# voichek/kmersGWAS

Measured on AMD Instinct MI355X. Metric: k-mers x permutations scored/sec, higher is better.
Workload: dtype fp4 x fp6/fp4 block-scaled filter + f32/f64 exact re-score

## Files before the change

include/kgwas.h:

```cpp
#ifndef KGWAS_H
#define KGWAS_H

#include <stddef.h>
#include <stdint.h>

#ifdef __cplusplus
extern "C" {
#endif

#define KGWAS_OK 0
#define KGWAS_ERR_ARG (-1)
#define KGWAS_ERR_IO (-2)
#define KGWAS_ERR_FORMAT (-3)
#define KGWAS_ERR_DEVICE (-4)
#define KGWAS_ERR_STATE (-5)
#define KGWAS_ERR_NOMEM (-6)

const char* kgwas_last_error(void);
int kgwas_version(void);
int kgwas_device_count(int* n_devices);
uint32_t kgwas_host_cpu_quota(void);

typedef struct kgwas_table kgwas_table;
int kgwas_table_open(const char* base, uint32_t kmer_len, kgwas_table** out);
int kgwas_table_info(const kgwas_table* t, uint64_t* n_acc_file, uint64_t* n_rows, uint64_t* words_per_row,
                     uint32_t* kmer_len);
int kgwas_table_name(const kgwas_table* t, uint64_t i, const char** name);
int kgwas_table_column_map(const kgwas_table* t, const char* const* acc, uint64_t n, uint64_t* col_out);
int kgwas_table_read_rows(kgwas_table* t, uint64_t row0, uint64_t n, uint64_t* dst);
void kgwas_table_close(kgwas_table* t);

typedef struct kgwas_pheno kgwas_pheno;
int kgwas_pheno_load(const char* path, kgwas_pheno** out);
int kgwas_pheno_info(const kgwas_pheno* p, uint64_t* n_pheno, uint64_t* n_acc);
int kgwas_pheno_name(const kgwas_pheno* p, uint64_t j, const char** name);
int kgwas_pheno_accession(const kgwas_pheno* p, uint64_t i, const char** acc);
int kgwas_pheno_values(const kgwas_pheno* p, const float** Y);
void kgwas_pheno_free(kgwas_pheno* p);

uint64_t kgwas_min_count(uint64_t n_acc, double maf, uint64_t mac);

int kgwas_heap_selfcheck(uint32_t flags);
typedef struct kgwas_heap kgwas_heap;
int kgwas_heap_new(uint64_t max_results, kgwas_heap** out);
int kgwas_heap_add_many(kgwas_heap* h, const uint64_t* kmer, const double* score, const uint64_t* row, uint64_t n);
int kgwas_heap_size(const kgwas_heap* h, uint64_t* size, uint64_t* insertions, double* lowest);
int kgwas_heap_pop_all(const kgwas_heap* h, uint64_t* kmer, double* score, uint64_t* row);
int kgwas_heap_output_list(const kgwas_heap* h, uint64_t* kmer, uint64_t* rank, uint64_t* row);
int kgwas_heap_rows_sorted(const kgwas_heap* h, uint64_t* row);
int kgwas_heap_output_to_file(const kgwas_heap* h, const char* path, int with_scores);
void kgwas_heap_free(kgwas_heap* h);

int kgwas_select_check(uint64_t topn, uint64_t n_chunks, const uint64_t* chunk_n, const uint64_t* chunk_row0, const double* chunk_thr,
                       const double* score, const uint64_t* kmer, const uint32_t* row_in_chunk, int by_ref, int64_t detach_after_chunk,
                       int* selected, uint64_t* out_kmer, double* out_score, uint64_t* out_row, uint64_t* out_n);

typedef struct kgwas_scan kgwas_scan;

#define KGWAS_KERNEL_AUTO 0
#define KGWAS_KERNEL_VALU 1
#define KGWAS_KERNEL_MFMA 2
#define KGWAS_KERNEL_COARSE 3
#define KGWAS_KERNEL_NARROW 4

typedef struct kgwas_scan_params {
    uint32_t struct_size;
    int32_t device;
    uint64_t n_acc_file;
    uint64_t n_acc;
    const uint64_t* col;
    uint64_t n_pheno;
    const float* Y;
    const uint64_t* topn;
    uint64_t min_count;
    uint64_t chunk_rows;
    uint32_t host_threads;
    uint32_t kernel;
    uint32_t record_history;
    uint32_t count_patterns;
} kgwas_scan_params;

typedef struct kgwas_scan_stats {
    uint64_t rows_fed;
    uint64_t rows_tested;
    uint64_t candidates;
    uint64_t heap_pushes;
    uint64_t chunks;
    uint64_t score_launches;
    double score_kernel_ms;
    double squeeze_kernel_ms;
    double replay_ms;
    double gpu_wait_ms;
    double dense_ms;
    double coarse_kernel_ms;
    uint64_t coarse_launches;
    uint32_t kernel_used;
    uint32_t direct_mode;
    uint64_t patterns;
    uint32_t coarse_mode_tiles[2];
    uint32_t coarse_mode_lgroups[2];
    uint64_t coarse_mode_launches[2];
    uint64_t coarse_mode_rows[2];
    double coarse_mode_ms[2];
    double replay_cpu_ms;
    double replay_tail_ms;
    uint32_t coarse_mode_tile_slices[2];
    uint32_t coarse_mx;
    uint32_t coarse_mx_s1_fp6;
    uint32_t coarse_mx_steps;
    uint32_t replay_threads;
    double replay_min_ms;
    double replay_wall_ms;
    uint64_t replay_splits;
    uint64_t columns_popped_ahead;
    uint32_t coarse_mx32;
    uint32_t coarse_mx_stream;
    uint32_t columns_selected;
    uint32_t columns_replayed_at_finish;
} kgwas_scan_stats;

#define KGWAS_ABI_VERSION 14
uint32_t kgwas_abi_version(void);

int kgwas_scan_create(const kgwas_scan_params* p, kgwas_scan** out);
int kgwas_scan_expect_finish(kgwas_scan* s);
int kgwas_scan_feed_device(kgwas_scan* s, const void* d_rows, uint64_t n_rows, uint64_t first_row, void* hip_stream);
int kgwas_scan_feed_host(kgwas_scan* s, const uint64_t* rows, uint64_t n_rows, uint64_t first_row);
int kgwas_scan_feed_table(kgwas_scan* s, kgwas_table* t, uint64_t row0, uint64_t n_rows);
int kgwas_scan_finish(kgwas_scan* s);
int kgwas_scan_result(kgwas_scan* s, uint64_t j, uint64_t* n, const uint64_t** kmer, const double** score,
                      const uint64_t** row);
int kgwas_scan_history(kgwas_scan* s, uint64_t j, uint64_t* n, const uint64_t** kmer, const double** score,
                       const uint64_t** row);
int kgwas_scan_get_stats(const kgwas_scan* s, kgwas_scan_stats* st);
int kgwas_scan_reset(kgwas_scan* s);
void kgwas_scan_destroy(kgwas_scan* s);

int kgwas_scan_lowest(kgwas_scan* s, double* lowest, uint8_t* full);
int kgwas_scan_select_mode(const kgwas_scan* s, int* on);
int kgwas_scan_debug_residuals(const kgwas_scan* s, uint32_t form, uint64_t column, double* out);
int kgwas_scan_debug_survivors(const kgwas_scan* s, uint64_t* n_chunks, uint64_t chunk, uint64_t* info, double* thr, uint32_t* pairs);
int kgwas_scan_absorb(kgwas_scan* s, uint64_t n_shards, const uint64_t* counts, const uint64_t* const* kmer,
                      const double* const* score, const uint64_t* const* row);
int kgwas_scan_history_above(kgwas_scan* s, const double* thr, uint64_t* counts, const uint64_t** kmer,
                             const double** score, const uint64_t** row);
int kgwas_scan_heaps_export(kgwas_scan* s, uint64_t n_cols, const uint64_t* cols, uint64_t* sizes, const uint64_t** kmer,
                            const double** score, const uint64_t** row);
int kgwas_scan_heaps_import(kgwas_scan* s, uint64_t n_cols, const uint64_t* cols, const uint64_t* sizes, const uint64_t* kmer,
                            const double* score, const uint64_t* row);
int kgwas_scan_history_above_msgs(kgwas_scan* s, const double* thr, uint64_t n_msgs, const uint64_t* msg_col0,
                                  const uint64_t* msg_ncols, uint64_t* out, uint64_t cap_words, uint64_t* msg_words);
int kgwas_scan_heaps_export_msgs(kgwas_scan* s, uint64_t n_msgs, const uint64_t* msg_col0, const uint64_t* msg_ncols,
                                 uint64_t* out, uint64_t cap_words, uint64_t* msg_words);

typedef struct kgwas_multiscan kgwas_multiscan;
int kgwas_multiscan_create(const kgwas_scan_params* p, const int32_t* devices, uint32_t n_devices, kgwas_multiscan** out);
int kgwas_multiscan_run_table(kgwas_multiscan* m, kgwas_table* t, uint64_t row0, uint64_t n_rows);
int kgwas_multiscan_run_device(kgwas_multiscan* m, const void* const* d_rows, const uint64_t* n_rows, const uint64_t* first_row);
int kgwas_multiscan_finish(kgwas_multiscan* m);
int kgwas_multiscan_result(kgwas_multiscan* m, uint64_t j, uint64_t* n, const uint64_t** kmer, const double** score,
                           const uint64_t** row);
int kgwas_multiscan_get_stats(const kgwas_multiscan* m, kgwas_scan_stats* total, kgwas_scan_stats* per_shard, double* scan_ms,
                              double* merge_ms, uint64_t* rescans);
void kgwas_multiscan_destroy(kgwas_multiscan* m);

int kgwas_scan_scores_dense(kgwas_scan* s, const void* rows, int rows_on_device, uint64_t n_rows, double* scores,
                            uint32_t* popcnt);

int kgwas_merge_shards(uint64_t n_pheno, const uint64_t* topn, uint64_t n_shards, const uint64_t* counts,
                       const uint64_t* const* kmer, const double* const* score, const uint64_t* const* row,
                       uint32_t threads, kgwas_heap** out_heaps);

typedef struct kgwas_kinship kgwas_kinship;
int kgwas_kinship_create(int32_t device, uint64_t n_acc_file, uint64_t min_count, kgwas_kinship** out);
int kgwas_kinship_feed_device(kgwas_kinship* k, const void* d_rows, uint64_t n_rows, void* hip_stream);
int kgwas_kinship_feed_host(kgwas_kinship* k, const uint64_t* rows, uint64_t n_rows);
int kgwas_kinship_feed_table(kgwas_kinship* k, kgwas_table* t, uint64_t row0, uint64_t n_rows);
int kgwas_kinship_partials(kgwas_kinship* k, uint64_t* hamming, uint64_t* n_used);
int kgwas_kinship_from_partials(uint64_t n_acc_file, const uint64_t* hamming, uint64_t n_used, uint64_t* K);
int kgwas_kinship_get_stats(const kgwas_kinship* k, double* kernel_ms, uint64_t* launches, uint64_t* rows_fed);
void kgwas_kinship_destroy(kgwas_kinship* k);
int kgwas_kinship_table_multi(const int32_t* devices, uint32_t n_devices, kgwas_table* t, uint64_t min_count, uint64_t* hamming,
                              uint64_t* n_used);
uint64_t kgwas_kinship_format(uint64_t n_acc_file, const uint64_t* K, uint64_t n_used, char* out, uint64_t cap);

int kgwas_write_plink(const char* out_base, kgwas_table* t, const uint64_t* col, uint64_t n_acc,
                      const char* const* acc_names, const float* y, uint64_t n, const uint64_t* kmer_pop,
                      const uint64_t* row_pop);
int kgwas_write_plink_many(uint64_t n_cols, const char* const* out_bases, kgwas_table* t, const uint64_t* col, uint64_t n_acc,
                           const char* const* acc_names, const float* Y, const uint64_t* n_win, const uint64_t* const* kmer_pop,
                           const uint64_t* const* row_pop, uint32_t threads);

int kgwas_table_to_bed(kgwas_table* t, const uint64_t* col, uint64_t n_acc, const char* const* acc_names, const float* y,
                       uint64_t min_count, uint64_t batch_size, int unique_patterns, const char* out_base, int device,
                       uint64_t* n_batches, uint64_t* n_written);

int kgwas_kmer_encode(const char* word, uint64_t len, uint64_t* code);
int kgwas_filter_kmers(kgwas_table* t, const uint64_t* codes, uint64_t n, int32_t device, uint64_t* file_rows, uint64_t* rows,
                       uint64_t* n_found);
int kgwas_filter_kmers_write(kgwas_table* t, const uint64_t* codes, uint64_t n, int32_t device, const char* out_path,
                             uint64_t* n_found);

int kgwas_build_table(const char* all_kmers_path, const char* const* kmer_paths, const char* const* names, uint64_t n,
                      uint32_t kmer_len, int32_t device, const char* out_base, uint64_t* n_rows);

int kgwas_list_kmers(const char* const* kmer_paths, uint64_t n, uint32_t kmer_len, uint64_t mac, double min_strand_percent,
                     int32_t device, const char* out_path, uint64_t counts[3]);

int kgwas_count_kmers_files(const char* const* paths, uint64_t n, uint32_t kmer_len, uint64_t ci, uint64_t cx, int32_t device,
                            const char* out_path, uint64_t counts[8]);
int kgwas_count_kmers_bases(const void* bases, uint64_t n_bytes, int on_device, uint32_t kmer_len, uint64_t ci, uint64_t cx,
                            int32_t device, const char* out_path, uint64_t counts[8]);

typedef struct kgwas_snps kgwas_snps;
int kgwas_snps_open(const char* base_bedbim, const char* const* samples, uint64_t n_samples, kgwas_snps** out);
int kgwas_snps_info(const kgwas_snps* s, uint64_t* n_snps, uint64_t* n_samples_file, uint64_t* bytes_per_snp);
int kgwas_snps_scores(kgwas_snps* s, const float* Y, uint64_t n_pheno, double mac, int device, double* scores);
int kgwas_snps_best(kgwas_snps* s, const float* Y, uint64_t n_pheno, uint64_t topn, double mac, int device, uint64_t* counts,
                    uint64_t* indices);
int kgwas_snps_write(kgwas_snps* s, uint64_t n_lists, const char* const* out_bases, const uint64_t* counts,
                     const uint64_t* indices, uint64_t stride);
void kgwas_snps_close(kgwas_snps* s);

typedef struct kgwas_snpkin kgwas_snpkin;
int kgwas_snpkin_open(const char* base_bedbim, int32_t device, kgwas_snpkin** out);
int kgwas_snpkin_info(const kgwas_snpkin* h, uint64_t* n_samples, uint64_t* n_snps, uint64_t* bytes_per_snp);
int kgwas_snpkin_feed_bed(kgwas_snpkin* h, const uint8_t* body, uint64_t n_snps);
int kgwas_snpkin_feed_file(kgwas_snpkin* h);
int kgwas_snpkin_sums(kgwas_snpkin* h, double* lower, uint64_t* n_used);
int kgwas_snpkin_matrix(kgwas_snpkin* h, double* K, uint64_t* n_used);
uint64_t kgwas_snpkin_format(uint64_t n_samples, const double* K, char* out, uint64_t cap);
void kgwas_snpkin_close(kgwas_snpkin* h);

typedef struct kgwas_lmm kgwas_lmm;
typedef struct kgwas_lmm_stats {
    double eigen_ms, rotate_ms, grid_ms, refine_ms;
    uint64_t variants_read, variants_tested, chunks, eigendecompositions, n_individuals;
} kgwas_lmm_stats;
int kgwas_sym_eigen(uint64_t n, const double* K, double* d, double* U, uint32_t threads);
int kgwas_lmm_create(uint64_t n, const double* K, int32_t device, double lmin, double lmax, uint64_t chunk_variants, kgwas_lmm** out);
int kgwas_lmm_null(kgwas_lmm* h, const double* y, double* logl0, double* lambda0);
int kgwas_lmm_test_bed(kgwas_lmm* h, const double* y, const uint8_t* bed_body, uint64_t n_variants, double maf, double miss, double* lrt,
                       double* lambda, double* p, double* af, uint32_t* n_miss, uint8_t* tested);
int kgwas_lmm_run_files(const char* kinship_path, uint64_t n_beds, const char* const* bfile_bases, const char* const* out_paths,
                        uint32_t pheno_col, double maf, double miss, double lmin, double lmax, uint64_t chunk_variants, int32_t device,
                        kgwas_lmm_stats* total);
int kgwas_lmm_test_bed_multi(kgwas_lmm* h, uint32_t n_pheno, const double* Y, const uint8_t* bed_body, uint64_t n_variants, double maf,
                             double miss, double* lrt, double* lambda, double* p, double* logl0, double* lambda0, double* af,
                             uint32_t* n_miss, uint8_t* tested);
int kgwas_lmm_run_file_multi(const char* kinship_path, const char* bfile_base, uint32_t n_cols, const uint32_t* pheno_cols,
                             const char* const* out_paths, double maf, double miss, double lmin, double lmax, uint64_t chunk_variants,
                             int32_t device, kgwas_lmm_stats* total);
int kgwas_lmm_get_stats(const kgwas_lmm* h, kgwas_lmm_stats* out);
void kgwas_lmm_destroy(kgwas_lmm* h);
int kgwas_lmm_read_kinship(const char* path, uint64_t n_expected, double* K);
int kgwas_lmm_read_fam(const char* path, uint32_t pheno_col, uint64_t cap, double* values, uint8_t* keep, uint64_t* n_lines);
uint64_t kgwas_lmm_format_assoc(const char* chr, const char* rs, const char* ps, uint32_t n_miss, const char* allele1, const char* allele0,
                                double af, double l_mle, double p_lrt, char* out, uint64_t cap);

int kgwas_synth_rows_device(void* d_rows, uint64_t first_row, uint64_t n_rows, uint64_t n_acc_file, uint64_t seed,
                            void* hip_stream);
int kgwas_synth_rows_host(uint64_t* rows, uint64_t first_row, uint64_t n_rows, uint64_t n_acc_file, uint64_t seed);

#ifdef __cplusplus
}
#endif
#endif
```

kmersgwas_amd/capi.py:

```python
from __future__ import annotations

import ctypes as C
import os

import numpy as np

_HERE = os.path.dirname(os.path.abspath(__file__))
LIB_PATH = os.environ.get("KGWAS_LIB") or os.path.join(_HERE, "lib", "libkgwas.so")

KGWAS_OK = 0
KGWAS_ERR_ARG, KGWAS_ERR_IO, KGWAS_ERR_FORMAT, KGWAS_ERR_DEVICE, KGWAS_ERR_STATE, KGWAS_ERR_NOMEM = -1, -2, -3, -4, -5, -6
KERNEL_AUTO, KERNEL_VALU, KERNEL_MFMA, KERNEL_COARSE, KERNEL_NARROW = 0, 1, 2, 3, 4

SYMBOLS = [
    "kgwas_last_error", "kgwas_version", "kgwas_abi_version", "kgwas_device_count", "kgwas_host_cpu_quota",
    "kgwas_table_open", "kgwas_table_info", "kgwas_table_name", "kgwas_table_column_map", "kgwas_table_read_rows",
    "kgwas_table_close",
    "kgwas_pheno_load", "kgwas_pheno_info", "kgwas_pheno_name", "kgwas_pheno_accession", "kgwas_pheno_values",
    "kgwas_pheno_free", "kgwas_min_count",
    "kgwas_heap_selfcheck", "kgwas_heap_new", "kgwas_heap_add_many", "kgwas_heap_size", "kgwas_heap_pop_all", "kgwas_heap_output_list", "kgwas_heap_rows_sorted", "kgwas_heap_output_to_file", "kgwas_select_check",
    "kgwas_heap_free",
    "kgwas_scan_create", "kgwas_scan_feed_device", "kgwas_scan_feed_host", "kgwas_scan_feed_table", "kgwas_scan_finish", "kgwas_scan_result",
    "kgwas_scan_history", "kgwas_scan_get_stats", "kgwas_scan_reset", "kgwas_scan_lowest", "kgwas_scan_select_mode", "kgwas_scan_debug_residuals", "kgwas_scan_debug_survivors", "kgwas_scan_absorb", "kgwas_scan_history_above", "kgwas_scan_heaps_export", "kgwas_scan_heaps_import", "kgwas_scan_expect_finish", "kgwas_scan_history_above_msgs", "kgwas_scan_heaps_export_msgs", "kgwas_scan_destroy", "kgwas_scan_scores_dense",
    "kgwas_merge_shards",
    "kgwas_multiscan_create", "kgwas_multiscan_run_table", "kgwas_multiscan_run_device", "kgwas_multiscan_finish",
    "kgwas_multiscan_result", "kgwas_multiscan_get_stats", "kgwas_multiscan_destroy", "kgwas_kinship_table_multi",
    "kgwas_kinship_create", "kgwas_kinship_feed_device", "kgwas_kinship_feed_host", "kgwas_kinship_feed_table", "kgwas_kinship_partials",
    "kgwas_kinship_from_partials", "kgwas_kinship_get_stats", "kgwas_kinship_destroy", "kgwas_kinship_format",
    "kgwas_write_plink", "kgwas_write_plink_many", "kgwas_table_to_bed",
    "kgwas_kmer_encode", "kgwas_filter_kmers", "kgwas_filter_kmers_write", "kgwas_build_table", "kgwas_list_kmers",
    "kgwas_count_kmers_files", "kgwas_count_kmers_bases",
    "kgwas_snps_open", "kgwas_snps_info", "kgwas_snps_scores", "kgwas_snps_best", "kgwas_snps_write", "kgwas_snps_close",
    "kgwas_snpkin_open", "kgwas_snpkin_info", "kgwas_snpkin_feed_bed", "kgwas_snpkin_feed_file", "kgwas_snpkin_sums",
    "kgwas_snpkin_matrix", "kgwas_snpkin_format", "kgwas_snpkin_close",
    "kgwas_sym_eigen", "kgwas_lmm_create", "kgwas_lmm_null", "kgwas_lmm_test_bed", "kgwas_lmm_run_files", "kgwas_lmm_get_stats",
    "kgwas_lmm_test_bed_multi", "kgwas_lmm_run_file_multi",
    "kgwas_lmm_destroy", "kgwas_lmm_read_kinship", "kgwas_lmm_read_fam", "kgwas_lmm_format_assoc",
    "kgwas_synth_rows_device", "kgwas_synth_rows_host",
]


class KgwasError(RuntimeError):
    def __init__(self, code: int, msg: str):
        super().__init__("libkgwas error %d: %s" % (code, msg))
        self.code = code
        self.msg = msg


class ScanParams(C.Structure):
    _fields_ = [
        ("struct_size", C.c_uint32), ("device", C.c_int32),
        ("n_acc_file", C.c_uint64), ("n_acc", C.c_uint64), ("col", C.POINTER(C.c_uint64)),
        ("n_pheno", C.c_uint64), ("Y", C.POINTER(C.c_float)), ("topn", C.POINTER(C.c_uint64)),
        ("min_count", C.c_uint64), ("chunk_rows", C.c_uint64),
        ("host_threads", C.c_uint32), ("kernel", C.c_uint32), ("record_history", C.c_uint32),
        ("count_patterns", C.c_uint32),
    ]


class ScanStats(C.Structure):
    _fields_ = [
        ("rows_fed", C.c_uint64), ("rows_tested", C.c_uint64), ("candidates", C.c_uint64),
        ("heap_pushes", C.c_uint64), ("chunks", C.c_uint64), ("score_launches", C.c_uint64),
        ("score_kernel_ms", C.c_double), ("squeeze_kernel_ms", C.c_double), ("replay_ms", C.c_double),
        ("gpu_wait_ms", C.c_double), ("dense_ms", C.c_double),
        ("coarse_kernel_ms", C.c_double), ("coarse_launches", C.c_uint64),
        ("kernel_used", C.c_uint32), ("direct_mode", C.c_uint32), ("patterns", C.c_uint64),
        ("coarse_mode_tiles", C.c_uint32 * 2), ("coarse_mode_lgroups", C.c_uint32 * 2),
        ("coarse_mode_launches", C.c_uint64 * 2), ("coarse_mode_rows", C.c_uint64 * 2),
        ("coarse_mode_ms", C.c_double * 2),
        ("replay_cpu_ms", C.c_double), ("replay_tail_ms", C.c_double),
        ("coarse_mode_tile_slices", C.c_uint32 * 2),
        ("coarse_mx", C.c_uint32), ("coarse_mx_s1_fp6", C.c_uint32), ("coarse_mx_steps", C.c_uint32),
        ("replay_threads", C.c_uint32),
        ("replay_min_ms", C.c_double), ("replay_wall_ms", C.c_double),
        ("replay_splits", C.c_uint64),
        ("columns_popped_ahead", C.c_uint64),
        ("coarse_mx32", C.c_uint32), ("coarse_mx_stream", C.c_uint32),
        ("columns_selected", C.c_uint32), ("columns_replayed_at_finish", C.c_uint32),
    ]

    def as_dict(self):
        d = {}
        for k, _ in self._fields_:
            v = getattr(self, k)
            d[k] = list(v) if hasattr(v, "__len__") else v
        return d


class LmmStats(C.Structure):
    _fields_ = [
        ("eigen_ms", C.c_double), ("rotate_ms", C.c_double), ("grid_ms", C.c_double), ("refine_ms", C.c_double),
        ("variants_read", C.c_uint64), ("variants_tested", C.c_uint64), ("chunks", C.c_uint64),
        ("eigendecompositions", C.c_uint64), ("n_individuals", C.c_uint64),
    ]

    def as_dict(self):
        return {k: getattr(self, k) for k, _ in self._fields_}


if not os.path.exists(LIB_PATH):
    raise ImportError(
        "libkgwas.so not found at %s — build it with `make -C kmersgwas_amd/csrc` "
        "(or __graft_entry__.build()). There is no fallback implementation." % LIB_PATH)



def _load_hip_runtime():
    import importlib.util
    cands = []
    try:
        spec = importlib.util.find_spec("torch")
        if spec and spec.origin:
            cands.append(os.path.join(os.path.dirname(spec.origin), "lib", "libamdhip64.so"))
    except Exception:
        pass
    rocm = os.environ.get("ROCM_PATH", "/opt/rocm")
    cands += [os.path.join(rocm, "lib", "libamdhip64.so.7"), os.path.join(rocm, "lib", "libamdhip64.so"),
              "libamdhip64.so.7", "libamdhip64.so"]
    errs = []
    for c in cands:
        if os.path.isabs(c) and not os.path.exists(c):
            continue
        try:
            return C.CDLL(c, mode=C.RTLD_GLOBAL), c
        except OSError as e:
            errs.append("%s: %s" % (c, e))
    raise ImportError("no HIP runtime (libamdhip64) could be loaded: %s" % "; ".join(errs))


_hip, HIP_RUNTIME_PATH = _load_hip_runtime()
lib = C.CDLL(LIB_PATH)

_vp, _u64, _u32, _i32, _dbl = C.c_void_p, C.c_uint64, C.c_uint32, C.c_int32, C.c_double
_pp = C.POINTER(C.c_void_p)
_pu64 = C.POINTER(C.c_uint64)
_pdbl = C.POINTER(C.c_double)
_pstr = C.POINTER(C.c_char_p)

lib.kgwas_last_error.restype = C.c_char_p
lib.kgwas_version.restype = C.c_int
lib.kgwas_device_count.argtypes = [C.POINTER(C.c_int)]
lib.kgwas_abi_version.argtypes = []
lib.kgwas_abi_version.restype = C.c_uint32
ABI_VERSION = 14
if lib.kgwas_abi_version() != ABI_VERSION:
    raise ImportError("libkgwas.so speaks ABI version %d, kmersgwas_amd/capi.py %d: rebuild (make -C kmersgwas_amd/csrc)" % (lib.kgwas_abi_version(), ABI_VERSION))
lib.kgwas_host_cpu_quota.argtypes = []
lib.kgwas_host_cpu_quota.restype = C.c_uint32
lib.kgwas_table_open.argtypes = [C.c_char_p, _u32, _pp]
lib.kgwas_table_info.argtypes = [_vp, _pu64, _pu64, _pu64, C.POINTER(_u32)]
lib.kgwas_table_name.argtypes = [_vp, _u64, _pstr]
lib.kgwas_table_column_map.argtypes = [_vp, _pstr, _u64, _pu64]
lib.kgwas_table_read_rows.argtypes = [_vp, _u64, _u64, _vp]
lib.kgwas_table_close.argtypes = [_vp]
lib.kgwas_table_close.restype = None
lib.kgwas_pheno_load.argtypes = [C.c_char_p, _pp]
lib.kgwas_pheno_info.argtypes = [_vp, _pu64, _pu64]
lib.kgwas_pheno_name.argtypes = [_vp, _u64, _pstr]
lib.kgwas_pheno_accession.argtypes = [_vp, _u64, _pstr]
lib.kgwas_pheno_values.argtypes = [_vp, C.POINTER(C.POINTER(C.c_float))]
lib.kgwas_pheno_free.argtypes = [_vp]
lib.kgwas_pheno_free.restype = None
lib.kgwas_min_count.argtypes = [_u64, _dbl, _u64]
lib.kgwas_min_count.restype = _u64
lib.kgwas_heap_new.argtypes = [_u64, _pp]
lib.kgwas_heap_add_many.argtypes = [_vp, _vp, _vp, _vp, _u64]
lib.kgwas_heap_size.argtypes = [_vp, _pu64, _pu64, _pdbl]
lib.kgwas_heap_pop_all.argtypes = [_vp, _vp, _vp, _vp]
lib.kgwas_heap_output_list.argtypes = [_vp, _vp, _vp, _vp]
lib.kgwas_heap_rows_sorted.argtypes = [_vp, _vp]
lib.kgwas_heap_output_to_file.argtypes = [_vp, C.c_char_p, C.c_int]
lib.kgwas_select_check.argtypes = [C.c_uint64, C.c_uint64, _vp, _vp, _vp, _vp, _vp, _vp, C.c_int, C.c_int64, C.POINTER(C.c_int), _vp, _vp, _vp, C.POINTER(C.c_uint64)]
lib.kgwas_heap_free.argtypes = [_vp]
lib.kgwas_heap_free.restype = None
lib.kgwas_scan_create.argtypes = [C.POINTER(ScanParams), _pp]
lib.kgwas_scan_feed_device.argtypes = [_vp, _vp, _u64, _u64, _vp]
lib.kgwas_scan_feed_host.argtypes = [_vp, _vp, _u64, _u64]
lib.kgwas_scan_feed_table.argtypes = [_vp, _vp, _u64, _u64]
lib.kgwas_scan_finish.argtypes = [_vp]
lib.kgwas_scan_expect_finish.argtypes = [_vp]
lib.kgwas_scan_result.argtypes = [_vp, _u64, _pu64, C.POINTER(_pu64), C.POINTER(_pdbl), C.POINTER(_pu64)]
lib.kgwas_scan_history.argtypes = [_vp, _u64, _pu64, C.POINTER(_pu64), C.POINTER(_pdbl), C.POINTER(_pu64)]
lib.kgwas_scan_get_stats.argtypes = [_vp, C.POINTER(ScanStats)]
lib.kgwas_scan_reset.argtypes = [_vp]
lib.kgwas_scan_lowest.argtypes = [_vp, _vp, _vp]
lib.kgwas_scan_select_mode.argtypes = [_vp, C.POINTER(C.c_int)]
lib.kgwas_scan_select_mode.restype = C.c_int
lib.kgwas_scan_debug_residuals.argtypes = [_vp, C.c_uint32, C.c_uint64, _vp]
lib.kgwas_scan_debug_residuals.restype = C.c_int
lib.kgwas_scan_debug_survivors.argtypes = [_vp, _vp, C.c_uint64, _vp, _vp, _vp]
lib.kgwas_scan_debug_survivors.restype = C.c_int
lib.kgwas_heap_selfcheck.argtypes = [C.c_uint32]
lib.kgwas_heap_selfcheck.restype = C.c_int
lib.kgwas_scan_absorb.argtypes = [_vp, _u64, _vp, _pp, _pp, _pp]
lib.kgwas_scan_history_above.argtypes = [_vp, _vp, _vp, _vp, _vp, _vp]
lib.kgwas_scan_heaps_export.argtypes = [_vp, _u64, _vp, _vp, _vp, _vp, _vp]
lib.kgwas_scan_history_above_msgs.argtypes = [_vp, _vp, _u64, _vp, _vp, _vp, _u64, _vp]
lib.kgwas_scan_heaps_export_msgs.argtypes = [_vp, _u64, _vp, _vp, _vp, _u64, _vp]
lib.kgwas_scan_heaps_import.argtypes = [_vp, _u64, _vp, _vp, _vp, _vp, _vp]
lib.kgwas_scan_destroy.argtypes = [_vp]
lib.kgwas_scan_destroy.restype = None
lib.kgwas_scan_scores_dense.argtypes = [_vp, _vp, C.c_int, _u64, _vp, _vp]
lib.kgwas_merge_shards.argtypes = [_u64, _vp, _u64, _vp, _pp, _pp, _pp, _u32, _pp]
lib.kgwas_multiscan_create.argtypes = [C.POINTER(ScanParams), _vp, _u32, _pp]
lib.kgwas_multiscan_run_table.argtypes = [_vp, _vp, _u64, _u64]
lib.kgwas_multiscan_run_device.argtypes = [_vp, _pp, _vp, _vp]
lib.kgwas_multiscan_finish.argtypes = [_vp]
lib.kgwas_multiscan_result.argtypes = [_vp, _u64, _pu64, C.POINTER(_pu64), C.POINTER(_pdbl), C.POINTER(_pu64)]
lib.kgwas_multiscan_get_stats.argtypes = [_vp, C.POINTER(ScanStats), _vp, _pdbl, _pdbl, _pu64]
lib.kgwas_multiscan_destroy.argtypes = [_vp]
lib.kgwas_multiscan_destroy.restype = None
lib.kgwas_kinship_table_multi.argtypes = [_vp, _u32, _vp, _u64, _vp, _pu64]
lib.kgwas_kinship_create.argtypes = [_i32, _u64, _u64, _pp]
lib.kgwas_kinship_feed_device.argtypes = [_vp, _vp, _u64, _vp]
lib.kgwas_kinship_feed_host.argtypes = [_vp, _vp, _u64]
lib.kgwas_kinship_feed_table.argtypes = [_vp, _vp, _u64, _u64]
lib.kgwas_kinship_partials.argtypes = [_vp, _vp, _pu64]
lib.kgwas_kinship_from_partials.argtypes = [_u64, _vp, _u64, _vp]
lib.kgwas_kinship_get_stats.argtypes = [_vp, _pdbl, _pu64, _pu64]
lib.kgwas_kinship_destroy.argtypes = [_vp]
lib.kgwas_kinship_destroy.restype = None
lib.kgwas_kinship_format.argtypes = [_u64, _vp, _u64, C.c_char_p, _u64]
lib.kgwas_kinship_format.restype = _u64
lib.kgwas_write_plink.argtypes = [C.c_char_p, _vp, _vp, _u64, _pstr, _vp, _u64, _vp, _vp]
lib.kgwas_write_plink_many.argtypes = [_u64, _pstr, _vp, _vp, _u64, _pstr, _vp, _vp, _pp, _pp, _u32]
lib.kgwas_snps_open.argtypes = [C.c_char_p, _pstr, _u64, _vp]
lib.kgwas_snps_info.argtypes = [_vp, _vp, _vp, _vp]
lib.kgwas_snps_scores.argtypes = [_vp, _vp, _u64, C.c_double, C.c_int, _vp]
lib.kgwas_snps_best.argtypes = [_vp, _vp, _u64, _u64, C.c_double, C.c_int, _vp, _vp]
lib.kgwas_snps_write.argtypes = [_vp, _u64, _pstr, _vp, _vp, _u64]
lib.kgwas_snps_close.argtypes = [_vp]
lib.kgwas_snps_close.restype = None
lib.kgwas_snpkin_open.argtypes = [C.c_char_p, _i32, _pp]
lib.kgwas_snpkin_info.argtypes = [_vp, _pu64, _pu64, _pu64]
lib.kgwas_snpkin_feed_bed.argtypes = [_vp, _vp, _u64]
lib.kgwas_snpkin_feed_file.argtypes = [_vp]
lib.kgwas_snpkin_sums.argtypes = [_vp, _vp, _pu64]
lib.kgwas_snpkin_matrix.argtypes = [_vp, _vp, _pu64]
lib.kgwas_snpkin_format.argtypes = [_u64, _vp, C.c_char_p, _u64]
lib.kgwas_snpkin_format.restype = _u64
lib.kgwas_snpkin_close.argtypes = [_vp]
lib.kgwas_snpkin_close.restype = None
lib.kgwas_table_to_bed.argtypes = [_vp, _vp, _u64, _pstr, _vp, _u64, _u64, C.c_int, C.c_char_p, C.c_int, _vp, _vp]
lib.kgwas_kmer_encode.argtypes = [C.c_char_p, _u64, _pu64]
lib.kgwas_filter_kmers.argtypes = [_vp, _vp, _u64, _i32, _vp, _vp, _pu64]
lib.kgwas_filter_kmers_write.argtypes = [_vp, _vp, _u64, _i32, C.c_char_p, _pu64]
lib.kgwas_build_table.argtypes = [C.c_char_p, _pstr, _pstr, _u64, _u32, _i32, C.c_char_p, _pu64]
lib.kgwas_list_kmers.argtypes = [_pstr, _u64, _u32, _u64, C.c_double, _i32, C.c_char_p, _pu64]
lib.kgwas_count_kmers_files.argtypes = [_pstr, _u64, _u32, _u64, _u64, _i32, C.c_char_p, _pu64]
lib.kgwas_count_kmers_bases.argtypes = [_vp, _u64, C.c_int, _u32, _u64, _u64, _i32, C.c_char_p, _pu64]
lib.kgwas_sym_eigen.argtypes = [_u64, _vp, _vp, _vp, _u32]
lib.kgwas_lmm_create.argtypes = [_u64, _vp, _i32, _dbl, _dbl, _u64, _pp]
lib.kgwas_lmm_null.argtypes = [_vp, _vp, _pdbl, _pdbl]
lib.kgwas_lmm_test_bed.argtypes = [_vp, _vp, _vp, _u64, _dbl, _dbl, _vp, _vp, _vp, _vp, _vp, _vp]
lib.kgwas_lmm_run_files.argtypes = [C.c_char_p, _u64, _pstr, _pstr, _u32, _dbl, _dbl, _dbl, _dbl, _u64, _i32, C.POINTER(LmmStats)]
lib.kgwas_lmm_test_bed_multi.argtypes = [_vp, _u32, _vp, _vp, _u64, _dbl, _dbl, _vp, _vp, _vp, _vp, _vp, _vp, _vp, _vp]
lib.kgwas_lmm_run_file_multi.argtypes = [C.c_char_p, C.c_char_p, _u32, _vp, _pstr, _dbl, _dbl, _dbl, _dbl, _u64, _i32, C.POINTER(LmmStats)]
lib.kgwas_lmm_get_stats.argtypes = [_vp, C.POINTER(LmmStats)]
lib.kgwas_lmm_destroy.argtypes = [_vp]
lib.kgwas_lmm_destroy.restype = None
lib.kgwas_lmm_read_kinship.argtypes = [C.c_char_p, _u64, _vp]
lib.kgwas_lmm_read_fam.argtypes = [C.c_char_p, _u32, _u64, _vp, _vp, _pu64]
lib.kgwas_lmm_format_assoc.argtypes = [C.c_char_p, C.c_char_p, C.c_char_p, _u32, C.c_char_p, C.c_char_p, _dbl, _dbl, _dbl, C.c_char_p, _u64]
lib.kgwas_lmm_format_assoc.restype = _u64
lib.kgwas_synth_rows_device.argtypes = [_vp, _u64, _u64, _u64, _u64, _vp]
lib.kgwas_synth_rows_host.argtypes = [_vp, _u64, _u64, _u64, _u64]


def check(rc: int) -> None:
    if rc != KGWAS_OK:
        raise KgwasError(rc, (lib.kgwas_last_error() or b"").decode(errors="replace"))


def ptr(a: np.ndarray):
    return a.ctypes.data_as(C.c_void_p)


def device_count() -> int:
    n = C.c_int(0)
    check(lib.kgwas_device_count(C.byref(n)))
    return n.value
```

kmersgwas_amd/csrc/kernels.h:

```cpp
#pragma once
#include <hip/hip_runtime.h>
#include <stdint.h>

#include "env.h"
#include "launch.h"

namespace kgwas {

struct Cand {
    uint64_t kmer;
    double score;
    uint64_t row;
};

struct RowSrc {
    const uint32_t* base;
    uint64_t stride_dw;
    uint32_t off_dw;
    uint32_t avail_dw;
};

constexpr uint32_t TESTED_SHARDS = 256;

struct ScoreArgs {
    RowSrc src;
    const uint32_t* dmask;
    const uint64_t* file_rows;
    uint64_t file_stride_w;
    uint64_t n_rows;
    uint64_t first_row;
    uint32_t S;
    uint32_t W_m;
    uint32_t n_pheno;
    uint32_t min_count;
    const float* Yperm;
    const float* Ymfma;
    const float* sums;
    const double* thr;
    double* dense;
    uint32_t* n1_out;
    uint64_t* kmer_out;
    Cand* cand;
    uint32_t* cand_cnt;
    uint32_t cap;
    unsigned long long* tested;
    uint32_t* hist;
    const uint32_t* hist_base;
    uint32_t hist_bins;
    double* so_score;
    uint64_t* so_kmer;
    uint32_t* so_row;
};

constexpr int HIST_SHIFT = 44;
constexpr uint32_t HIST_BINS = 16384;

hipError_t launch_copy_to_host(const void* src, void* dst_dev, size_t bytes, hipStream_t st);
hipError_t launch_chunk_tail(const uint32_t* meta, uint32_t n_meta, uint32_t* h_meta, const unsigned long long* tested, uint32_t n_tested,
                             unsigned long long* h_tested, const double* thr, uint32_t n_thr, double* h_thr, hipStream_t st);
hipError_t launch_thr_tail(const uint32_t* hist, const uint32_t* hist_base, uint32_t bins, const uint64_t* topn, const double* thr_host, double* thr,
                           uint32_t n_pheno, const uint32_t* meta, uint32_t n_meta, uint32_t* h_meta, const unsigned long long* tested,
                           uint32_t n_tested, unsigned long long* h_tested, double* h_thr, hipStream_t st);
hipError_t launch_records_to_host(const double* sc, const uint64_t* km, const uint32_t* rw, uint32_t n, double* h_sc, uint64_t* h_km, uint32_t* h_rw,
                                  hipStream_t st);
hipError_t launch_thr_update(const uint32_t* hist, const uint32_t* hist_base, uint32_t bins, const uint64_t* topn,
                             const double* thr_host, double* thr, uint32_t n_pheno, hipStream_t st);

hipError_t launch_dense_select(const double* dense, const uint32_t* n1, uint32_t n_rows, uint32_t n_pheno, uint32_t S, uint32_t min_count,
                               const uint64_t* topn, double* thr_a, double* thr_b, double* thr_host_copy, uint32_t* info, hipStream_t st);

hipError_t launch_score_valu(const ScoreArgs& a, hipStream_t st);
hipError_t launch_score_mfma(const ScoreArgs& a, uint32_t rows_per_block, uint32_t nb_full, hipStream_t st);
size_t mfma_lds_bytes(uint32_t W_m);

struct CoarseCol {
    double kalpha;
    float iu;
    int32_t pheno;
};
struct CoarseArgs {
    RowSrc src;
    uint64_t n_rows;
    uint32_t S, n_pheno, min_count;
    uint32_t n_kgroups;
    uint32_t n_lgroups;
    uint32_t n_slices;
    const int8_t* Bq;
    const CoarseCol* cols;
    const double* thr;
    unsigned long long* bitmap;
    uint64_t words_per_col;
    unsigned long long* tested;
    float eg_max, rall_max, rmax_max;
};
size_t coarse_lds_bytes(uint32_t n_kgroups, uint32_t T);
hipError_t launch_coarse(const CoarseArgs& a, uint32_t T, uint32_t rows_per_block, hipStream_t st);
struct MxArgs {
    RowSrc src;
    uint64_t n_rows;
    uint32_t S, n_pheno, min_count;
    uint32_t n_full, n_quarter;
    uint32_t n_lgroups;
    uint32_t n_slices;
    uint32_t s1_fp6;
    uint32_t scale0;
    const uint8_t* Bq;
    const CoarseCol* cols;
    const double* thr;
    unsigned long long* bitmap;
    uint64_t words_per_col;
    unsigned long long* tested;
    float eg_max, rall_max, rmax_max;
};
size_t mx_lds_bytes(uint32_t n_steps, uint32_t CT, uint32_t n_slices, uint32_t s1_fp6);
uint32_t mx_step_bytes_rt(uint32_t n_slices, uint32_t s1_fp6);
uint32_t mx_row_tiles(uint32_t CT);
hipError_t launch_mx(const MxArgs& a, uint32_t CT, uint32_t rows_per_block, hipStream_t st);
bool mxs_supported(uint32_t CT, uint32_t NG, uint32_t n_slices, uint32_t s1_fp6);
size_t mxs_lds_bytes(uint32_t CT, uint32_t NG);
hipError_t launch_mxs(const MxArgs& a, uint32_t CT, uint32_t NG, uint32_t form, uint32_t rows_per_block, hipStream_t st);
hipError_t launch_rescore(const ScoreArgs& a, const uint32_t* keys, const uint32_t* surv_off, const uint32_t* surv_cnt,
                          uint32_t row_bits, uint32_t* tile_pref, uint32_t* tile_cnt, double* tmp_score,
                          const uint32_t* key_count, uint32_t* meta, hipStream_t st);
hipError_t launch_rescore_direct(const ScoreArgs& a, const uint32_t* keys, const uint32_t* surv_off, const uint32_t* surv_cnt,
                                 uint32_t row_bits, const uint32_t* tile_pref, hipStream_t st);
struct PrepThr {
    const uint32_t* hist;
    const uint32_t* hist_base;
    uint32_t bins;
    const uint64_t* topn;
    const double* thr_host;
    double* thr;
};
hipError_t launch_chunk_prep(uint32_t* cand_cnt, uint32_t n_pheno, unsigned long long* tested, uint32_t* key_count,
                             unsigned long long* bitmap, uint64_t bitmap_words, uint32_t* seg_cnt, uint32_t n_seg_words, const PrepThr& tu,
                             hipStream_t st);

constexpr int NARROW_SLICES = 3;
constexpr uint32_t NARROW_MAX_COLS = 4;
struct NarrowCol {
    double w[NARROW_SLICES];
    double t1;
    double eg, rall, rmax;
    double pad;
    float wf[3];
    float slackf;
};
struct NarrowArgs {
    RowSrc src;
    uint64_t n_rows;
    uint32_t S, n_pheno, min_count;
    uint32_t n_kgroups;
    const uint8_t* Bn;
    const NarrowCol* cols;
    const double* thr;
    unsigned long long* bitmap;
    uint64_t words_per_col;
    unsigned long long* tested;
    uint32_t row_off;
    uint32_t* seg_cnt;
    uint32_t n_segs;
    uint64_t slack_rows;
    uint32_t pack1;
};
hipError_t launch_bitmap_keys(unsigned long long* bitmap, uint64_t words_per_col, uint64_t n_rows, uint32_t n_pheno, uint32_t* blk_scratch,
                              unsigned long long* blk_mask, uint32_t* keys_sorted, uint32_t key_cap, uint32_t row_bits, uint32_t* surv_off,
                              uint32_t* surv_cnt, uint32_t* key_count, uint32_t* tile_pref, bool nibble_transposed, hipStream_t st);
hipError_t launch_narrow_keys(const unsigned long long* bitmap, uint64_t words_per_col, uint64_t n_rows, uint32_t n_pheno, const uint32_t* seg_cnt,
                              uint32_t* keys_sorted, uint32_t key_cap, uint32_t row_bits, uint32_t* surv_off, uint32_t* surv_cnt,
                              uint32_t* key_count, uint32_t* tile_pref, uint32_t* meta, const unsigned long long* tested_shards, hipStream_t st);
size_t narrow_lds_bytes(uint32_t n_kgroups);
hipError_t launch_narrow(const NarrowArgs& a, uint32_t rows_per_block, hipStream_t st);

hipError_t launch_pattern_hash(const RowSrc& src, const uint32_t* dmask, uint64_t n_rows, uint32_t S, uint32_t W_m,
                               uint32_t min_count, uint64_t* out, unsigned long long* out_count, hipStream_t st);
hipError_t count_distinct_u64(uint64_t* keys, uint64_t n, uint64_t* result, hipStream_t st);

hipError_t launch_bed_rowinfo(const uint32_t* sq, uint64_t n_rows, uint32_t W_m, uint32_t* n1_out, uint64_t* hash_out,
                              hipStream_t st);
hipError_t launch_bed_bytes(const uint32_t* sq, uint64_t n_rows, uint32_t W_m, uint32_t bytes_per_row, uint8_t* out,
                            hipStream_t st);

hipError_t launch_snp_planes(const uint8_t* bed, uint64_t n_snps, uint32_t bytes_per_snp, const uint32_t* byte_idx,
                             const uint32_t* shift, uint32_t S, uint32_t ndw, uint32_t* planes, hipStream_t st);
hipError_t launch_snp_score(const uint32_t* planes, uint64_t n_snps, uint32_t ndw, const float* Yperm, uint32_t L, uint32_t n_pheno,
                            double mac, double* scores, hipStream_t st);

uint32_t snpkin_vals_stride(uint32_t S);
size_t snpkin_vals_bytes(uint32_t S, uint32_t chunk_snps);
size_t snpkin_params_bytes(uint32_t chunk_snps);
hipError_t launch_snpkin_prep(const uint8_t* bed, uint32_t n_snps, uint32_t bytes_per_snp, uint32_t S, void* params, void* vals,
                              unsigned long long* n_used, hipStream_t st);
hipError_t launch_snpkin_accumulate(int rows_per_wave, const uint8_t* bed, uint32_t n_snps, uint32_t bytes_per_snp, uint32_t S,
                                    const void* params, const void* vals, const uint2* tiles, uint32_t n_tiles, double* sums,
                                    hipStream_t st);

constexpr uint32_t FK_SPLITTERS = 4096;
hipError_t launch_fk_match(const uint64_t* rows, uint64_t stride, uint32_t n_rows, const uint64_t* L, uint64_t n,
                           const uint64_t* spl, uint32_t ns, uint64_t B, uint64_t carry_key, bool has_prev, uint64_t* lb,
                           uint64_t* cnt, uint32_t* head, uint32_t* first_desc, hipStream_t st);
size_t fk_scan_temp_bytes(uint32_t max_rows);
hipError_t launch_fk_select(const uint64_t* rows, uint64_t stride, uint32_t n_rows, const uint64_t* cnt, const uint32_t* head,
                            uint32_t* run_start, uint64_t carry_run, const uint32_t* first_desc, uint8_t* emit, uint32_t* sel,
                            uint32_t* n_sel, uint64_t* info, void* temp, size_t temp_bytes, hipStream_t st);
hipError_t launch_fk_keys(const uint64_t* rows, uint64_t stride, uint32_t r0, uint32_t n_rows, uint64_t* keys, hipStream_t st);
hipError_t launch_fk_gather(const uint64_t* rows, uint64_t stride, const uint32_t* sel, uint32_t m, uint64_t* out, hipStream_t st);
hipError_t launch_fk_format(const uint64_t* rows, uint64_t stride, const uint32_t* sel, uint32_t m, uint32_t k, uint32_t S_f,
                            void* text, hipStream_t st);

hipError_t launch_bt_init(uint64_t* A, uint64_t n, uint64_t stride, uint64_t* rows, hipStream_t st);
hipError_t launch_bt_match(const uint64_t* A, uint64_t n, const uint64_t* spl, uint32_t ns, uint64_t B, const uint64_t* slice,
                           uint32_t m, uint64_t carry_key, bool has_prev, uint64_t* rows, uint64_t stride, uint64_t accession,
                           uint32_t* descends, hipStream_t st);

constexpr uint32_t LL_MAX_SLOTS = 4096;
constexpr uint32_t LL_NEED_NONE = 0xFFFFFFFFu;
struct ListArgs {
    const uint64_t* words;
    const uint32_t* seg_off;
    const uint32_t* seg_len;
    uint32_t n_seg;
    const uint64_t* sample;
    uint32_t m, nb, slots;
    uint64_t N, mac;
    const uint32_t* need;
    uint64_t* stage_pass;
    uint64_t* stage_np_key;
    uint64_t* stage_np_cnt;
    uint32_t* bk_base;
    uint32_t* bk_pass;
    uint32_t* bk_np;
    unsigned long long* stats;
    uint32_t* flags;
    unsigned long long* err_key;
};
hipError_t launch_ll_check(const uint64_t* words, uint32_t m, uint64_t carry_key, bool has_prev, uint32_t file, uint32_t* flags,
                           hipStream_t st);
size_t ll_temp_bytes(uint32_t max_sample, uint32_t max_buckets);
hipError_t launch_ll_splitters(const uint64_t* words, uint64_t total, uint32_t m, uint64_t* sample_raw, uint64_t* sample, void* temp,
                               size_t temp_bytes, hipStream_t st);
size_t ll_count_lds_bytes(uint32_t slots);
hipError_t launch_ll_count(const ListArgs& a, hipStream_t st);
hipError_t launch_ll_gather(const ListArgs& a, uint32_t* off_pass, uint32_t* off_np, uint64_t* out_pass, uint64_t* out_np_key,
                            uint64_t* out_np_cnt, void* temp, size_t temp_bytes, hipStream_t st);
hipError_t launch_ll_commit(unsigned long long* total, unsigned long long* piece, uint64_t n, hipStream_t st);

constexpr uint64_t CK_MAX_PASS_WORDS = 1ull << 30;
uint32_t ck_blocks(uint64_t max_words);
size_t ck_temp_bytes(uint64_t max_words, uint32_t max_sample, uint32_t kmer_len);
hipError_t launch_ck_encode(const uint8_t* bases, uint64_t n, uint32_t kmer_len, uint64_t lo, uint64_t hi, uint64_t* words, uint64_t cap,
                            unsigned long long* ctr, hipStream_t st);
hipError_t launch_ck_sample(const uint8_t* bases, uint64_t n, uint32_t kmer_len, uint32_t m, uint64_t* sample, hipStream_t st);
hipError_t launch_ck_sort_sample(const uint64_t* raw, uint64_t* sorted, uint32_t m, void* temp, size_t temp_bytes, hipStream_t st);
hipError_t launch_ck_sort(const uint64_t* words, uint64_t* sorted, uint64_t n, uint32_t kmer_len, void* temp, size_t temp_bytes, hipStream_t st);
hipError_t launch_ck_heads(const uint64_t* sorted, uint64_t n, uint32_t* blk, uint32_t* off, uint32_t* heads, void* temp, size_t temp_bytes,
                           hipStream_t st);
hipError_t launch_ck_reduce(const uint64_t* sorted, uint64_t n, const uint32_t* heads, uint32_t n_runs, uint64_t ci, uint64_t cx, uint64_t* res,
                            uint32_t* blk, uint32_t* off, uint64_t* out, unsigned long long* counts, void* temp, size_t temp_bytes, hipStream_t st);

constexpr uint64_t SQUEEZE_MAX_WORDS = 319;
void check_squeeze_fits(const char* who, uint64_t S_f, uint64_t S);
hipError_t launch_squeeze(const uint64_t* file_rows, uint64_t file_stride_w, uint64_t n_rows, const uint32_t* colmap,
                          uint32_t W_m, uint32_t W_f, uint32_t* out, hipStream_t st);

hipError_t launch_synth(uint64_t* rows, uint64_t first_row, uint64_t n_rows, uint64_t n_acc, uint64_t seed,
                        hipStream_t st);

// ... 10 lines not shown
```

kmersgwas_amd/csrc/scan_api.cpp:

```cpp
#include "scan_internal.h"

namespace {
struct MsgPlan {
    std::vector<uint64_t> start;
    uint64_t total() const { return start.back(); }
};
struct FinishHint {
    kgwas_scan* s;
    bool given;
    explicit FinishHint(kgwas_scan* s_) : s(s_), given(s_ && s_->final_feed_next) {
        if (s) s->final_feed_next = false;
    }
    ~FinishHint() {
        if (s) s->final_feed_next = false;
    }
};

template <class Cnt>
MsgPlan plan_msgs(const kgwas_scan* s, uint64_t n_msgs, const uint64_t* col0, const uint64_t* ncols, uint64_t* msg_words, Cnt cnt, const char* who) {
    MsgPlan p;
    p.start.assign(n_msgs + 1, 0);
    for (uint64_t m = 0; m < n_msgs; m++) {
        if (ncols[m] && (col0[m] >= s->n_pheno || ncols[m] > s->n_pheno - col0[m])) throw Error(KGWAS_ERR_ARG, std::string(who) + ": columns out of range");
        uint64_t T = 0;
// ... 452 lines not shown
}

int kgwas_scan_heaps_export_msgs(kgwas_scan* s, uint64_t n_msgs, const uint64_t* msg_col0, const uint64_t* msg_ncols,
                                 uint64_t* out, uint64_t cap_words, uint64_t* msg_words) {
    return guarded([&] {
        if (!s || (n_msgs && (!msg_col0 || !msg_ncols || !msg_words))) throw Error(KGWAS_ERR_ARG, "kgwas_scan_heaps_export_msgs: null argument");
        lazy_materialize_all(s);
        const MsgPlan plan = plan_msgs(s, n_msgs, msg_col0, msg_ncols, msg_words, [&](uint64_t j) { return (uint64_t)s->heaps[j].size(); }, "kgwas_scan_heaps_export_msgs");
        if (!out || cap_words < plan.total()) return;
        struct Job {
            uint64_t j, ok, os, orw;
        };
        std::vector<Job> jobs;
        for (uint64_t m = 0; m < n_msgs; m++) {
            uint64_t* msg = out + plan.start[m];
            msg[0] = msg_words[m] - 1;
            uint64_t T = 0;
            for (uint64_t c = 0; c < msg_ncols[m]; c++) T += (msg[1 + c] = s->heaps[msg_col0[m] + c].size());
            uint64_t o = plan.start[m] + 1 + msg_ncols[m];
            for (uint64_t c = 0; c < msg_ncols[m]; c++) {
                const uint64_t j = msg_col0[m] + c;
                jobs.push_back(Job{j, o, o + T, o + 2 * T});
                o += s->heaps[j].size();
            }
        }
        static_assert(sizeof(double) == sizeof(uint64_t), "score bit patterns travel as 64-bit words");
        s->pool->parallel_for(jobs.size(), [&](size_t i) {
            const Job& b = jobs[i];
            s->heaps[b.j].export_state(out + b.ok, reinterpret_cast<double*>(out + b.os), out + b.orw);
        });
    });
}

int kgwas_scan_debug_residuals(const kgwas_scan* s, uint32_t form, uint64_t column, double* out) {
    return guarded([&] {
        if (!s || !out || form > 2 || column >= s->n_pheno) throw Error(KGWAS_ERR_ARG, "kgwas_scan_debug_residuals: bad argument");
        if (!s->dbg_keep_resid) throw Error(KGWAS_ERR_STATE, "kgwas_scan_debug_residuals: the session was not created under KGWAS_DEBUG_RESIDUALS=1");
        memcpy(out, s->dbg_resid[form].data() + column * s->S, s->S * sizeof(double));
    });
}

int kgwas_scan_debug_survivors(const kgwas_scan* s, uint64_t* n_chunks, uint64_t chunk, uint64_t* info, double* thr, uint32_t* pairs) {
    return guarded([&] {
        if (!s) throw Error(KGWAS_ERR_ARG, "kgwas_scan_debug_survivors: null session");
        if (!s->dbg_keep_surv) throw Error(KGWAS_ERR_STATE, "kgwas_scan_debug_survivors: the session was not created under KGWAS_DEBUG_SURVIVORS=1 (or has no filter)");
        if (n_chunks) *n_chunks = s->dbg_chunks.size();
        if (!info && !thr && !pairs) return;
        if (chunk >= s->dbg_chunks.size()) throw Error(KGWAS_ERR_ARG, "kgwas_scan_debug_survivors: no such chunk");
        const kgwas_scan::DbgChunk& ch = s->dbg_chunks[chunk];
        if (info) {
            info[0] = ch.first_row;
            info[1] = ch.n_rows;
            info[2] = ch.set;
            info[3] = ch.overflow;
            info[4] = ch.pairs.size() / 2;
        }
        if (thr) memcpy(thr, ch.thr.data(), s->n_pheno * sizeof(double));
        if (pairs && !ch.pairs.empty()) memcpy(pairs, ch.pairs.data(), ch.pairs.size() * sizeof(uint32_t));
    });
}

int kgwas_scan_select_mode(const kgwas_scan* s, int* on) {
    return guarded([&] {
        if (!s || !on) throw Error(KGWAS_ERR_ARG, "kgwas_scan_select_mode: null argument");
        *on = s->lazy_enabled ? 1 : 0;
    });
}

int kgwas_scan_lowest(kgwas_scan* s, double* lowest, uint8_t* full) {
    return guarded([&] {
        if (!s || !lowest || !full) throw Error(KGWAS_ERR_ARG, "kgwas_scan_lowest: null argument");
        for (uint64_t j = 0; j < s->n_pheno; j++) {
            if (s->lazy[j].on) {
                bool f = false;
                if (lazy_lowest(s, j, &lowest[j], &f)) {
                    full[j] = f ? 1 : 0;
                    continue;
                }
                s->st.heap_pushes += lazy_materialize(s, j);
            }
            lowest[j] = s->heaps[j].lowest();
            full[j] = s->heaps[j].full() ? 1 : 0;
        }
    });
}

int kgwas_scan_absorb(kgwas_scan* s, uint64_t n_shards, const uint64_t* counts, const uint64_t* const* kmer,
                      const double* const* score, const uint64_t* const* row) {
    return guarded([&] {
        if (!s || (n_shards && (!counts || !kmer || !score || !row))) throw Error(KGWAS_ERR_ARG, "kgwas_scan_absorb: null argument");
        const uint64_t P = s->n_pheno;
        std::vector<std::vector<uint64_t>> off(n_shards, std::vector<uint64_t>(P + 1, 0));
        for (uint64_t g = 0; g < n_shards; g++)
            for (uint64_t j = 0; j < P; j++) off[g][j + 1] = off[g][j] + counts[g * P + j];
        std::atomic<uint64_t> pushes(0);
        s->pool->parallel_for(P, [&](size_t j) {
            BestHeap& h = s->heaps[j];
            uint64_t local = 0;
            if (s->lazy[j].on) {
                for (uint64_t g = 0; g < n_shards; g++) {
                    const uint64_t o = off[g][j], n = counts[g * P + j];
                    for (uint64_t i = 0; i < n; i++) s->lazy[j].add(kmer[g][o + i], score[g][o + i], row[g][o + i]);
                }
                return;
            }
            for (uint64_t g = 0; g < n_shards; g++) {
                const uint64_t o = off[g][j], n = counts[g * P + j];
                for (uint64_t i = 0; i < n; i++)
                    if (h.add(kmer[g][o + i], score[g][o + i], (size_t)row[g][o + i])) {
                        local++;
                        if (s->record_history) s->hist[j].push(kmer[g][o + i], score[g][o + i], row[g][o + i]);
                    }
            }
            if (s->record_history) _mm_sfence();
        pushes += local;
        });
        s->st.heap_pushes += pushes.load();
        s->finished = false;
        for (uint64_t j = 0; j < s->n_pheno; j++) s->col_popped[j].store(0);
        refresh_full(s);
        KGWAS_HIP(hipSetDevice(s->device));
        s->hist_ready = false;
        upload_thresholds(s);
    });
}

int kgwas_scan_reset(kgwas_scan* s) {
    return guarded([&] {
        if (!s) throw Error(KGWAS_ERR_ARG, "kgwas_scan_reset: null");
        KGWAS_HIP(hipSetDevice(s->device));
        KGWAS_HIP(hipStreamSynchronize(s->stream));
        make_heaps(s);
        lazy_reset(s);
        for (uint64_t j = 0; j < s->n_pheno; j++) s->col_popped[j].store(0);
        s->final_feed_next = false;
        for (auto& h : s->hist) h.clear();
        s->all_full = false;
        s->hist_ready = false;
        s->rows_submitted = 0;
        s->pat_upper = 0;
        KGWAS_HIP(hipMemset(s->d_pat_cnt.p, 0, 8));
        KGWAS_HIP(hipStreamSynchronize(nullptr));
        s->rows_done = 0;
        s->finished = false;
        s->dbg_chunks.clear();
        const kgwas_scan_stats old = s->st;
        s->st = kgwas_scan_stats{};
        s->st.kernel_used = old.kernel_used;
        s->st.direct_mode = old.direct_mode;
        s->st.coarse_mx = old.coarse_mx;
        s->st.coarse_mx_s1_fp6 = old.coarse_mx_s1_fp6;
        s->st.coarse_mx_steps = old.coarse_mx_steps;
        s->st.coarse_mx_stream = old.coarse_mx_stream;
        s->st.replay_threads = old.replay_threads;
        for (int mi = 0; mi < 2; mi++) {
            s->st.coarse_mode_tiles[mi] = old.coarse_mode_tiles[mi];
            s->st.coarse_mode_lgroups[mi] = old.coarse_mode_lgroups[mi];
            s->st.coarse_mode_tile_slices[mi] = old.coarse_mode_tile_slices[mi];
        }
    });
}

int kgwas_scan_get_stats(const kgwas_scan* s, kgwas_scan_stats* st) {
    return guarded([&] {
        if (!s || !st) throw Error(KGWAS_ERR_ARG, "kgwas_scan_get_stats: null");
        *st = s->st;
    });
}

void kgwas_scan_destroy(kgwas_scan* s) { delete s; }

int kgwas_scan_scores_dense(kgwas_scan* s, const void* rows, int rows_on_device, uint64_t n_rows, double* scores,
                            uint32_t* popcnt) {
    return guarded([&] {
        if (!s || (!rows && n_rows) || !scores || !popcnt) throw Error(KGWAS_ERR_ARG, "kgwas_scan_scores_dense: null argument");
        KGWAS_HIP(hipSetDevice(s->device));
        const uint64_t stride = 1 + s->W_f;
        const uint64_t piece = s->dense_rows;
        if (!rows_on_device && s->d_stage.n < piece * stride) s->d_stage.alloc(piece * stride);
        std::vector<double> tmp(s->n_pheno * piece);
        for (uint64_t pos = 0; pos < n_rows; pos += piece) {
            const uint64_t c = std::min<uint64_t>(piece, n_rows - pos);
            const uint64_t* d_rows;
            if (rows_on_device) {
                d_rows = reinterpret_cast<const uint64_t*>(rows) + pos * stride;
            } else {
                KGWAS_HIP(hipMemcpy(s->d_stage.p, reinterpret_cast<const uint64_t*>(rows) + pos * stride, c * stride * 8,
                                    hipMemcpyHostToDevice));
                d_rows = s->d_stage.p;
            }
            run_dense(s, d_rows, c, pos, tmp.data(), popcnt + pos, false);
            for (uint64_t j = 0; j < s->n_pheno; j++)
                memcpy(scores + j * n_rows + pos, tmp.data() + j * c, c * sizeof(double));
        }
    });
}

struct kgwas_heap {
    BestHeap h;
    explicit kgwas_heap(size_t n) : h(n) {}
};

int kgwas_heap_new(uint64_t max_results, kgwas_heap** out) {
    return guarded([&] {
        if (!out || max_results == 0) throw Error(KGWAS_ERR_ARG, "kgwas_heap_new: bad argument");
        require_heap_emulation();
        *out = new kgwas_heap((size_t)max_results);
    });
}
int kgwas_heap_add_many(kgwas_heap* h, const uint64_t* kmer, const double* score, const uint64_t* row, uint64_t n) {
    return guarded([&] {
        if (!h || (n && (!kmer || !score || !row))) throw Error(KGWAS_ERR_ARG, "kgwas_heap_add_many: null argument");
        for (uint64_t i = 0; i < n; i++) h->h.add(kmer[i], score[i], (size_t)row[i]);
    });
}
int kgwas_heap_size(const kgwas_heap* h, uint64_t* size, uint64_t* insertions, double* lowest) {
    return guarded([&] {
        if (!h) throw Error(KGWAS_ERR_ARG, "kgwas_heap_size: null");
        if (size) *size = h->h.size();
        if (insertions) *insertions = h->h.inserted();
        if (lowest) *lowest = h->h.lowest();
    });
}
int kgwas_heap_pop_all(const kgwas_heap* h, uint64_t* kmer, double* score, uint64_t* row) {
    return guarded([&] {
        if (!h) throw Error(KGWAS_ERR_ARG, "kgwas_heap_pop_all: null");
        std::vector<uint64_t> k, r;
        std::vector<double> sc;
        h->h.pop_all(k, sc, r);
        if (kmer) memcpy(kmer, k.data(), k.size() * 8);
        if (score) memcpy(score, sc.data(), sc.size() * 8);
        if (row) memcpy(row, r.data(), r.size() * 8);
    });
}
int kgwas_heap_output_list(const kgwas_heap* h, uint64_t* kmer, uint64_t* rank, uint64_t* row) {
    return guarded([&] {
        if (!h || !kmer || !rank || !row) throw Error(KGWAS_ERR_ARG, "kgwas_heap_output_list: null");
        std::vector<uint64_t> k, r;
        std::vector<double> sc;
        h->h.pop_all(k, sc, r);
        const size_t n = k.size();
        std::vector<size_t> idx(n);
        for (size_t i = 0; i < n; i++) idx[i] = i;
        std::sort(idx.begin(), idx.end(), [&](size_t a, size_t b) { return r[a] < r[b]; });
        for (size_t i = 0; i < n; i++) {
            kmer[i] = k[idx[i]];
            rank[i] = n - idx[i];
            row[i] = r[idx[i]];
        }
    });
}
int kgwas_heap_rows_sorted(const kgwas_heap* h, uint64_t* row) {
    return guarded([&] {
        if (!h || !row) throw Error(KGWAS_ERR_ARG, "kgwas_heap_rows_sorted: null");
        const std::vector<uint64_t> r = h->h.rows_sorted();
        std::copy(r.begin(), r.end(), row);
    });
}
int kgwas_heap_output_to_file(const kgwas_heap* h, const char* path, int with_scores) {
    return guarded([&] {
        if (!h || !path) throw Error(KGWAS_ERR_ARG, "kgwas_heap_output_to_file: null");
        std::vector<uint64_t> k, r;
        std::vector<double> sc;
        h->h.pop_all(k, sc, r);
        FILE* f = fopen(path, "wb");
        if (!f) throw Error(KGWAS_ERR_IO, std::string("cannot open ") + path);
        bool ok = true;
        for (size_t i = 0; i < k.size() && ok; i++) {
            ok = fwrite(&k[i], 8, 1, f) == 1;
            if (ok && with_scores) ok = fwrite(&sc[i], 8, 1, f) == 1;
        }
        ok = (fclose(f) == 0) && ok;
        if (!ok) throw Error(KGWAS_ERR_IO, std::string("cannot write ") + path);
    });
}
void kgwas_heap_free(kgwas_heap* h) { delete h; }

int kgwas_merge_shards(uint64_t n_pheno, const uint64_t* topn, uint64_t n_shards, const uint64_t* counts,
                       const uint64_t* const* kmer, const double* const* score, const uint64_t* const* row,
                       uint32_t threads, kgwas_heap** out_heaps) {
    return guarded([&] {
        if (!topn || !counts || !kmer || !score || !row || !out_heaps) throw Error(KGWAS_ERR_ARG, "kgwas_merge_shards: null");
        for (uint64_t j = 0; j < n_pheno; j++) {
            if (topn[j] == 0) throw Error(KGWAS_ERR_ARG, "heap size must be >= 1");
            out_heaps[j] = new kgwas_heap((size_t)topn[j]);
        }
        std::vector<std::vector<uint64_t>> off(n_shards, std::vector<uint64_t>(n_pheno + 1, 0));
        for (uint64_t g = 0; g < n_shards; g++)
            for (uint64_t j = 0; j < n_pheno; j++) off[g][j + 1] = off[g][j] + counts[g * n_pheno + j];
        unsigned nt = threads ? threads : usable_cpus();
        nt = (unsigned)std::min<uint64_t>(nt, n_pheno);
        Pool pool(nt);
        pool.parallel_for(n_pheno, [&](size_t j) {
            BestHeap& h = out_heaps[j]->h;
            for (uint64_t g = 0; g < n_shards; g++) {
                const uint64_t o = off[g][j], n = counts[g * n_pheno + j];
                for (uint64_t i = 0; i < n; i++) h.add(kmer[g][o + i], score[g][o + i], (size_t)row[g][o + i]);
            }
        });
    });
}

}
```

kmersgwas_amd/csrc/scan_create.cpp:

```cpp
#include "scan_internal.h"
#include <chrono>

struct CreateTrace {
    const bool on = opt_set("KGWAS_TRACE");
    const std::chrono::steady_clock::time_point t0 = std::chrono::steady_clock::now();
    void operator()(const char* what) const {
        if (on)
            fprintf(stderr, "[kgwas] scan_create +%.1f ms: %s\n", std::chrono::duration<double, std::milli>(std::chrono::steady_clock::now() - t0).count(), what);
    }
};

static std::unique_ptr<kgwas_scan> new_session(const kgwas_scan_params* p, ScanShape& sh) {
    if (p->struct_size != sizeof(kgwas_scan_params)) throw Error(KGWAS_ERR_ARG, "kgwas_scan_params: size mismatch");
    if (!p->col || !p->Y || !p->topn || p->n_acc == 0 || p->n_pheno == 0 || p->n_acc_file == 0)
        throw Error(KGWAS_ERR_ARG, "kgwas_scan_create: empty problem");
    if (p->n_acc > p->n_acc_file) throw Error(KGWAS_ERR_ARG, "more phenotyped accessions than table columns");
    if (p->n_acc_file >= (1ull << 31)) throw Error(KGWAS_ERR_ARG, "too many accessions");
    require_heap_emulation();
    check_device(p->device);
    KGWAS_HIP(hipSetDevice(p->device));
    std::unique_ptr<kgwas_scan> s(new kgwas_scan);
    s->device = p->device;
    s->S_f = p->n_acc_file;
    s->S = p->n_acc;
    s->W_f = (s->S_f + 63) / 64;
    s->W_m = 2 * ((s->S + 127) / 128);
    s->L = 64 * s->W_m;
    s->n_pheno = p->n_pheno;
    s->min_count = p->min_count;
    s->col.assign(p->col, p->col + s->S);
    s->topn.assign(p->topn, p->topn + s->n_pheno);
    s->Y.assign(p->Y, p->Y + s->n_pheno * s->S);
    if (p->record_history > 2) throw Error(KGWAS_ERR_ARG, "record_history: 0 (off), 1 (full log) or 2 (eviction ring)");
    s->record_history = p->record_history == 1;
    if (p->record_history == 2) {
        s->history_ring = 1;
        if (const char* e = opt_str("KGWAS_HISTORY_RING"))
            if (atoll(e) > 0) s->history_ring = (size_t)atoll(e);
    }
    s->count_patterns = p->count_patterns != 0;
    std::vector<bool> seen(s->S_f, false);
    for (uint64_t i = 0; i < s->S; i++) {
        if (s->col[i] >= s->S_f) throw Error(KGWAS_ERR_ARG, "column index out of range");
        if (seen[s->col[i]]) throw Error(KGWAS_ERR_ARG, "duplicate column index");
        seen[s->col[i]] = true;
    }
    for (uint64_t j = 0; j < s->n_pheno; j++) {
        if (s->topn[j] == 0) throw Error(KGWAS_ERR_ARG, "heap size must be >= 1");
        s->max_topn = std::max(s->max_topn, s->topn[j]);
        s->sum_topn += s->topn[j];
    }
    s->direct = true;
    for (uint64_t i = 0; i < s->S; i++) s->direct = s->direct && (s->col[i] == i);
    if (!s->direct) check_squeeze_fits("kgwas_scan_create", s->S_f, s->S);

    bool finite = true;
    for (float v : s->Y) finite = finite && std::isfinite(v);
    bool chain_safe = finite;
    for (uint64_t j = 0; j < s->n_pheno && chain_safe; j++) {
        double a = 0;
        for (uint64_t i = 0; i < s->S; i++) a += std::fabs((double)s->Y[j * s->S + i]);
        chain_safe = a * (1.0 + (double)(s->S + 8) * 0x1p-23) < 0.99 * (double)std::numeric_limits<float>::max();
    }
    sh = ScanShape{s->S, s->L, s->W_m, s->W_f, s->n_pheno, s->max_topn, s->direct, finite, chain_safe};
    return s;
}

static void create_streams(kgwas_scan* s, const CreateTrace& tcreate) {
    KGWAS_HIP(hipStreamCreateWithFlags(&s->stream, hipStreamNonBlocking));
    tcreate("stream created (HIP context up)");
    KGWAS_HIP(hipEventCreate(&s->ev_user));
    KGWAS_HIP(hipEventCreate(&s->ev_ds));
    KGWAS_HIP(hipEventCreateWithFlags(&s->ev_dcopy, hipEventDisableTiming));
    KGWAS_HIP(hipEventCreate(&s->ev_d0));
    KGWAS_HIP(hipEventCreate(&s->ev_d1));
    tcreate("events created");
}

static std::vector<float> upload_exact_layouts(kgwas_scan* s, const ScanShape& sh, const CreateTrace& tcreate) {
    ExactLayouts ex = exact_layouts(sh, s->col, s->Y);
    s->nb_full = ex.nb_full;
    tcreate("phenotype layouts built (host)");
    const uint64_t P = s->n_pheno;
    s->d_dmask.alloc(ex.dmask.size());
    s->d_colmap.alloc(ex.colmap.size());
    s->d_sums.alloc(P);
    s->d_thr.alloc(P);
    s->h_thr.alloc(8 * P);
    s->d_thr_host.alloc(P);
    s->d_thr_redo.alloc(P);
    s->h_thr_redo.alloc(P);
    s->d_hist.alloc(P * (size_t)HIST_BINS);
    s->d_hist_base.alloc(P);
    s->h_hist_base.alloc(P);
    s->d_pat_cnt.alloc(1);
    KGWAS_HIP(hipMemset(s->d_pat_cnt.p, 0, 8));
    KGWAS_HIP(hipMemset(s->d_thr.p, 0, P * sizeof(double)));
    KGWAS_HIP(hipMemset(s->d_thr_host.p, 0, P * sizeof(double)));
    KGWAS_HIP(hipStreamSynchronize(nullptr));
    s->d_topn.alloc(P);
    s->d_sel.alloc(P);
    s->h_sel.alloc(P);
    s->d_sel_info.alloc(2);
    s->h_sel_info.alloc(2);
    KGWAS_HIP(hipMemcpy(s->d_topn.p, s->topn.data(), P * 8, hipMemcpyHostToDevice));
    KGWAS_HIP(hipMemcpy(s->d_dmask.p, ex.dmask.data(), ex.dmask.size() * 4, hipMemcpyHostToDevice));
    KGWAS_HIP(hipMemcpy(s->d_colmap.p, ex.colmap.data(), ex.colmap.size() * 4, hipMemcpyHostToDevice));
    KGWAS_HIP(hipMemcpy(s->d_sums.p, ex.sums.data(), P * 4, hipMemcpyHostToDevice));
    if (s->kernel_used == KGWAS_KERNEL_MFMA) {
        s->d_Ymfma.alloc(ex.Ymfma.size());
        KGWAS_HIP(hipMemcpy(s->d_Ymfma.p, ex.Ymfma.data(), ex.Ymfma.size() * 4, hipMemcpyHostToDevice));
    }
    if (s->kernel_used != KGWAS_KERNEL_MFMA || s->coarse) {
        s->d_Yperm.alloc(ex.Yperm.size());
        KGWAS_HIP(hipMemcpy(s->d_Yperm.p, ex.Yperm.data(), ex.Yperm.size() * 4, hipMemcpyHostToDevice));
    }
    tcreate("small device buffers allocated and uploaded");
    return std::move(ex.sums);
}

static void upload_filters(kgwas_scan* s, const ScanPlan& pl, const ScanShape& sh, const std::vector<float>& sums) {
    if (pl.narrow) {
        const NarrowOperands op = narrow_operands(sh, pl, s->Y, sums, s->dbg_keep_resid ? s->dbg_resid[2].data() : nullptr);
        s->d_Bn.alloc(op.Bn.size());
        s->d_ncols.alloc(sh.P);
        KGWAS_HIP(hipMemcpy(s->d_Bn.p, op.Bn.data(), op.Bn.size(), hipMemcpyHostToDevice));
        KGWAS_HIP(hipMemcpy(s->d_ncols.p, op.ncols.data(), sh.P * sizeof(NarrowCol), hipMemcpyHostToDevice));
    }
    for (int mi = 0; mi < 2; mi++) {
        const FilterSet& fs = pl.set[mi];
        if (!fs.slices) continue;
        kgwas_scan::CoarseMode& M = s->cmode[mi];
        M.mx = fs.mx;
        M.mx_full = fs.n_full;
        M.mx_quarter = fs.n_quarter;
        M.mx_s1_fp6 = fs.s1_fp6;
        if (fs.mx) M.mx_scale0 = 0x01010101u * (uint32_t)(0x7F + (fs.slices == 1 ? 0 : 5));
        M.slices = fs.slices;
        M.n_parts = (uint32_t)fs.parts.size();
        M.tile_slices = fs.tile_slices;
        M.tile_slices_eq = fs.tile_slices_eq;
        uint32_t groups_all = 0;
        for (size_t pi = 0; pi < fs.parts.size(); pi++) {
            const FilterPart& fp = fs.parts[pi];
            kgwas_scan::CoarsePart& Pt = M.part[pi];
            Pt.T = fp.T;
            Pt.n_lgroups = (uint32_t)(fp.groups / fp.ng);
            Pt.stream = fp.stream;
            Pt.ng = fp.ng;
            if (fp.stream) s->st.coarse_mx_stream = fp.stream;
            groups_all += Pt.n_lgroups;
            double* resid = s->dbg_keep_resid ? s->dbg_resid[mi].data() : nullptr;
            const PartOperands op = fs.mx ? block_scaled_operands(sh, fs, fp, s->Y, sums, resid)
                                          : int8_operands(sh, pl.n_kgroups, fs, fp, s->Y, sums, resid);
            M.eg_max = std::max(M.eg_max, op.eg_max);
            M.rall_max = std::max(M.rall_max, op.rall_max);
            M.rmax_max = std::max(M.rmax_max, op.rmax_max);
            Pt.d_Bq.alloc(op.Bq.size());
            Pt.d_cols.alloc(op.cols.size());
            KGWAS_HIP(hipMemcpy(Pt.d_Bq.p, op.Bq.data(), op.Bq.size(), hipMemcpyHostToDevice));
            KGWAS_HIP(hipMemcpy(Pt.d_cols.p, op.cols.data(), op.cols.size() * sizeof(CoarseCol), hipMemcpyHostToDevice));
        }
        s->st.coarse_mode_tiles[mi] = M.part[0].T;
        s->st.coarse_mode_lgroups[mi] = groups_all;
        s->st.coarse_mode_tile_slices[mi] = M.tile_slices;
        if (fs.mx) {
            if (pl.use_mx) s->st.coarse_mx = 1;
            s->st.coarse_mx_s1_fp6 = fs.s1_fp6;
            s->st.coarse_mx_steps = fs.n_steps;
        }
        M.ready = true;
    }
}

static void alloc_filter_buffers(kgwas_scan* s) {
    const uint64_t P = s->n_pheno;
    s->key_slots = (uint32_t)std::min<uint64_t>((uint64_t)s->cap * P, 0x7FFFFFFFull);
    s->d_surv_sorted.alloc(s->key_slots);
    s->bitmap_words = (s->chunk_max + 63) / 64;
    s->d_bitmap.alloc(P * s->bitmap_words);
    s->d_bm_blocks.alloc(P * ((s->bitmap_words + 1023) / 1024 + 1) + 4);
    if (!s->narrow) s->d_bm_mask.alloc(P * ((s->bitmap_words + 1023) / 1024) * 4 + 4);
    s->bitmap_clean = false;
    s->d_surv_cnt.alloc(P);
    s->d_surv_off.alloc(P);
    s->d_key_count.alloc(2);
    s->d_tile_pref.alloc(P + 1);
    s->d_tile_cnt.alloc((size_t)s->key_slots / 256 + P + 2);
    s->d_tmp_score.alloc(s->key_slots);
    int least = 0, greatest = 0;
    KGWAS_HIP(hipDeviceGetStreamPriorityRange(&least, &greatest));
    const bool hi = !(exp_int("KGWAS_COPY_PRIO", 1) == 0);
    KGWAS_HIP(hipStreamCreateWithPriority(&s->copy_stream, hipStreamNonBlocking, hi ? greatest : least));
    s->row_key_bits = 1;
    while (s->row_key_bits < 32 && (1ull << s->row_key_bits) < s->chunk_max) s->row_key_bits++;
}

static void alloc_slots(kgwas_scan* s, const CreateTrace& tcreate) {
    const uint64_t P = s->n_pheno;
    if (!s->direct) s->d_sq.alloc(s->chunk_max * 2 * s->W_m);
    if (s->coarse) {
        const uint64_t slot_bytes = (uint64_t)s->key_slots * 20;
        s->n_slots = (int)std::min<uint64_t>(MAX_SLOTS, std::max<uint64_t>(4, (4ull << 30) / std::max<uint64_t>(slot_bytes, 1)));
        s->ring_size = (size_t)std::max<uint64_t>(std::min<uint64_t>(1ull << 30, std::min<uint64_t>((uint64_t)s->n_slots * slot_bytes, std::max<uint64_t>(64ull << 20, 8 * slot_bytes))),
                                                  2 * slot_bytes + 4096);
        if (opt_str("KGWAS_RING_BYTES"))
            s->ring_size = (size_t)std::max<uint64_t>(strtoull(opt_str("KGWAS_RING_BYTES"), nullptr, 10), slot_bytes + 4096);
        tcreate("device buffers and slots allocated");
        s->ring.alloc(s->ring_size);
        s->ring_dev = s->ring.dev();
        tcreate("pinned record ring allocated");
    } else {
        const uint64_t slot_bytes = (uint64_t)s->cap * P * sizeof(Cand);
        s->n_slots = (int)std::min<uint64_t>(16, std::max<uint64_t>(4, (1ull << 30) / std::max<uint64_t>(slot_bytes, 1)));
    }
    for (int si = 0; si < s->n_slots + (s->coarse ? 1 : 0); si++) {
        const bool is_redo = si == s->n_slots;
        Slot& sl = is_redo ? s->redo : s->slot[si];
        if (s->coarse && !is_redo) {
            sl.d_so_score.alloc(s->key_slots);
            sl.d_so_kmer.alloc(s->key_slots);
            sl.d_so_row.alloc(s->key_slots);
            sl.d_meta.alloc(2 * P + 4);
            sl.h_meta.alloc(2 * P + 4);
            sl.h_thr.alloc(P);
            memset(sl.h_thr.p, 0, P * sizeof(double));
            memset(sl.h_meta.p, 0, (2 * P + 4) * sizeof(uint32_t));
            sl.h_meta_dev = sl.h_meta.dev();
            sl.h_thr_dev = sl.h_thr.dev();
            KGWAS_HIP(hipEventCreateWithFlags(&sl.ev_counts, hipEventBlockingSync));
        } else {
            sl.cand.alloc((uint64_t)s->cap * P);
            sl.d_cand = sl.cand.dev();
        }
        sl.d_cnt.alloc(P);
        sl.h_cnt.alloc(P);
        sl.d_tested.alloc(TESTED_SHARDS);
        sl.h_tested.alloc(TESTED_SHARDS);
        sl.h_tested_dev = sl.h_tested.dev();
        KGWAS_HIP(hipEventCreate(&sl.ev_sq0));
        KGWAS_HIP(hipEventCreate(&sl.ev_k0));
        KGWAS_HIP(hipEventCreate(&sl.ev_k1));
        KGWAS_HIP(hipEventCreateWithFlags(&sl.ev_done, hipEventBlockingSync));
        KGWAS_HIP(hipEventCreate(&sl.ev_mid));
    }
    s->d_dense.alloc(P * s->dense_rows);
    s->h_dense.alloc(P * s->dense_rows);
    s->d_n1.alloc(s->dense_rows);
    s->h_n1.alloc(s->dense_rows);
    s->d_kmer.alloc(s->dense_rows);
    s->h_kmer.alloc(s->dense_rows);
    s->h_dense_dev = s->h_dense.dev();
    s->h_n1_dev = s->h_n1.dev();
    s->h_kmer_dev = s->h_kmer.dev();
    s->d_tested_dense.alloc(TESTED_SHARDS);
}

static void make_heaps_and_select(kgwas_scan* s) {
    make_heaps(s);
    const char* fr = opt_str("KGWAS_FULL_REPLAY");
    s->lazy_enabled = s->coarse && !s->record_history && !(fr && atoi(fr) != 0);
    s->lazy_log_mode = s->lazy_enabled && s->history_ring != 0;
    lazy_reset(s);
    s->hist.resize(s->n_pheno);
    s->keys.resize(s->n_pheno);
    s->col_ms.assign(s->n_pheno, 0.0);
}

static void make_replay_pool(kgwas_scan* s, const kgwas_scan_params& p) {
    const uint64_t P = s->n_pheno;
    s->trace = opt_set("KGWAS_TRACE");
    unsigned nt = p.host_threads ? p.host_threads : usable_cpus();
    if (const char* e = opt_str("KGWAS_HOST_THREADS"))
        if (atoi(e) > 0) nt = (unsigned)atoi(e);
    nt = (unsigned)std::min<uint64_t>(nt, P);
    s->pool.reset(new Pool(nt, pick_replay_cpus(nt, s->device)));
    s->st.replay_threads = nt;
    s->ingest.producer_cpus_ = p.host_threads ? p.host_threads : usable_cpus();
    const uint64_t T = nt, base = P / T;
    const uint64_t MKc = (uint64_t)BestHeap::MAX_LOCKSTEP;
    uint64_t per = base ? (base + ((base + MKc - 1) / MKc) - 1) / ((base + MKc - 1) / MKc) : 0;
    if (const char* e = exp_str("KGWAS_REPLAY_GROUP"))
        if (atoi(e) > 0 && per) per = std::min<uint64_t>((uint64_t)atoi(e), MKc);
    for (uint64_t w = 0; w < T && base; w++) {
        std::vector<uint32_t> cur;
        for (uint64_t i = 0; i < base; i++) {
            cur.push_back((uint32_t)(i * T + w));
            if (cur.size() == per || i + 1 == base) {
                s->grp_cols.push_back(cur);
                s->grp_home.push_back((int)w);
                cur.clear();
            }
        }
    }
    for (uint64_t j = base * T; j < P; j++) {
        s->grp_cols.push_back(std::vector<uint32_t>(1, (uint32_t)j));
        s->grp_home.push_back(-1);
    }
    s->n_groups0 = s->grp_cols.size();
    s->n_groups.store(s->n_groups0);
    s->grp_cols0 = s->grp_cols;
    const size_t cap = s->n_groups0 + (size_t)P;
    s->grp_cols.resize(cap);
// ... 66 lines not shown
```

kmersgwas_amd/csrc/scan_gpu.cpp:

```cpp
#include "scan_internal.h"

namespace kgwas {


void fill_args(kgwas_scan* s, ScoreArgs& a, const uint64_t* d_rows, uint64_t n_rows, uint64_t first_row,
               bool squeezed) {
    memset(&a, 0, sizeof(a));
    if (squeezed) {
        a.src.base = s->d_sq.p;
        a.src.stride_dw = 2 * s->W_m;
        a.src.off_dw = 0;
        a.src.avail_dw = (uint32_t)(2 * s->W_m);
    } else {
        a.src.base = reinterpret_cast<const uint32_t*>(d_rows);
        a.src.stride_dw = 2 * (1 + s->W_f);
        a.src.off_dw = 2;
        a.src.avail_dw = (uint32_t)(2 * s->W_f);
    }
    a.dmask = s->d_dmask.p;
    a.file_rows = d_rows;
    a.file_stride_w = 1 + s->W_f;
    a.n_rows = n_rows;
    a.first_row = first_row;
    a.S = (uint32_t)s->S;
// ... 236 lines not shown
    kgwas_scan::DbgChunk ch;
    ch.first_row = first_row;
    ch.n_rows = n_rows;
    ch.set = set;
    ch.thr.resize(s->n_pheno);
    KGWAS_HIP(hipMemcpyAsync(ch.thr.data(), d_thr, s->n_pheno * sizeof(double), hipMemcpyDeviceToHost, s->stream));
    KGWAS_HIP(hipStreamSynchronize(s->stream));
    s->dbg_chunks.push_back(std::move(ch));
}

static void dbg_log_survivors(kgwas_scan* s) {
    kgwas_scan::DbgChunk& ch = s->dbg_chunks.back();
    const uint64_t P = s->n_pheno;
    std::vector<uint32_t> off(P), cnt(P);
    uint32_t total = 0;
    KGWAS_HIP(hipMemcpyAsync(off.data(), s->d_surv_off.p, P * sizeof(uint32_t), hipMemcpyDeviceToHost, s->stream));
    KGWAS_HIP(hipMemcpyAsync(cnt.data(), s->d_surv_cnt.p, P * sizeof(uint32_t), hipMemcpyDeviceToHost, s->stream));
    KGWAS_HIP(hipMemcpyAsync(&total, s->d_key_count.p, sizeof(uint32_t), hipMemcpyDeviceToHost, s->stream));
    KGWAS_HIP(hipStreamSynchronize(s->stream));
    ch.overflow = total > s->key_slots ? 1u : 0u;
    if (ch.overflow || !total) return;
    std::vector<uint32_t> keys(total);
    KGWAS_HIP(hipMemcpyAsync(keys.data(), s->d_surv_sorted.p, (size_t)total * sizeof(uint32_t), hipMemcpyDeviceToHost, s->stream));
    KGWAS_HIP(hipStreamSynchronize(s->stream));
    const uint32_t row_mask = s->row_key_bits >= 32 ? 0xFFFFFFFFu : (1u << s->row_key_bits) - 1u;
    for (uint64_t p = 0; p < P; p++) {
        if ((uint64_t)off[p] + cnt[p] > total) throw Error(KGWAS_ERR_STATE, "survivor log: a column's key range leaves the list");
        for (uint32_t i = 0; i < cnt[p]; i++) {
            const uint32_t key = keys[off[p] + i];
            ch.pairs.push_back(s->row_key_bits >= 32 ? 0u : key >> s->row_key_bits);
            ch.pairs.push_back(key & row_mask);
        }
    }
}

void submit_sparse(kgwas_scan* s, Slot& sl, const uint64_t* d_rows, uint64_t n_rows, uint64_t first_row,
                   bool count_hist) {
    ScoreArgs a;
    fill_args(s, a, d_rows, n_rows, first_row, !s->direct);
    a.cand = sl.d_cand;
    a.cand_cnt = sl.d_cnt.p;
    a.cap = s->cap;
    a.tested = sl.d_tested.p;
    if (count_hist) {
        if (!s->hist_ready) start_histograms(s);
        a.hist = s->d_hist.p;
        a.hist_base = s->d_hist_base.p;
        a.hist_bins = HIST_BINS;
    } else {
        for (uint64_t j = 0; j < s->n_pheno; j++) s->h_thr_redo.p[j] = s->lazy[j].on ? s->lazy[j].bound() : s->heaps[j].lowest();
        KGWAS_HIP(hipMemcpyAsync(s->d_thr_redo.p, s->h_thr_redo.p, s->n_pheno * sizeof(double), hipMemcpyHostToDevice,
                                 s->stream));
        a.thr = s->d_thr_redo.p;
    }
    const bool use_coarse = s->coarse && count_hist;
    if (!s->direct) {
        KGWAS_HIP(hipEventRecord(sl.ev_sq0, s->stream));
        maybe_squeeze(s, d_rows, n_rows);
        KGWAS_HIP(hipEventRecord(sl.ev_k0, s->stream));
    }
    {
        const uint64_t n_words = (n_rows + 63) / 64;
        const uint32_t n_segs = (uint32_t)((n_words + 1023) / 1024);
        PrepThr tu;
        memset(&tu, 0, sizeof(tu));
        if (use_coarse && s->narrow && s->hist_ready) {
            tu.hist = s->d_hist.p;
            tu.hist_base = s->d_hist_base.p;
            tu.bins = HIST_BINS;
            tu.topn = s->d_topn.p;
            tu.thr_host = s->d_thr_host.p;
            tu.thr = s->d_thr.p;
        }
        const bool zero_bitmap = use_coarse && (s->narrow || !s->bitmap_clean);
        const uint64_t zero_words = !zero_bitmap ? 0 : (s->narrow ? s->n_pheno * n_words : s->d_bitmap.n);
        const auto prep = [&] {
            return launch_chunk_prep(sl.d_cnt.p, (uint32_t)s->n_pheno, sl.d_tested.p, use_coarse ? s->d_key_count.p : nullptr,
                                     zero_bitmap ? s->d_bitmap.p : nullptr, zero_words,
                                     (use_coarse && s->narrow) ? s->d_bm_blocks.p : nullptr, (use_coarse && s->narrow) ? (uint32_t)s->n_pheno * n_segs : 0u,
                                     tu, s->stream);
        };
        if (s->direct) KGWAS_HIP(bind_stop(sl.ev_k0, s->stream, prep));
        else KGWAS_HIP(prep());
    }
    sl.used_coarse = use_coarse;
    if (use_coarse) {
        CoarseArgs c;
        memset(&c, 0, sizeof(c));
        c.src = a.src;
        c.n_rows = n_rows;
        c.S = a.S;
        c.n_pheno = a.n_pheno;
        c.min_count = a.min_count;
        c.n_kgroups = s->n_kgroups;
        const int cm = s->narrow ? 0 : pick_coarse_mode(s);
        if (s->dbg_keep_surv) dbg_log_thresholds(s, a.thr, n_rows, first_row, s->narrow ? 2u : (uint32_t)cm);
        const kgwas_scan::CoarseMode& M = s->cmode[cm];
        sl.coarse_mode = cm;
        sl.cand_est = (double)s->sum_topn * (double)n_rows / (double)std::max<uint64_t>(s->rows_submitted, 1);
        c.n_slices = M.slices;
        c.eg_max = M.eg_max;
        c.rall_max = M.rall_max;
        c.rmax_max = M.rmax_max;
        c.thr = a.thr;
        c.tested = a.tested;
        static const uint32_t rpb_env = (uint64_t)exp_int("KGWAS_COARSE_RPB", 0u);
        const uint64_t n_words = (n_rows + 63) / 64;
        if (s->narrow) {
            NarrowArgs na;
            memset(&na, 0, sizeof(na));
            na.src = a.src;
            na.n_rows = n_rows;
            na.S = a.S;
            na.n_pheno = a.n_pheno;
            na.min_count = a.min_count;
            na.n_kgroups = s->n_kgroups;
            na.Bn = s->d_Bn.p;
            na.cols = s->d_ncols.p;
            na.thr = a.thr;
            na.bitmap = s->d_bitmap.p;
            na.words_per_col = n_words;
            na.tested = a.tested;
            na.pack1 = s->narrow_pack1 ? 1u : 0u;
            na.seg_cnt = s->d_bm_blocks.p;
            na.n_segs = (uint32_t)((n_words + 1023) / 1024);
            na.slack_rows = s->direct ? s->slack_rows : 0;
            KGWAS_HIP(bind_stop(sl.ev_mid, s->stream, [&] { return launch_narrow(na, rpb_env ? rpb_env : (n_rows >= (1u << 24) ? 1280u : n_rows >= (1u << 18) ? 768u : 256u), s->stream); }));
        } else {
            s->bitmap_clean = false;
            c.bitmap = s->d_bitmap.p;
            c.words_per_col = n_words;
            for (uint32_t pi = 0; pi < M.n_parts; pi++) {
                const kgwas_scan::CoarsePart& Pt = M.part[pi];
                c.n_lgroups = Pt.n_lgroups;
                c.Bq = Pt.d_Bq.p;
                c.cols = Pt.d_cols.p;
                c.tested = pi == 0 ? a.tested : nullptr;
                const bool last_part = pi + 1u == M.n_parts;
                const uint32_t rpb = rpb_env ? rpb_env : (n_rows >= (1u << 22) ? 4096u : n_rows >= (1u << 20) ? 2048u : 512u);
                if (M.mx) {
                    MxArgs x;
                    memset(&x, 0, sizeof(x));
                    x.src = c.src;
                    x.n_rows = n_rows;
                    x.S = c.S;
                    x.n_pheno = c.n_pheno;
                    x.min_count = c.min_count;
                    x.n_full = M.mx_full;
                    x.n_quarter = M.mx_quarter;
                    x.n_lgroups = Pt.n_lgroups;
                    x.n_slices = M.slices;
                    x.s1_fp6 = M.mx_s1_fp6;
                    x.scale0 = M.mx_scale0;
                    x.Bq = reinterpret_cast<const uint8_t*>(Pt.d_Bq.p);
                    x.cols = Pt.d_cols.p;
                    x.thr = c.thr;
                    x.bitmap = c.bitmap;
                    x.words_per_col = c.words_per_col;
                    x.tested = c.tested;
                    x.eg_max = c.eg_max;
                    x.rall_max = c.rall_max;
                    x.rmax_max = c.rmax_max;
                    const auto filt = [&] {
                        return Pt.stream ? launch_mxs(x, Pt.T, Pt.ng, Pt.stream - 1u, rpb, s->stream) : launch_mx(x, Pt.T, rpb, s->stream);
                    };
                    if (last_part) KGWAS_HIP(bind_stop(sl.ev_mid, s->stream, filt));
                    else KGWAS_HIP(filt());
                } else {
                    const auto filt = [&] { return launch_coarse(c, Pt.T, rpb, s->stream); };
                    if (last_part) KGWAS_HIP(bind_stop(sl.ev_mid, s->stream, filt));
                    else KGWAS_HIP(filt());
                }
            }
            if (!M.n_parts) KGWAS_HIP(hipEventRecord(sl.ev_mid, s->stream));
        }
        a.tested = nullptr;
        a.so_score = sl.d_so_score.p;
        a.so_kmer = sl.d_so_kmer.p;
        a.so_row = sl.d_so_row.p;
        if (s->narrow) {
            KGWAS_HIP(launch_narrow_keys(s->d_bitmap.p, n_words, n_rows, (uint32_t)s->n_pheno, s->d_bm_blocks.p, s->d_surv_sorted.p, s->key_slots,
                                         s->row_key_bits, s->d_surv_off.p, s->d_surv_cnt.p, s->d_key_count.p, s->d_tile_pref.p, sl.d_meta.p, sl.d_tested.p, s->stream));
            if (s->dbg_keep_surv) dbg_log_survivors(s);
            KGWAS_HIP(bind_stop(sl.ev_k1, s->stream, [&] { return launch_rescore_direct(a, s->d_surv_sorted.p, s->d_surv_off.p, s->d_surv_cnt.p, s->row_key_bits, s->d_tile_pref.p, s->stream); }));
        } else {
        KGWAS_HIP(launch_bitmap_keys(s->d_bitmap.p, n_words, n_rows, (uint32_t)s->n_pheno, s->d_bm_blocks.p, s->d_bm_mask.p, s->d_surv_sorted.p, s->key_slots,
                                     s->row_key_bits, s->d_surv_off.p, s->d_surv_cnt.p, s->d_key_count.p, s->d_tile_pref.p, !s->narrow, s->stream));
        s->bitmap_clean = true;
        if (s->dbg_keep_surv) dbg_log_survivors(s);
        a.so_score = sl.d_so_score.p;
        a.so_kmer = sl.d_so_kmer.p;
        a.so_row = sl.d_so_row.p;
        KGWAS_HIP(bind_stop(sl.ev_k1, s->stream, [&] {
            return launch_rescore(a, s->d_surv_sorted.p, s->d_surv_off.p, s->d_surv_cnt.p, s->row_key_bits, s->d_tile_pref.p,
                                  s->d_tile_cnt.p, s->d_tmp_score.p, s->d_key_count.p, sl.d_meta.p, s->stream);
        }));
        }
        s->st.score_launches++;
    } else {
        if (s->direct) KGWAS_HIP(hipEventRecord(sl.ev_k0, s->stream));
        launch_score(s, a);
        KGWAS_HIP(hipEventRecord(sl.ev_k1, s->stream));
    }
    const bool fused_tail = use_coarse && s->narrow;
    static const bool tail_kernel = !(exp_int("KGWAS_TAIL_KERNEL", 1) == 0);
    const bool one_launch = use_coarse && tail_kernel && sl.h_meta_dev;
    const bool thr_and_tail = one_launch && s->hist_ready && !fused_tail;
    if (s->hist_ready && !fused_tail && !thr_and_tail)
        KGWAS_HIP(launch_thr_update(s->d_hist.p, s->d_hist_base.p, HIST_BINS, s->d_topn.p, s->d_thr_host.p, s->d_thr.p,
                                    (uint32_t)s->n_pheno, s->stream));
    if (!fused_tail && !one_launch)
        KGWAS_HIP(hipMemcpyAsync(sl.h_tested.p, sl.d_tested.p, TESTED_SHARDS * sizeof(unsigned long long), hipMemcpyDeviceToHost,
                                 s->stream));
    sl.tested_in_meta = fused_tail;
    if (thr_and_tail) {
        const bool thr_too = s->lazy_any.load(std::memory_order_relaxed);
        KGWAS_HIP(bind_stop(sl.ev_counts, s->stream, [&] {
            return launch_thr_tail(s->d_hist.p, s->d_hist_base.p, HIST_BINS, s->d_topn.p, s->d_thr_host.p, s->d_thr.p, (uint32_t)s->n_pheno, sl.d_meta.p,
                                   (uint32_t)(2 * s->n_pheno + 4), sl.h_meta_dev, sl.d_tested.p, (uint32_t)TESTED_SHARDS, sl.h_tested_dev,
                                   thr_too ? sl.h_thr_dev : nullptr, s->stream);
        }));
    } else if (one_launch) {
        const bool thr_too = s->lazy_any.load(std::memory_order_relaxed);
        KGWAS_HIP(bind_stop(sl.ev_counts, s->stream, [&] {
            return launch_chunk_tail(sl.d_meta.p, (uint32_t)(2 * s->n_pheno + 4), sl.h_meta_dev, sl.d_tested.p, fused_tail ? 0u : (uint32_t)TESTED_SHARDS,
                                     sl.h_tested_dev, s->d_thr.p, thr_too ? (uint32_t)s->n_pheno : 0u, sl.h_thr_dev, s->stream);
        }));
    } else if (use_coarse) {
        KGWAS_HIP(hipMemcpyAsync(sl.h_meta.p, sl.d_meta.p, (2 * s->n_pheno + 4) * sizeof(uint32_t), hipMemcpyDeviceToHost, s->stream));
        if (s->lazy_any.load(std::memory_order_relaxed))
            KGWAS_HIP(hipMemcpyAsync(sl.h_thr.p, s->d_thr.p, s->n_pheno * sizeof(double), hipMemcpyDeviceToHost, s->stream));
        KGWAS_HIP(hipEventRecord(sl.ev_counts, s->stream));
    } else {
        KGWAS_HIP(hipMemcpyAsync(sl.h_cnt.p, sl.d_cnt.p, s->n_pheno * sizeof(uint32_t), hipMemcpyDeviceToHost, s->stream));
        KGWAS_HIP(hipEventRecord(sl.ev_done, s->stream));
    }
    sl.rows = d_rows;
    sl.first_row = first_row;
    sl.n_rows = n_rows;
    sl.busy = true;
    s->st.chunks++;
}

bool chunk_complete(kgwas_scan* s, Slot& sl) {
    sl.busy = false;
    float ms = 0;
    KGWAS_HIP(hipEventElapsedTime(&ms, sl.ev_k0, sl.ev_k1));
    s->st.score_kernel_ms += ms;
    if (sl.used_coarse) {
        float mc = 0;
        KGWAS_HIP(hipEventElapsedTime(&mc, sl.ev_k0, sl.ev_mid));
        s->st.coarse_kernel_ms += mc;
        s->st.coarse_launches++;
        s->st.coarse_mode_ms[sl.coarse_mode] += mc;
        s->st.coarse_mode_launches[sl.coarse_mode]++;
        s->st.coarse_mode_rows[sl.coarse_mode] += sl.n_rows;
    }
    if (!s->direct) {
        float mq = 0;
        KGWAS_HIP(hipEventElapsedTime(&mq, sl.ev_sq0, sl.ev_k0));
        s->st.squeeze_kernel_ms += mq;
    }
    bool over = false;
    if (sl.used_coarse) {
        over = sl.h_meta.p[2 * s->n_pheno + 1] > s->key_slots;
    } else {
        for (uint64_t j = 0; j < s->n_pheno && !over; j++) over = sl.h_cnt.p[j] > s->cap;
    }
    if (s->trace) {
        uint64_t tot = 0, mx = 0;
        for (uint64_t q = 0; q < s->n_pheno; q++) {
            const uint64_t v = sl.used_coarse ? sl.h_meta.p[q] : sl.h_cnt.p[q];
            tot += v;
            mx = std::max<uint64_t>(mx, v);
        }
        fprintf(stderr, "[kgwas] chunk rows=%llu first=%llu kernel=%.3fms records %llu (max per column %llu)%s%s\n",
                (unsigned long long)sl.n_rows, (unsigned long long)sl.first_row, ms, (unsigned long long)tot,
                (unsigned long long)mx, sl.used_coarse ? (" survivors " + std::to_string(sl.h_meta.p[2 * s->n_pheno + 1])).c_str() : "",
                over ? " OVERFLOW" : "");
    }
    if (over) return false;
    if (sl.tested_in_meta)
        s->st.rows_tested += (uint64_t)sl.h_meta.p[2 * s->n_pheno + 2] | ((uint64_t)sl.h_meta.p[2 * s->n_pheno + 3] << 32);
    else
        for (uint32_t i = 0; i < TESTED_SHARDS; i++) s->st.rows_tested += sl.h_tested.p[i];
    return true;
}

uint64_t next_sparse_chunk(const kgwas_scan* s) {
    const double m = (double)std::max<uint64_t>(s->rows_submitted, 1);
    static const double fill_env = exp_num("KGWAS_FILL", 0.0);
    const double fill = fill_env > 0.0 ? fill_env : (s->narrow ? (s->lazy_any.load(std::memory_order_relaxed) ? 0.15 : 0.05) : 0.4);
    double c;
    if (s->coarse) {
        const double infl = s->narrow ? 1.0 : std::max(1.0, s->infl_obs[pick_coarse_mode(s)]);
        c = fill * m * (double)s->key_slots / (infl * (double)std::max<uint64_t>(s->sum_topn, 1));
    } else {
        c = m * (double)s->cap / (3.0 * (double)std::max<uint64_t>(s->max_topn, 1));
    }
    uint64_t ci = (uint64_t)std::min<double>(c, (double)s->chunk_max);
    ci = std::max<uint64_t>(ci, std::min<uint64_t>(s->dense_rows, s->chunk_max));
    ci = std::min<uint64_t>(ci, s->chunk_max);
    return (ci + 127) / 128 * 128;
}

void wait_event(kgwas_scan* s, hipEvent_t ev) {
// ... 84 lines not shown
```

kmersgwas_amd/csrc/scan_internal.h:

```cpp
#pragma once
#include <algorithm>
#include <atomic>
#include <chrono>
#include <cmath>
#include <condition_variable>
#include <deque>
#include <limits>
#include <cstdio>
#include <cstdlib>
#include <cstring>
#include <functional>
#include <memory>
#include <mutex>
#include <string>
#include <thread>
#include <vector>

#include <dirent.h>
#include <immintrin.h>
#include <pthread.h>
#include <sched.h>
#include <sys/mman.h>

#include "common.h"
// ... 183 lines not shown
    struct Ent {
        uint64_t bits;
        uint64_t kmer, row;
    };
    static constexpr uint64_t NEG_INF = 0xFFF0000000000000ull;
    bool on = false;
    bool bad = false;
    uint64_t topn = 0;
    uint64_t n_logged = 0;
    uint64_t bound_bits = 0;
    bool have_bound = false;
    uint32_t n_prunes = 0;
    struct Seg {
        const double* sc;
        const uint64_t* km;
        const uint32_t* rw;
        uint64_t row0;
        size_t off;
        uint32_t n;
    };
    std::vector<Seg> segs;
    double* l_sc = nullptr;
    uint64_t* l_km = nullptr;
    uint64_t* l_rw = nullptr;
    size_t l_n = 0, l_cap = 0;
    std::vector<Ent> pool;
    template <class F>
    inline void for_each(F&& f) const {
        for (const Seg& g : segs) {
            if (g.sc) {
                for (uint32_t i = 0; i < g.n; i++) f(g.sc[i], g.km[i], g.row0 + g.rw[i]);
            } else {
                for (size_t i = g.off; i < g.off + g.n; i++) f(l_sc[i], l_km[i], l_rw[i]);
            }
        }
    }
    inline void owned_appended(size_t n) {
        if (!segs.empty() && !segs.back().sc && segs.back().off + segs.back().n == l_n - n && (uint64_t)segs.back().n + n < (1ull << 32))
            segs.back().n += (uint32_t)n;
        else
            segs.push_back(Seg{nullptr, nullptr, nullptr, 0, l_n - n, (uint32_t)n});
    }
    void detach();
    LazyCol() = default;
    LazyCol(const LazyCol&) = delete;
    LazyCol& operator=(const LazyCol&) = delete;
    LazyCol(LazyCol&& o) noexcept { *this = std::move(o); }
    LazyCol& operator=(LazyCol&& o) noexcept {
        if (this != &o) {
            release_log();
            on = o.on, bad = o.bad, topn = o.topn, n_logged = o.n_logged, bound_bits = o.bound_bits, have_bound = o.have_bound, n_prunes = o.n_prunes;
            l_sc = o.l_sc, l_km = o.l_km, l_rw = o.l_rw, l_n = o.l_n, l_cap = o.l_cap;
            o.l_sc = nullptr, o.l_km = nullptr, o.l_rw = nullptr, o.l_n = o.l_cap = 0;
            segs = std::move(o.segs);
            o.segs.clear();
            scan_seg = o.scan_seg, scan_off = o.scan_off, unscanned = o.unscanned;
            pool = std::move(o.pool);
        }
        return *this;
    }
    ~LazyCol() { release_log(); }
    void release_log() {
        free(l_sc);
        free(l_km);
        free(l_rw);
        l_sc = nullptr, l_km = nullptr, l_rw = nullptr;
        l_n = l_cap = 0;
        segs.clear();
        scan_seg = 0, scan_off = 0, unscanned = 0;
    }
    void reserve_log(size_t need);
    void reset(bool enable, uint64_t topn_);
    void compact();
    void prune(uint64_t thr_bits);
    bool select(std::vector<uint64_t>& kmer, std::vector<double>& score, std::vector<uint64_t>& row);
    bool ties_now();
    void take_chunk(const double* sc, const uint64_t* km, const uint32_t* rw, uint32_t n, uint64_t row0, uint64_t thr_bits, bool by_ref);
    inline bool full() const { return n_logged >= topn; }
    inline double bound() const {
        double v = 0.0;
        if (have_bound) memcpy(&v, &bound_bits, 8);
        return v;
    }
    inline void add(uint64_t kmer, double score, uint64_t row) {
        uint64_t b;
        memcpy(&b, &score, 8);
        if (b == NEG_INF) return;
        if (l_n == l_cap) reserve_log(l_n + 1);
        l_sc[l_n] = score;
        l_km[l_n] = kmer;
        l_rw[l_n] = row;
        l_n++;
        owned_appended(1);
        n_logged++;
        if (++unscanned >= 4 * topn + 1024) scan_pending();
    }
    void scan_pending();
    size_t scan_seg = 0;
    uint32_t scan_off = 0;
    uint64_t unscanned = 0;
};

inline size_t ring_size(size_t forced, uint64_t topn) {
    if (forced > 1) return forced;
    const double r = 16.0 * std::sqrt(2.0 * (double)topn);
    return (size_t)std::min<double>(std::max<double>(r, 256.0), 1048576.0);
}

constexpr int MAX_SLOTS = 48;

struct ReplayAcc {
    uint64_t pushes = 0, cands = 0, busy_ns = 0, units = 0;
};

struct Slot {
    PinBuf<Cand> cand;
    Cand* d_cand = nullptr;
    DevBuf<uint32_t> d_cnt;
    PinBuf<uint32_t> h_cnt;
    bool copies_ordered = false;
    double* so_score = nullptr;
    uint64_t* so_kmer = nullptr;
    uint32_t* so_row = nullptr;
    size_t ring_end = 0;
    DevBuf<double> d_so_score;
    DevBuf<uint64_t> d_so_kmer;
    DevBuf<uint32_t> d_so_row;
    DevBuf<uint32_t> d_meta;
    PinBuf<uint32_t> h_meta;
    uint32_t* h_meta_dev = nullptr;
    double* h_thr_dev = nullptr;
    unsigned long long* h_tested_dev = nullptr;
    PinBuf<double> h_thr;
    bool tie_check = false;
    bool tested_in_meta = false;
    hipEvent_t ev_counts = nullptr;
    DevBuf<unsigned long long> d_tested;
    PinBuf<unsigned long long> h_tested;
    hipEvent_t ev_sq0 = nullptr, ev_k0 = nullptr, ev_k1 = nullptr, ev_done = nullptr, ev_mid = nullptr;
    bool used_coarse = false;
    int coarse_mode = 0;
    double cand_est = 0;
    const uint64_t* rows = nullptr;
    uint64_t first_row = 0, n_rows = 0;
    bool squeezed = false, busy = false;
};

}

using namespace kgwas;

struct kgwas_scan {
    int device = 0;
    uint64_t S_f = 0, S = 0, W_f = 0, W_m = 0, L = 0, n_pheno = 0, min_count = 0;
    std::vector<uint64_t> col, topn;
    std::vector<float> Y;
    bool direct = false;
    uint32_t kernel_used = 0;
    bool record_history = false;
    size_t history_ring = 0;
    uint64_t chunk_max = 0, dense_rows = 0, dense_chunk = 0;
    uint32_t cap = 0;
    uint64_t max_topn = 0;
    uint32_t nb_full = 0;

    hipStream_t stream = nullptr, copy_stream = nullptr;
    hipEvent_t ev_user = nullptr, ev_ds = nullptr, ev_d0 = nullptr, ev_d1 = nullptr;
    hipEvent_t ev_dcopy = nullptr;
    bool dense_copy_pending = false;
    DevBuf<uint32_t> d_dmask, d_colmap, d_sq;
    DevBuf<float> d_Yperm, d_Ymfma, d_sums;
    DevBuf<double> d_thr;
    PinBuf<double> h_thr;
    uint32_t thr_flip = 0;
    DevBuf<uint32_t> d_hist, d_hist_base;
    PinBuf<uint32_t> h_hist_base;
    DevBuf<uint64_t> d_topn;
    DevBuf<double> d_thr_host, d_thr_redo;
    PinBuf<double> h_thr_redo;
    bool hist_ready = false;
    uint64_t rows_submitted = 0;
    bool coarse = false;
    uint32_t n_kgroups = 0;
    struct CoarsePart {
        uint32_t T = 0, n_lgroups = 0;
        uint32_t stream = 0;
        uint32_t ng = 1;
        DevBuf<int8_t> d_Bq;
        DevBuf<CoarseCol> d_cols;
    };
    struct CoarseMode {
        bool ready = false;
        bool mx = false;
        uint32_t mx_full = 0, mx_quarter = 0, mx_s1_fp6 = 0, mx_scale0 = 0;
        uint32_t slices = 0, n_parts = 0;
        uint32_t tile_slices = 0;
        double tile_slices_eq = 0;
        float eg_max = 0, rall_max = 0, rmax_max = 0;
        CoarsePart part[2];
    } cmode[2];
    DevBuf<double> d_sel;
    PinBuf<double> h_sel;
    DevBuf<uint32_t> d_sel_info;
    PinBuf<uint32_t> h_sel_info;
    bool sel_valid = false;
    double infl_obs[2] = {4.0, 1.1};
    double mode_k = 0;
    std::chrono::steady_clock::time_point t_feed0;
    double t_ms() const { return std::chrono::duration<double, std::milli>(std::chrono::steady_clock::now() - t_feed0).count(); }
    uint64_t sum_topn = 0;
    bool narrow = false;
    bool narrow_pack1 = false;
    DevBuf<uint8_t> d_Bn;
    DevBuf<NarrowCol> d_ncols;
    DevBuf<unsigned long long> d_bitmap;
    uint64_t bitmap_words = 0;
    DevBuf<uint32_t> d_bm_blocks;
    DevBuf<unsigned long long> d_bm_mask;
    bool bitmap_clean = false;
    uint64_t slack_rows = 0;
    DevBuf<uint32_t> d_surv_sorted, d_surv_cnt, d_surv_off, d_key_count;
    DevBuf<uint32_t> d_tile_pref, d_tile_cnt;
    DevBuf<double> d_tmp_score;
    uint32_t key_slots = 0;
    uint32_t row_key_bits = 32;
    bool count_patterns = false;
    DevBuf<uint64_t> d_pat;
    DevBuf<unsigned long long> d_pat_cnt;
    uint64_t pat_upper = 0;
    Slot slot[MAX_SLOTS];
    PinBuf<uint8_t> ring;
    uint8_t* ring_dev = nullptr;
    bool streamed_feed = false;
    double* h_dense_dev = nullptr;
    uint32_t* h_n1_dev = nullptr;
    uint64_t* h_kmer_dev = nullptr;
    size_t ring_size = 0, ring_head = 0, ring_tail = 0;
    std::atomic<bool> ring_keep{false};
    size_t ring_feed_start = 0;
    uint64_t ring_freed = 0;
    Slot redo;
    int n_slots = MAX_SLOTS;
    DevBuf<double> d_dense;
    DevBuf<uint32_t> d_n1;
    DevBuf<uint64_t> d_kmer;
    PinBuf<double> h_dense;
    PinBuf<uint32_t> h_n1;
    PinBuf<uint64_t> h_kmer;
    DevBuf<unsigned long long> d_tested_dense;
    DevBuf<uint64_t> d_stage;
    Ingest ingest;

    struct HugeArena {
        void* p = nullptr;
        size_t bytes = 0;
        ~HugeArena() { free(p); }
    } heap_arena;
    std::unique_ptr<std::pmr::monotonic_buffer_resource> heap_mr;
    std::vector<BestHeap> heaps;
    bool lazy_enabled = false;
    bool dbg_keep_resid = false;
    std::vector<double> dbg_resid[3];
    struct DbgChunk {
        uint64_t first_row = 0, n_rows = 0;
        uint32_t set = 0, overflow = 0;
        std::vector<double> thr;
        std::vector<uint32_t> pairs;
    };
    bool dbg_keep_surv = false;
    std::vector<DbgChunk> dbg_chunks;
    bool lazy_log_mode = false;
    std::vector<LazyCol> lazy;
    std::atomic<bool> lazy_any{false};
    std::atomic<uint64_t> n_selected{0}, n_unselected{0}, lazy_pushes{0};
    uint64_t tie_check_rows = 0;
    std::vector<History> hist;
    std::vector<uint64_t> exp_kmer, exp_row;
    std::vector<double> exp_score;
    std::vector<std::vector<uint64_t>> keys;
    bool trace = false;
    std::vector<double> col_ms;
    bool all_full = false;
    uint64_t rows_done = 0;
    std::unique_ptr<Pool> pool;
    struct alignas(64) GroupState {
        std::atomic<uint64_t> done{0};
        std::atomic<uint32_t> busy{0};
    };
    std::atomic<size_t> n_groups{1};
    size_t n_groups0 = 1;
    std::vector<std::vector<uint32_t>> grp_cols;
    std::vector<std::vector<uint32_t>> grp_cols0;
    std::vector<int> grp_home;
    std::unique_ptr<std::atomic<int>[]> grp_owner;
    std::unique_ptr<GroupState[]> gstate;
    std::unique_ptr<std::atomic<uint32_t>[]> slot_left;
    std::atomic<int> rp_hungry{0};
    std::atomic<bool> rp_all_published{false};
    std::atomic<uint64_t> rp_final_pub{0};
    std::atomic<bool> final_feed{false};
    bool final_feed_next = false;
    std::unique_ptr<std::atomic<uint8_t>[]> col_popped;
    std::atomic<uint64_t> n_popped_ahead{0};
    std::mutex split_mu;
    bool split_lagging = true;
    uint64_t float_lead = 2;
    std::atomic<uint64_t> n_floated{0};
    int dbg_slow_worker = -1, dbg_slow_pct = 0, dbg_slow_min_us = 0;
    std::atomic<uint64_t> n_splits{0};
    std::atomic<uint64_t> seq_submitted{0}, seq_published{0}, seq_replayed{0};
    std::atomic<bool> rp_quit{false}, rp_failed{false};
    std::atomic<bool> rp_drain{false};
    std::atomic<int> rp_idle{0};
    std::mutex rp_mu;
    std::condition_variable rp_cv_work, rp_cv_done;
    std::function<void(size_t)> rp_fn;
    ReplayAcc rp_acc;
    std::atomic<uint64_t> prof_scan{0}, prof_heap{0};
    uint64_t rp_max_busy_ns = 0, rp_min_busy_ns = ~0ull;
    kgwas_scan_stats st{};
    bool finished = false;
    std::vector<std::vector<uint64_t>> res_kmer, res_row;
    std::vector<std::vector<double>> res_score;

    ~kgwas_scan() {
        (void)hipSetDevice(device);
        auto drop_events = [](Slot& s) {
            if (s.ev_sq0) (void)hipEventDestroy(s.ev_sq0);
            if (s.ev_k0) (void)hipEventDestroy(s.ev_k0);
            if (s.ev_k1) (void)hipEventDestroy(s.ev_k1);
            if (s.ev_done) (void)hipEventDestroy(s.ev_done);
            if (s.ev_mid) (void)hipEventDestroy(s.ev_mid);
            if (s.ev_counts) (void)hipEventDestroy(s.ev_counts);
        };
        for (auto& s : slot) drop_events(s);
        drop_events(redo);
        if (ev_user) (void)hipEventDestroy(ev_user);
        if (ev_ds) (void)hipEventDestroy(ev_ds);
        if (ev_dcopy) (void)hipEventDestroy(ev_dcopy);
        if (ev_d0) (void)hipEventDestroy(ev_d0);
        if (ev_d1) (void)hipEventDestroy(ev_d1);
        if (stream) (void)hipStreamDestroy(stream);
        if (copy_stream) (void)hipStreamDestroy(copy_stream);
    }
};

namespace kgwas {
void check_device(int device);
void make_heaps(kgwas_scan* s);
void fill_args(kgwas_scan* s, ScoreArgs& a, const uint64_t* d_rows, uint64_t n_rows, uint64_t first_row, bool squeezed);
void hash_patterns(kgwas_scan* s, const uint64_t* d_rows, uint64_t n_rows);
void upload_thresholds(kgwas_scan* s);
void refresh_full(kgwas_scan* s);
void run_dense(kgwas_scan* s, const uint64_t* d_rows, uint64_t n_rows, uint64_t first_row, double* scores_out, uint32_t* popcnt_out,
               bool replay, bool select = false);
void wait_dense_copy(kgwas_scan* s);
void dense_fill(kgwas_scan* s, uint64_t n_rows, uint64_t first_row, std::chrono::steady_clock::time_point td0,
                const std::function<void()>* meanwhile = nullptr);
int pick_coarse_mode(const kgwas_scan* s);
void submit_sparse(kgwas_scan* s, Slot& sl, const uint64_t* d_rows, uint64_t n_rows, uint64_t first_row, bool count_hist);
bool chunk_complete(kgwas_scan* s, Slot& sl);
uint64_t next_sparse_chunk(const kgwas_scan* s);
void wait_event(kgwas_scan* s, hipEvent_t ev);
bool fetch_records(kgwas_scan* s, Slot& sl, uint64_t seq);
void ring_to_recycling(kgwas_scan* s, uint64_t replayed);
uint64_t lazy_materialize(kgwas_scan* s, size_t j);
void lazy_materialize_all(kgwas_scan* s);
void lazy_finish_column(kgwas_scan* s, size_t j, bool known_tie = false);
void lazy_reset(kgwas_scan* s);
bool lazy_lowest(kgwas_scan* s, size_t j, double* lowest, bool* full);
void replay_group(kgwas_scan* s, Slot& sl, size_t g, ReplayAcc& acc);
void add_replay_stats(kgwas_scan* s, const ReplayAcc& a);
void replay_worker(kgwas_scan* s, size_t w);
void feed_device_impl(kgwas_scan* s, const uint64_t* d_rows, uint64_t n_rows, uint64_t first_row);
struct FilterOpts {
    int coarse_mx = -1;
    int coarse_slices = -1;
    bool mx_s1_fp6 = false;
    int mxs = 1, mxs_form = 0;
    bool narrow = true;
    bool debug_residuals = false;
    bool debug_survivors = false;
    bool mixed = true, split = true, narrow_pack = true;
    long long cap_mult = -1, cap_budget = 4ll << 20;
    double mode_k = 0.09;
};
FilterOpts read_filter_opts();
struct ScanShape {
    uint64_t S, L, W_m, W_f, P, max_topn;
    bool direct, finite, chain_safe;
};
struct FilterPart {
    uint64_t j0, n, cper;
    uint32_t T;
    uint64_t groups;
    uint32_t stream = 0, ng = 1;
};
struct FilterSet {
    bool mx = false;
    uint32_t slices = 0, s1_fp6 = 0;
    uint32_t n_full = 0, n_quarter = 0, n_steps = 0;
    std::vector<FilterPart> parts;
    uint32_t tile_slices = 0;
    double tile_slices_eq = 0;
};
struct ScanPlan {
    uint32_t kernel = 0;
    bool coarse = false, narrow = false, narrow_pack1 = false;
    bool use_mx = false;
    bool keep_resid = false;
    bool keep_surv = false;
    uint32_t n_kgroups = 0;
    uint64_t chunk_max = 0, dense_rows = 0, dense_chunk = 0;
    uint32_t cap = 0;
    FilterSet set[2];
};
ScanPlan plan_scan(const kgwas_scan_params& p, const ScanShape& sh, const FilterOpts& o, const std::vector<float>& Y,
                   std::vector<double> resid[3]);
struct ExactLayouts {
    std::vector<uint32_t> dmask, colmap;
    std::vector<float> Yperm, Ymfma, sums;
    uint32_t nb_full = 0;
};
ExactLayouts exact_layouts(const ScanShape& sh, const std::vector<uint64_t>& col, const std::vector<float>& Y);
struct NarrowOperands {
    std::vector<uint8_t> Bn;
    std::vector<NarrowCol> ncols;
};
NarrowOperands narrow_operands(const ScanShape& sh, const ScanPlan& pl, const std::vector<float>& Y, const std::vector<float>& sums,
                               double* resid);
struct PartOperands {
    std::vector<uint8_t> Bq;
    std::vector<CoarseCol> cols;
    float eg_max = 0, rall_max = 0, rmax_max = 0;
};
PartOperands int8_operands(const ScanShape& sh, uint32_t n_kgroups, const FilterSet& fs, const FilterPart& fp, const std::vector<float>& Y,
                           const std::vector<float>& sums, double* resid);
PartOperands block_scaled_operands(const ScanShape& sh, const FilterSet& fs, const FilterPart& fp, const std::vector<float>& Y,
                                   const std::vector<float>& sums, double* resid);
}
```

kmersgwas_amd/csrc/scan_plan.cpp:

```cpp
#include "scan_internal.h"

namespace kgwas {

FilterOpts read_filter_opts() {
    FilterOpts o;
    if (const char* e = opt_str("KGWAS_COARSE_MX"))
        if (*e) o.coarse_mx = atoll(e) != 0 ? 1 : 0;
    if (const char* e = opt_str("KGWAS_COARSE_SLICES")) o.coarse_slices = (atoi(e) == 1 || atoi(e) == 2) ? atoi(e) : 0;
    o.mx_s1_fp6 = opt_int("KGWAS_MX_S1", -1) == 6;
    o.mxs = (int)opt_int("KGWAS_MXS", 1);
    o.mxs_form = (int)opt_int("KGWAS_MXS_FORM", 0);
    o.narrow = !(opt_int("KGWAS_NARROW", 1) == 0);
    o.debug_residuals = opt_set("KGWAS_DEBUG_RESIDUALS");
    o.debug_survivors = opt_set("KGWAS_DEBUG_SURVIVORS");
    o.mixed = !(exp_int("KGWAS_COARSE_MIXED", 1) == 0);
    o.split = !exp_set("KGWAS_COARSE_NOSPLIT");
    o.narrow_pack = !(exp_int("KGWAS_NARROW_PACK", 1) == 0);
    o.cap_mult = exp_int("KGWAS_CAP_MULT", -1);
    o.cap_budget = exp_int("KGWAS_CAP_BUDGET", (long long)(4ull << 20));
    if (const char* e = exp_str("KGWAS_MODE_K")) o.mode_k = atof(e);
    return o;
}


static float permute_and_sum(const std::vector<float>& V, float* R) {
    const uint64_t L = V.size();
    for (uint64_t b = 0; b < L / 128; b++)
        for (uint64_t sx = 0; sx < 32; sx++)
            for (uint64_t l = 0; l < 4; l++) R[128 * b + 4 * sx + l] = V[128 * b + 32 * l + 31 - sx];
    volatile float sum = 0.0f;
    for (uint64_t i = 0; i < L; i++) sum = sum + R[i];
    return sum;
}

ExactLayouts exact_layouts(const ScanShape& sh, const std::vector<uint64_t>& col, const std::vector<float>& Y) {
    const uint64_t S = sh.S, L = sh.L, W_m = sh.W_m, P = sh.P;
    ExactLayouts ex;
    ex.dmask.assign(2 * W_m, 0);
    ex.colmap.assign(L, 0xFFFFFFFFu);
    for (uint64_t d = 0; d < 2 * W_m; d++) {
        if (!sh.direct)
            ex.dmask[d] = 0xFFFFFFFFu;
        else if (32 * d + 32 <= S)
            ex.dmask[d] = 0xFFFFFFFFu;
        else if (32 * d < S)
            ex.dmask[d] = (1u << (S - 32 * d)) - 1u;
    }
    for (uint64_t i = 0; i < S; i++) ex.colmap[i] = (uint32_t)col[i];
    const uint64_t P4 = (P + 3) / 4 * 4, nct = (P + 15) / 16;
    ex.Yperm.assign(P4 * L, 0.0f);
    ex.Ymfma.assign(nct * L * 16, 0.0f);
    ex.sums.assign(P, 0.0f);
    std::vector<float> V(L);
    for (uint64_t j = 0; j < P; j++) {
        std::fill(V.begin(), V.end(), 0.0f);
        for (uint64_t i = 0; i < S; i++) V[i] = Y[j * S + i];
        ex.sums[j] = permute_and_sum(V, &ex.Yperm[j * L]);
        const uint64_t ct = j / 16, n = j % 16;
        for (uint64_t b = 0; b < L / 128; b++)
            for (uint64_t l = 0; l < 4; l++)
                for (uint64_t sx = 0; sx < 32; sx++)
                {
                    const uint64_t t = sx / 4, kk = sx % 4;
                    ex.Ymfma[ct * L * 16 + (((b * 4 + l) * 2 + t / 4) * 64 + kk * 16 + n) * 4 + t % 4] =
                        V[128 * b + 32 * l + 31 - sx];
                }
    }
    const uint64_t avail = sh.direct ? 2 * sh.W_f : 2 * W_m;
    while (ex.nb_full < W_m / 2 && 4ull * ex.nb_full + 3 < avail && ex.dmask[4 * ex.nb_full] == 0xFFFFFFFFu &&
           ex.dmask[4 * ex.nb_full + 1] == 0xFFFFFFFFu && ex.dmask[4 * ex.nb_full + 2] == 0xFFFFFFFFu &&
           ex.dmask[4 * ex.nb_full + 3] == 0xFFFFFFFFu)
        ex.nb_full++;
    return ex;
}

struct ErrBound {
    float eg, rall, rmax;
    float egD, rallD, rmaxD;
};

static double chain_gamma(uint64_t L) {
    const double u32 = std::ldexp(1.0, -24);
    const double nterms = (double)L / 4.0 + 3.0;
    return nterms * u32 / (1.0 - nterms * u32);
}

static float up(double x) { return std::nextafter((float)x, std::numeric_limits<float>::infinity()); }

static void column_bound(uint64_t S, uint64_t L, double sum, double A, double u, double rpos, double rneg, double rmax,
                         CoarseCol& cc, ErrBound& eb) {
    const double Nd = (double)S;
    const double c = sum / Nd;
    const double rho = Nd * std::fabs(Nd * c - sum) * 2.0 + 1e-9 * (1.0 + std::fabs(sum));
    const double Eg = chain_gamma(L) * A * (1.0 + 1e-6) + 1e-12 * (1.0 + A);
    cc.kalpha = (1.0 - std::ldexp(1.0, -19)) / (Nd * u);
    cc.iu = up(1.0 / u * (1.0 + 1e-6));
    eb.eg = up((Eg + rho / Nd) * (1.0 + 1e-6) + 1e-30);
    eb.rall = up(std::max(rpos, rneg) * (1.0 + 1e-6));
    eb.rmax = up(rmax * (1.0 + 1e-6));
    const double iu = 1.0 / u * (1.0 + 1e-6);
    eb.egD = up((double)eb.eg * iu);
    eb.rallD = up((double)eb.rall * iu);
    eb.rmaxD = up((double)eb.rmax * iu);
}

static void narrow_bound(uint64_t S, uint64_t L, double sum, double c, double mx, double A, double rpos, double rneg, double rmax,
                         NarrowCol& nc) {
    const double Nd = (double)S;
    const double fuzz = 64.0 * std::ldexp(1.0, -52) * (mx + std::fabs(c));
    nc.t1 = Nd * c - sum;
    nc.eg = (chain_gamma(L) * A * (1.0 + 1e-6) + 1e-12 * (1.0 + A)) * (1.0 + 1e-9);
    nc.rall = (std::max(rpos, rneg) + Nd * fuzz) * (1.0 + 1e-9);
    nc.rmax = (rmax + fuzz) * (1.0 + 1e-9);
    nc.pad = 256.0 * std::ldexp(1.0, -52) * Nd * Nd * (mx + std::fabs(c) + 1.0) + 1e-300;
    const double slack = Nd * (nc.eg + std::min(nc.rall, Nd * nc.rmax)) + Nd * std::fabs(nc.t1) + nc.pad +
                         Nd * std::ldexp(1.0, -20) * mx * Nd;
    for (int k = 0; k < 3; k++) nc.wf[k] = (float)nc.w[k];
    nc.slackf = std::nextafter((float)(slack * 1.001), std::numeric_limits<float>::infinity());
}

static void quantise_int8(const float* y, uint64_t S, uint64_t L, double sum, int ns, int* q0, int* q1, double* resid,
                          CoarseCol& cc, ErrBound& eb) {
    const double c = sum / (double)S;
    double mx = 0, A = 0;
    for (uint64_t i = 0; i < S; i++) {
        mx = std::max(mx, std::fabs((double)y[i] - c));
        A += std::fabs((double)y[i]);
    }
    const double u = mx > 0 ? (ns == 2 ? mx / (127.0 * 254.0) : mx / 127.0) : 1.0;
    const double a0 = ns == 2 ? 254.0 * u : u;
    double rpos = 0, rneg = 0, rmax = 0;
    for (uint64_t i = 0; i < S; i++) {
        const double yc = (double)y[i] - c;
        int v0 = (int)std::lrint(yc / a0);
        v0 = std::max(-127, std::min(127, v0));
        double r = yc - a0 * v0;
        int v1 = 0;
        if (ns == 2) {
            v1 = (int)std::lrint(r / u);
            v1 = std::max(-127, std::min(127, v1));
            r -= u * v1;
        }
        q0[i] = v0;
        q1[i] = v1;
        if (resid) resid[i] = r;
        if (r > 0) rpos += r; else rneg -= r;
        rmax = std::max(rmax, std::fabs(r));
    }
    column_bound(S, L, sum, A, u, rpos, rneg, rmax, cc, eb);
}


static uint64_t tiles_for(uint64_t cols) { return (cols + 1 + 15) / 16; }

static uint64_t groups_for(uint64_t P, uint32_t tmax) {
    uint64_t g = 1;
    while (tmax && tiles_for((P + g - 1) / g) > tmax) g++;
    return tmax ? g : ~0ull;
}

static uint32_t resident_tiles(uint32_t n_steps, uint32_t ns, uint32_t s1_fp6) {
    for (uint32_t ct = 7; ct >= 1; ct--)
        if (mx_lds_bytes(n_steps, ct, ns, s1_fp6) <= 160u * 1024u) return ct;
    return 0u;
}

static bool streams(const FilterOpts& o, bool mxs_can, uint64_t P, uint32_t ct) {
    return mxs_can && (o.mxs >= 3 || !ct || (groups_for(P, ct) >= 2 && (o.mxs >= 2 || ct <= 2)));
}

static std::vector<FilterPart> split_parts(uint64_t P, uint32_t ns, uint32_t tmax, double premium, bool split) {
    const uint64_t groups = groups_for(P, tmax), cper = (P + groups - 1) / groups;
    const uint32_t T = ns * (uint32_t)tiles_for(cper);
    std::vector<FilterPart> parts{FilterPart{0, P, cper, T, groups}};
    const uint64_t cpf = (uint64_t)tmax * 16 - 1;
    const uint64_t full = P / cpf, rem = P - full * cpf;
    const uint64_t Tr = rem ? ns * tiles_for(rem) : 0;
    if (groups > 1 && split && full >= 1 && full + (rem ? 1 : 0) <= groups &&
        (double)(full * ns * tmax + Tr) + premium < (double)(groups * T)) {
        parts = {FilterPart{0, full * cpf, cpf, ns * tmax, full}};
        if (rem) parts.push_back(FilterPart{full * cpf, rem, rem, (uint32_t)Tr, 1});
    }
    return parts;
}

static FilterSet plan_int8(uint64_t P, int ns, uint32_t coarse_T, const FilterOpts& o) {
    FilterSet fs;
    fs.slices = (uint32_t)ns;
    const uint32_t Tmax = ns == 2 ? coarse_T & ~1u : coarse_T;
    fs.parts = split_parts(P, (uint32_t)ns, Tmax / (uint32_t)ns, 0.0, o.split);
    for (const FilterPart& fp : fs.parts) fs.tile_slices += fp.T * (uint32_t)fp.groups;
    return fs;
}

static FilterSet plan_block_scaled(uint64_t S, uint64_t P, int ns, uint32_t n_kgroups, bool mxs_can, const FilterOpts& o) {
    FilterSet fs;
    fs.mx = true;
    fs.slices = (uint32_t)ns;
    fs.n_full = (uint32_t)(S / 512);
    fs.n_quarter = (uint32_t)((S % 512 + 127) / 128);
    fs.n_steps = 4 * fs.n_full + fs.n_quarter;
    fs.s1_fp6 = ns == 2 && o.mx_s1_fp6 && resident_tiles(fs.n_steps, 2, 1) ? 1u : 0u;
    const uint32_t CTmax = resident_tiles(fs.n_steps, (uint32_t)ns, fs.s1_fp6);
    if (mxs_can && ns == 2 && !fs.s1_fp6 && streams(o, mxs_can, P, CTmax)) {
        uint64_t g = 1, ng = 1, ct = 0;
        uint32_t form = 0;
        if (P + 1 <= 7 * 16) {
            ct = std::max<uint64_t>(3, tiles_for(P));
        } else if (o.mxs_form == 1 || o.mxs_form == 2) {
            while (tiles_for((P + g - 1) / g) > 13) g++;
            ct = tiles_for((P + g - 1) / g);
            if (ct > 7) form = (uint32_t)o.mxs_form;
        } else {
            ng = 2;
            g = 2;
            while (tiles_for((P + g - 1) / g) > 7) g += 2;
            ct = std::max<uint64_t>(4, tiles_for((P + g - 1) / g));
        }
        if (mxs_supported((uint32_t)ct, (uint32_t)ng, 2, 0) && mxs_lds_bytes((uint32_t)ct, (uint32_t)ng) <= 160u * 1024u)
            fs.parts = {FilterPart{0, P, (P + g - 1) / g, (uint32_t)ct, g, 1u + form, (uint32_t)ng}};
    }
    if (!CTmax && fs.parts.empty()) throw Error(KGWAS_ERR_ARG, "coarse filter: too many accessions for the LDS");
    const bool streamed = !fs.parts.empty();
    if (!streamed) fs.parts = split_parts(P, 1, CTmax, 2.5, o.split);
    for (const FilterPart& fp : fs.parts) fs.tile_slices += fp.T * (uint32_t)ns * (uint32_t)fp.groups;
    fs.tile_slices_eq = (double)fs.tile_slices * (double)fs.n_steps / (8.0 * (double)n_kgroups) * ((CTmax <= 3 && !streamed) ? 1.30 : 1.0);
    return fs;
}

ScanPlan plan_scan(const kgwas_scan_params& p, const ScanShape& sh, const FilterOpts& o, const std::vector<float>& Y,
                   std::vector<double> resid[3]) {
    const uint64_t S = sh.S, P = sh.P;
    ScanPlan pl;
    uint32_t kern = p.kernel;
    const bool mfma_fits = mfma_lds_bytes((uint32_t)sh.W_m) <= 160u * 1024u;
    pl.n_kgroups = (uint32_t)((sh.W_m + 7) / 8);
    uint32_t coarse_T = 0;
    for (uint32_t T : {8u, 7u, 6u, 5u, 4u, 3u, 2u})
        if (coarse_lds_bytes(pl.n_kgroups, T) <= 152u * 1024u) {
            coarse_T = T;
            break;
        }
    const bool mxs_can = o.mxs != 0 && o.coarse_mx != 0 && o.coarse_slices < 0 && !o.mx_s1_fp6;
    const bool filter_fits = coarse_T != 0 || mxs_can;
    if (kern == KGWAS_KERNEL_COARSE) {
        if (!sh.chain_safe || !filter_fits)
            throw Error(KGWAS_ERR_ARG, "coarse filter needs finite phenotype values whose float32 sums cannot overflow (sum |y| < FLT_MAX per column) and, for its int8 form, <= 5120 accessions");
        pl.coarse = true;
        kern = KGWAS_KERNEL_AUTO;
    } else if (kern == KGWAS_KERNEL_AUTO && sh.chain_safe && filter_fits) {
        pl.coarse = true;
    }
    if (kern == KGWAS_KERNEL_AUTO) kern = (P >= 4 && sh.finite && mfma_fits) ? KGWAS_KERNEL_MFMA : KGWAS_KERNEL_VALU;
    if (kern == KGWAS_KERNEL_MFMA && !mfma_fits)
        throw Error(KGWAS_ERR_ARG, "MFMA scorer: phenotype tile does not fit LDS for this many accessions");
    if (kern == KGWAS_KERNEL_MFMA && !sh.finite)
        throw Error(KGWAS_ERR_ARG, "MFMA scorer needs finite phenotype values (0*inf); use the VALU scorer");
    if (kern != KGWAS_KERNEL_MFMA && kern != KGWAS_KERNEL_VALU) throw Error(KGWAS_ERR_ARG, "unknown kernel id");
    pl.kernel = kern;
    pl.narrow = pl.coarse && p.kernel == KGWAS_KERNEL_AUTO && P <= NARROW_MAX_COLS &&
                narrow_lds_bytes(pl.n_kgroups) <= 64u * 1024u && o.narrow;

    pl.chunk_max = p.chunk_rows ? p.chunk_rows : ((pl.narrow && sh.direct) ? (128ull << 20) : (8ull << 20));
    pl.chunk_max = std::max<uint64_t>(128, (pl.chunk_max + 127) / 128 * 128);
    if (pl.coarse) {
        uint32_t pbits = 1;
        while ((1ull << pbits) < P + 1) pbits++;
        if (pbits > 22) throw Error(KGWAS_ERR_ARG, "coarse filter: too many phenotype columns for 32-bit survivor keys");
        pl.chunk_max = std::max<uint64_t>(128, std::min<uint64_t>(pl.chunk_max, 1ull << (32 - pbits)));
    }
    if (pl.coarse && !pl.narrow) {
        const uint64_t stride_dw = 2 * (1 + std::max<uint64_t>(sh.W_f, sh.W_m));
        const uint64_t lim = ((1ull << 32) - (1ull << 20)) / (4 * stride_dw) / 128 * 128;
        pl.chunk_max = std::max<uint64_t>(128, std::min<uint64_t>(pl.chunk_max, lim));
    }
    pl.dense_rows = std::min<uint64_t>(16384, pl.chunk_max);
    pl.dense_chunk = std::min<uint64_t>(pl.dense_rows, std::max<uint64_t>(1024, (sh.max_topn + sh.max_topn / 8 + 512 + 127) / 128 * 128));
    const uint64_t budget = (uint64_t)o.cap_budget;
    const uint64_t cap_mult = (uint64_t)(o.cap_mult >= 0 ? o.cap_mult : (pl.narrow ? 16 : 2));
    const uint64_t cap = std::min<uint64_t>(cap_mult * sh.max_topn + 4096, std::max<uint64_t>(budget / P, 1024));
    pl.cap = (uint32_t)std::min<uint64_t>(cap, 0x7FFFFFFFull);
    if (!pl.coarse) return pl;

    pl.keep_resid = o.debug_residuals;
    pl.keep_surv = o.debug_survivors;
    if (pl.keep_resid)
        for (int f = 0; f < 3; f++) resid[f].assign(P * S, 0.0);
    std::vector<float> V(sh.L), R(sh.L);
    std::vector<int> q0(S), q1(S);
    bool one_ok = true;
    for (uint64_t j = 0; j < P && one_ok; j++) {
        const float* y = &Y[j * S];
        std::fill(V.begin(), V.end(), 0.0f);
        std::copy(y, y + S, V.begin());
        CoarseCol cc;
        ErrBound eb;
        quantise_int8(y, S, sh.L, (double)permute_and_sum(V, R.data()), 1, q0.data(), q1.data(),
                      pl.keep_resid ? &resid[0][j * S] : nullptr, cc, eb);
        double mean = 0, var = 0;
        for (uint64_t i = 0; i < S; i++) mean += (double)y[i];
        mean /= (double)S;
        for (uint64_t i = 0; i < S; i++) var += ((double)y[i] - mean) * ((double)y[i] - mean);
        const double sigma = std::sqrt(var / (double)S);
        const double e_half = (double)eb.eg + std::min((double)eb.rall, 0.5 * (double)S * (double)eb.rmax);
        if (!(e_half <= 0.15 * 2.0 * sigma * std::sqrt((double)S))) one_ok = false;
    }
    if (pl.narrow) {
        pl.narrow_pack1 = P == 1 && o.narrow_pack;
        return pl;
    }
    bool want[2] = {one_ok, true};
    if (o.coarse_slices == 1) want[0] = true, want[1] = false;
    if (o.coarse_slices == 2) want[0] = false, want[1] = true;
    if (o.coarse_mx >= 0) {
        pl.use_mx = o.coarse_mx == 1;
    } else {
        const uint32_t ctm = resident_tiles(4u * (uint32_t)(S / 512) + (uint32_t)((S % 512 + 127) / 128), 2, 0);
        pl.use_mx = streams(o, mxs_can, P, ctm) || !coarse_T || groups_for(P, ctm) <= groups_for(P, coarse_T) + 1;
    }
    const bool mixed = !pl.use_mx && o.coarse_mx < 0 && o.coarse_slices < 0 && want[0] && want[1] && o.mixed;
    if (pl.use_mx && o.coarse_slices < 0) want[0] = false;
    for (int mi = 0; mi < 2; mi++)
        if (want[mi])
            pl.set[mi] = (pl.use_mx || (mixed && mi == 1)) ? plan_block_scaled(S, P, mi + 1, pl.n_kgroups, mxs_can, o)
                                                           : plan_int8(P, mi + 1, coarse_T, o);
    return pl;
}


NarrowOperands narrow_operands(const ScanShape& sh, const ScanPlan& pl, const std::vector<float>& Y, const std::vector<float>& sums,
                               double* resid) {
    const uint64_t S = sh.S, P = sh.P, n_kgroups = pl.n_kgroups;
    auto e4m3 = [](int v) -> uint8_t {
        if (v == 0) return 0;
        const int sg = v < 0 ? 0x80 : 0, av = std::abs(v);
        int e = 0;
        while ((2 << e) <= av) e++;
        return (uint8_t)(sg | ((e + 7) << 3) | ((av * 8) / (1 << e) - 8));
    };
    const uint64_t n_steps = 4ull * n_kgroups;
    NarrowOperands op;
    op.Bn.assign(n_steps * 64 * 32, 0);
    op.ncols.resize(P);
    std::vector<int> q(S);
    auto put_slot = [&](uint64_t slot, const std::vector<int>& v) {
        for (uint64_t g = 0; g < n_kgroups; g++)
            for (uint64_t jj = 0; jj < 4; jj++)
                for (uint64_t k = 0; k < 128; k++) {
                    const uint64_t kbA = k / 32, e = k % 32, smp = 512 * g + 128 * kbA + 32 * (e / 8) + 4 * (e % 8) + jj;
                    if (smp >= S) continue;
                    const uint64_t lane = slot + 16 * ((k % 64) / 16), byte = (k / 64) * 16 + k % 16;
                    op.Bn[((g * 4 + jj) * 64 + lane) * 32 + byte] = e4m3(v[smp]);
                }
    };
    for (uint64_t j = 0; j < P; j++) {
        const double Nd = (double)S, sum = (double)sums[j];
        const double c = sum / Nd;
        double mx = 0, A = 0;
        std::vector<double> t(S);
        for (uint64_t i = 0; i < S; i++) {
            t[i] = (double)Y[j * S + i] - c;
            mx = std::max(mx, std::fabs(t[i]));
            A += std::fabs((double)Y[j * S + i]);
        }
        double u = mx > 0 ? mx / 15.0 : 1.0;
        NarrowCol& nc = op.ncols[j];
        for (int k = 0; k < NARROW_SLICES; k++) {
            for (uint64_t i = 0; i < S; i++) {
                int v = (int)std::lrint(t[i] / u);
                v = std::max(-15, std::min(15, v));
                q[i] = v;
                t[i] -= u * v;
            }
            put_slot(4 * j + k, q);
            if (pl.narrow_pack1)
                for (uint64_t t = 1; t < 4; t++) put_slot(4 * t + k, q);
            nc.w[k] = 2.0 * u;
            u /= 30.0;
        }
        double rpos = 0, rneg = 0, rmax = 0;
        for (uint64_t i = 0; i < S; i++) {
            if (resid) resid[j * S + i] = t[i];
            if (t[i] > 0) rpos += t[i]; else rneg -= t[i];
            rmax = std::max(rmax, std::fabs(t[i]));
        }
        narrow_bound(S, sh.L, sum, c, mx, A, rpos, rneg, rmax, nc);
    }
    for (uint64_t j = 0; j < (pl.narrow_pack1 ? 4 : P); j++) put_slot(4 * j + 3, std::vector<int>(S, 1));
    return op;
}

static PartOperands empty_part(const FilterPart& fp, size_t Bq_bytes, uint64_t slots) {
    PartOperands op;
    op.Bq.assign(Bq_bytes, 0);
    op.cols.resize(fp.groups * slots);
    for (auto& cc : op.cols) {
        memset(&cc, 0, sizeof(cc));
        cc.pheno = -1;
    }
    return op;
}

static void fold_bound(PartOperands& op, const ErrBound& eb) {
    op.eg_max = std::max(op.eg_max, eb.egD);
    op.rall_max = std::max(op.rall_max, eb.rallD);
    op.rmax_max = std::max(op.rmax_max, eb.rmaxD);
}

PartOperands int8_operands(const ScanShape& sh, uint32_t n_kgroups, const FilterSet& fs, const FilterPart& fp, const std::vector<float>& Y,
                           const std::vector<float>& sums, double* resid) {
    const uint64_t S = sh.S;
    const int ns = (int)fs.slices;
    const uint32_t Tp = fp.T, PG = Tp / (uint32_t)ns, slots = PG * 16;
    PartOperands op = empty_part(fp, fp.groups * n_kgroups * 8ull * Tp * 1024ull, slots);
    auto put = [&](uint64_t lg, uint64_t slot, const std::vector<int>& v0, const std::vector<int>& v1) {
        const uint64_t pgl = slot / 16, n = slot % 16;
        for (uint64_t g = 0; g < n_kgroups; g++)
            for (uint64_t jj = 0; jj < 8; jj++)
                for (uint64_t kg = 0; kg < 4; kg++)
                    for (uint64_t e = 0; e < 16; e++) {
                        const uint64_t smp = 512 * g + 128 * kg + 32 * (e / 4) + 8 * (e % 4) + jj;
                        if (smp >= S) continue;
                        const uint64_t lane = kg * 16 + n;
                        const uint64_t base = (((lg * n_kgroups + g) * 8 + jj) * Tp);
                        if (ns == 1) {
                            op.Bq[((base + pgl) * 64 + lane) * 16 + e] = (uint8_t)v0[smp];
                        } else {
                            op.Bq[((base + 2 * pgl) * 64 + lane) * 16 + e] = (uint8_t)v0[smp];
                            op.Bq[((base + 2 * pgl + 1) * 64 + lane) * 16 + e] = (uint8_t)v1[smp];
                        }
                    }
    };
    std::vector<int> q0(S), q1(S);
    for (uint64_t j = fp.j0; j < fp.j0 + fp.n; j++) {
        const uint64_t lg = (j - fp.j0) / fp.cper, slot = (j - fp.j0) % fp.cper;
        CoarseCol& cc = op.cols[lg * slots + slot];
        ErrBound eb;
        quantise_int8(&Y[j * S], S, sh.L, (double)sums[j], ns, q0.data(), q1.data(), resid ? resid + j * S : nullptr, cc, eb);
        fold_bound(op, eb);
        cc.pheno = (int32_t)j;
        put(lg, slot, q0, q1);
    }
    {
        std::vector<int> ones(S, 1), zeros(S, 0);
        for (uint64_t lg = 0; lg < fp.groups; lg++) put(lg, slots - 1, ns == 1 ? ones : zeros, ones);
    }
    return op;
}

PartOperands block_scaled_operands(const ScanShape& sh, const FilterSet& fs, const FilterPart& fp, const std::vector<float>& Y,
                                   const std::vector<float>& sums, double* resid) {
    const uint64_t S = sh.S;
    const int ns = (int)fs.slices;
    const uint32_t s1_fp6 = fs.s1_fp6, n_full = fs.n_full, n_steps = fs.n_steps;
    std::vector<int> G6, G4;
    for (int q = 60; q >= 32; q -= 4) G6.push_back(-q);
    for (int q = 30; q >= 16; q -= 2) G6.push_back(-q);
    for (int q = 15; q >= -15; q--) G6.push_back(-q);
    for (int q = 16; q <= 30; q += 2) G6.push_back(q);
    for (int q = 32; q <= 60; q += 4) G6.push_back(q);
    for (int h : {-12, -8, -6, -4, -3, -2, -1, 0, 1, 2, 3, 4, 6, 8, 12}) G4.push_back(h);
    auto nearest = [](const std::vector<int>& g, double v) {
        size_t hi = std::lower_bound(g.begin(), g.end(), v, [](int a, double b) { return (double)a < b; }) - g.begin();
        if (hi == 0) return (size_t)0;
        if (hi == g.size()) return g.size() - 1;
        return (v - (double)g[hi - 1] <= (double)g[hi] - v) ? hi - 1 : hi;
    };
    auto e2m3 = [](int q) -> uint32_t {
        const uint32_t sg = q < 0 ? 0x20u : 0u;
        const int a = std::abs(q);
        if (a < 8) return sg | (uint32_t)a;
        int e = 1, base = 8;
        while (a >= 2 * base) base *= 2, e++;
        return sg | ((uint32_t)e << 3) | (uint32_t)((a - base) / (base / 8));
    };
    auto e2m1 = [](int h) -> uint32_t {
        static const int tab[8] = {0, 1, 2, 3, 4, 6, 8, 12};
        uint32_t i = 0;
        while (tab[i] != std::abs(h)) i++;
        return (h < 0 ? 8u : 0u) | i;
    };
    const int sh1 = ns == 1 ? 0 : (s1_fp6 ? 5 : 3);
    const double kappa = (ns == 2 && !s1_fp6) ? 0.25 : 0.0625;
    const int t_ones = (int)(1.0 / kappa);
    const double t_max = ns == 1 ? 60.0 : (s1_fp6 ? 32.0 * 60.0 + 60.0 : 8.0 * 60.0 + 12.0);
    const std::vector<int>& G1 = s1_fp6 ? G6 : G4;
    auto quantise_mx = [&](uint64_t j, CoarseCol& cc, ErrBound& eb, std::vector<int>& a0, std::vector<int>& a1) {
        const double Nd = (double)S, sum = (double)sums[j];
        const double c = sum / Nd;
        double mx = 0, A = 0;
        for (uint64_t i = 0; i < S; i++) {
            const double y = (double)Y[j * S + i];
            mx = std::max(mx, std::fabs(y - c));
            A += std::fabs(y);
        }
        const double w = mx > 0 ? mx / t_max : 1.0;
        const double u = w / kappa;
        double rpos = 0, rneg = 0, rmax = 0;
        for (uint64_t i = 0; i < S; i++) {
            const double y = (double)Y[j * S + i] - c;
            const double x = y / w;
            int b0 = 0, b1 = 0;
            if (ns == 1) {
                b0 = G6[nearest(G6, x)];
            } else {
                const double sc = (double)(1 << sh1);
                const size_t k0 = nearest(G6, x / sc);
                double best = 1e300;
                for (size_t k = k0 ? k0 - 1 : 0; k <= std::min(k0 + 1, G6.size() - 1); k++) {
                    const int c1 = G1[nearest(G1, x - sc * G6[k])];
                    const double r = std::fabs(x - sc * G6[k] - c1);
                    if (r < best) best = r, b0 = G6[k], b1 = c1;
                }
            }
            a0[i] = b0;
            a1[i] = b1;
            const double r = y - w * ((double)(1 << sh1) * b0 + b1);
            if (resid) resid[j * S + i] = r;
            if (r > 0) rpos += r; else rneg -= r;
            rmax = std::max(rmax, std::fabs(r));
        }
        column_bound(S, sh.L, sum, A, u, rpos, rneg, rmax, cc, eb);
    };
    const uint32_t CT = fp.T, slots = CT * 16;
    const uint64_t NGs = fp.ng;
    const uint32_t SB = mx_step_bytes_rt((uint32_t)ns, s1_fp6);
    const size_t group_bytes = (size_t)n_steps * CT * SB;
    PartOperands op = empty_part(fp, fp.groups * group_bytes + 1024, slots);
    auto put = [&](uint64_t lg, uint64_t slot, const std::vector<int>& v0, const std::vector<int>& v1) {
        const uint64_t t = slot / 16, n = slot % 16;
        for (uint64_t st = 0; st < n_steps; st++) {
            uint8_t* blk = &op.Bq[(lg / NGs) * (NGs * group_bytes) + ((st * NGs + lg % NGs) * CT + t) * SB];
            for (uint64_t kb = 0; kb < 4; kb++) {
                const uint64_t lane = kb * 16 + n;
                for (uint64_t e = 0; e < 32; e++) {
                    const uint64_t smp = st < 4ull * n_full ? 512 * (st / 4) + 128 * kb + 32 * (e / 8) + 4 * (e % 8) + st % 4
                                                            : 512ull * n_full + 128 * (st - 4ull * n_full) + 32 * kb + 4 * (e % 8) + e / 8;
                    if (smp >= S) continue;
                    auto put6 = [&](uint8_t* part, int q) {
                        const uint32_t code = e2m3(q);
                        for (int b = 0; b < 6; b++)
                            if (code & (1u << b)) {
                                const uint64_t bit = 6 * e + b, dw = bit / 32;
                                uint8_t* d = dw < 4 ? part + lane * 16 + dw * 4 : part + 1024 + lane * 8 + (dw - 4) * 4;
                                d[(bit % 32) / 8] |= (uint8_t)(1u << (bit % 8));
                            }
                    };
                    put6(blk, v0[smp]);
                    if (ns == 2) {
                        if (s1_fp6)
                            put6(blk + 1536, v1[smp]);
                        else
                            blk[1536 + lane * 16 + e / 2] |= (uint8_t)(e2m1(v1[smp]) << (4 * (e % 2)));
                    }
                }
            }
        }
    };
    {
        std::vector<ErrBound> ebs(fp.n);
        const unsigned nt = (unsigned)std::max<uint64_t>(1, std::min<uint64_t>(std::min<uint64_t>(usable_cpus(), 16), fp.n / 4));
        std::atomic<uint64_t> next(0);
        kgwas_run_on_threads(nt, "kgwas-quant", [&] {
            std::vector<int> b0(S), b1(S);
            try {
                for (uint64_t i; (i = next.fetch_add(1, std::memory_order_relaxed)) < fp.n;) {
                    const uint64_t j = fp.j0 + i, lg = i / fp.cper, slot = i % fp.cper;
                    CoarseCol& cc = op.cols[lg * slots + slot];
                    quantise_mx(j, cc, ebs[i], b0, b1);
                    cc.pheno = (int32_t)j;
                    put(lg, slot, b0, b1);
                }
            } catch (...) {
                next.store(fp.n);
                throw;
            }
        });
        for (const ErrBound& eb : ebs) fold_bound(op, eb);
    }
    {
        std::vector<int> ones(S, t_ones), zeros(S, 0);
        for (uint64_t lg = 0; lg < fp.groups; lg++) put(lg, slots - 1, ns == 1 ? ones : zeros, ones);
    }
    return op;
}

}
```

kmersgwas_amd/csrc/score_mx.hip:

```cpp
#include <stdlib.h>

#include <algorithm>

#include "score_common.h"

#ifndef KGWAS_MX_ABLATE
#define KGWAS_MX_ABLATE 0
#endif

#ifndef KGWAS_MX_NT
#define KGWAS_MX_NT 0
#endif

#ifndef KGWAS_MX_WARM
#define KGWAS_MX_WARM 0
#endif
#ifndef KGWAS_MX_PERSIST
#define KGWAS_MX_PERSIST 1
#endif

namespace kgwas {

typedef int mxv8i __attribute__((ext_vector_type(8)));
typedef float mxv4f __attribute__((ext_vector_type(4)));

namespace {
constexpr uint32_t MX_PART0 = 1536u;
}

#ifndef KGWAS_MX_PRIO
#define KGWAS_MX_PRIO 0
#endif
#ifndef KGWAS_MX_PRIO_EPI
#define KGWAS_MX_PRIO_EPI 3
#endif

template <int NS, int S1F>
__host__ __device__ constexpr uint32_t mx_step_bytes() {
    return NS == 1 ? MX_PART0 : (S1F == 4 ? MX_PART0 + 1024u : 2u * MX_PART0);
}

template <int CT, int RT, int NS, int S1F, int TH>
__global__ void __launch_bounds__(TH) mx_kernel(MxArgs a, uint32_t rows_per_block, uint32_t n_rowblocks, uint32_t grid_lg) {
    extern __shared__ uint4 mlds[];
    constexpr uint32_t SB = mx_step_bytes<NS, S1F>();
    constexpr int SLOTS = CT * 16;
    constexpr int NW = RT / 4;
    uint32_t rb = blockIdx.x, lg0 = 0, lg1 = a.n_lgroups;
    if (grid_lg) {
        const uint32_t idx = blockIdx.x >> 3;
        rb = (idx / a.n_lgroups) * 8u + (blockIdx.x & 7u);
        lg0 = idx % a.n_lgroups;
        lg1 = lg0 + 1u;
    }
    const bool persist = KGWAS_MX_PERSIST && !grid_lg;
    if (!persist && rb >= n_rowblocks) return;
    const uint32_t lane = threadIdx.x & 63u, wave = threadIdx.x >> 6;
    const uint32_t kb = lane >> 4, m = lane & 15u;
    const uint32_t n_steps = 4u * a.n_full + a.n_quarter;
    const uint32_t group_bytes = n_steps * CT * SB;
    char* lds = reinterpret_cast<char*>(mlds);
    float* colc = reinterpret_cast<float*>(lds + group_bytes);
    const int* colp = reinterpret_cast<const int*>(colc + 2 * SLOTS);
    float* wscr = colc + 3 * SLOTS + wave * (RT * 48u);
    const uint32_t rows_per_pass = (TH / 64) * (RT * 16u);
    const uint64_t blk_row0 = (uint64_t)rb * rows_per_block;
    const float Nf = (float)a.S;
    const char* rows_base = reinterpret_cast<const char*>(a.src.base);
    const uint32_t avail_b = a.src.avail_dw * 4u;
    const int sc0 = (int)a.scale0;
    uint32_t tested_local = 0;

    for (uint32_t lg = lg0; lg < lg1; lg++) {
        if (lg != lg0) __syncthreads();
        {
            const uint4* src = reinterpret_cast<const uint4*>(a.Bq + (size_t)lg * group_bytes);
            for (uint32_t i = threadIdx.x; i < group_bytes / 16u; i += TH) mlds[i] = src[i];
            if (threadIdx.x < SLOTS) {
                const CoarseCol cc = a.cols[lg * SLOTS + threadIdx.x];
                float al = __builtin_huge_valf();
                if (cc.pheno >= 0) al = (float)(sqrt(a.thr[cc.pheno]) * cc.kalpha);
                colc[threadIdx.x] = al;
                colc[SLOTS + threadIdx.x] = cc.iu;
                reinterpret_cast<int*>(colc + 2 * SLOTS)[threadIdx.x] = cc.pheno;
            }
        }
        __syncthreads();

        uint32_t ro[RT];
        const uint64_t wave_row0 = blk_row0 + wave * (RT * 16u);
        auto set_rows = [&](uint32_t (&o)[RT], uint64_t rb0) {
#pragma unroll
            for (int rt = 0; rt < RT; rt++) {
                uint64_t r = rb0 + rt * 16u + m;
                if (r >= a.n_rows) r = a.n_rows - 1;
                o[rt] = ((uint32_t)r * (uint32_t)a.src.stride_dw + a.src.off_dw) * 4u;
            }
        };
        struct __attribute__((aligned(8))) U4 {
            uint32_t x, y, z, w;
        };
        auto load_group = [&](uint32_t (&pc)[RT][4], const uint32_t (&o)[RT], uint32_t g) {
            const uint32_t b0 = 64u * g + 16u * kb;
#pragma unroll
            for (int rt = 0; rt < RT; rt++) {
                uint32_t off = o[rt] + b0;
                asm volatile("" : "+v"(off));
                U4 v;
                if (KGWAS_MX_ABLATE & 8)
                    v = U4{off, lane * 2654435761u, lane, b0};
                else {
#if KGWAS_MX_NT
                    typedef uint32_t nt_u4 __attribute__((ext_vector_type(4), aligned(8)));
                    const nt_u4 t = __builtin_nontemporal_load(reinterpret_cast<const nt_u4*>(rows_base + off));
                    v = U4{t.x, t.y, t.z, t.w};
#else
                    v = *reinterpret_cast<const U4*>(rows_base + off);
#endif
                }
                pc[rt][0] = v.x;
                pc[rt][1] = v.y;
                pc[rt][2] = v.z;
                pc[rt][3] = v.w;
            }
        };
        constexpr int UT = 2;
        constexpr int NU = (CT + UT - 1) / UT;
        typedef uint32_t u32x4 __attribute__((ext_vector_type(4)));
        typedef uint32_t u32x2 __attribute__((ext_vector_type(2)));
        u32x4 Bx[CT], Bz[CT];
        u32x2 By[CT], Bv[CT];
#pragma unroll
        for (int t = 0; t < CT; t++) Bx[t] = Bz[t] = (u32x4){0u, 0u, 0u, 0u}, By[t] = Bv[t] = (u32x2){0u, 0u};
        struct StepAddr {
            uint32_t o16, o8, o8b;
        };
        auto step_addr = [&](const char* bstep) {
            StepAddr sa;
            sa.o16 = (uint32_t)(bstep - lds) + lane * 16u;
            sa.o8 = (uint32_t)(bstep - lds) + lane * 8u + 1024u;
            sa.o8b = sa.o8 + SB;
            asm volatile("" : "+v"(sa.o16), "+v"(sa.o8), "+v"(sa.o8b));
            return sa;
        };
        auto read_unit = [&](int u, const StepAddr& sa) {
#pragma unroll
            for (int t = UT * u; t < (UT * u + UT < CT ? UT * u + UT : CT); t++) {
                if (KGWAS_MX_ABLATE & 4) {
                    Bx[t] = (u32x4){lane, (uint32_t)t, 3u, (uint32_t)u};
                    By[t] = (u32x2){5u, 6u};
                    Bz[t] = (u32x4){lane, (uint32_t)t, 7u, (uint32_t)u};
                    Bv[t] = (u32x2){1u, 2u};
                    continue;
                }
                const char* p16 = lds + sa.o16 + t * SB;
                const char* p8 = (t & 1) ? lds + sa.o8b + (t - 1) * SB : lds + sa.o8 + t * SB;
                Bx[t] = *reinterpret_cast<const u32x4*>(p16);
                By[t] = *reinterpret_cast<const u32x2*>(p8);
                if (NS == 2) {
                    Bz[t] = *reinterpret_cast<const u32x4*>(p16 + MX_PART0);
                    if (S1F == 2) Bv[t] = *reinterpret_cast<const u32x2*>(p8 + MX_PART0);
                }
            }
        };
        uint32_t piece[RT][4];
        const uint64_t pass_stride = persist ? (uint64_t)gridDim.x * rows_per_pass : rows_per_pass;
        const uint64_t wave_row00 = persist ? (uint64_t)blockIdx.x * rows_per_pass + wave * (RT * 16u) : wave_row0;
        const uint64_t n_pass_blk = persist ? ~0ull : (rows_per_block + rows_per_pass - 1) / rows_per_pass;
        set_rows(ro, wave_row00);
        if (a.n_full && wave_row00 < a.n_rows) load_group(piece, ro, 0);
        StepAddr sadr = step_addr(lds);
        read_unit(0, sadr);
        for (uint64_t ps = 0; ps < n_pass_blk; ps++) {
            const uint64_t rbase = wave_row00 + ps * pass_stride;
            if (rbase >= a.n_rows) break;
            uint32_t ro_next[RT];
            set_rows(ro_next, rbase + pass_stride);
#if KGWAS_MX_WARM
            {
                const uint64_t r0 = rbase + pass_stride;
                if (r0 < a.n_rows) {
                    const uint64_t r1 = r0 + RT * 16u < a.n_rows ? r0 + RT * 16u : a.n_rows;
                    const uint32_t b0 = ((uint32_t)r0 * (uint32_t)a.src.stride_dw + a.src.off_dw) * 4u & ~127u;
                    const uint32_t b1 = ((uint32_t)(r1 - 1u) * (uint32_t)a.src.stride_dw + a.src.off_dw) * 4u + avail_b - 4u;
                    asm volatile("s_waitcnt vmcnt(0)" ::: "memory");
                    const uint32_t junk = (uint32_t)(reinterpret_cast<char*>(colc + 3 * SLOTS + (TH / 64) * (RT * 48u)) - lds);
                    const uint32_t n_warm = (b1 - b0) / 8192u + 1u;
                    for (uint32_t k = 0; k < n_warm; k++) {
                        uint32_t off = (b1 - b0) - k * 8192u >= lane * 128u ? b0 + k * 8192u + lane * 128u : b1;
                        asm volatile("s_mov_b32 m0, %0\n\ts_nop 0\n\tglobal_load_lds_dword %1, %2" ::"s"(junk), "v"(off), "s"(rows_base) : "memory");
                    }
                }
            }
#endif
            mxv4f acc[RT][CT];
#pragma unroll
            for (int rt = 0; rt < RT; rt++)
#pragma unroll
                for (int t = 0; t < CT; t++) acc[rt][t] = (mxv4f){0.0f, 0.0f, 0.0f, 0.0f};

            auto mfma_unit = [&](int u, const mxv8i (&A)[RT], int sa) {
#pragma unroll
                for (int t = UT * u; t < (UT * u + UT < CT ? UT * u + UT : CT); t++) {
                    const mxv8i B0 = {(int)Bx[t].x, (int)Bx[t].y, (int)Bx[t].z, (int)Bx[t].w, (int)By[t].x, (int)By[t].y, 0, 0};
#pragma unroll
                    for (int rt = 0; rt < RT; rt++)
                        acc[rt][t] = __builtin_amdgcn_mfma_scale_f32_16x16x128_f8f6f4(A[rt], B0, acc[rt][t], 4, 2, 0, sa, 0, sc0);
                    if (NS == 2) {
                        mxv8i B1 = {(int)Bz[t].x, (int)Bz[t].y, (int)Bz[t].z, (int)Bz[t].w, 0, 0, 0, 0};
                        if (S1F == 2) {
                            B1[4] = (int)Bv[t].x;
                            B1[5] = (int)Bv[t].y;
                        }
#pragma unroll
                        for (int rt = 0; rt < RT; rt++)
                            acc[rt][t] = __builtin_amdgcn_mfma_scale_f32_16x16x128_f8f6f4(A[rt], B1, acc[rt][t], 4, S1F, 0, sa, 0, 0x7F7F7F7F);
                    }
                }
            };
            auto run_step = [&](const mxv8i (&A)[RT], const char* bs_next, int sa) {
                const StepAddr nadr = step_addr(bs_next);
                if (NU == 1) {
                    u32x4 kx[CT], kz[CT];
                    u32x2 ky[CT], kv[CT];
#pragma unroll
                    for (int t = 0; t < CT; t++) kx[t] = Bx[t], ky[t] = By[t], kz[t] = Bz[t], kv[t] = Bv[t];
                    read_unit(0, nadr);
                    u32x4 nx[CT], nz[CT];
                    u32x2 ny[CT], nv[CT];
#pragma unroll
                    for (int t = 0; t < CT; t++) nx[t] = Bx[t], ny[t] = By[t], nz[t] = Bz[t], nv[t] = Bv[t];
#pragma unroll
                    for (int t = 0; t < CT; t++) Bx[t] = kx[t], By[t] = ky[t], Bz[t] = kz[t], Bv[t] = kv[t];
                    __builtin_amdgcn_sched_barrier(0);
                    mfma_unit(0, A, sa);
                    __builtin_amdgcn_sched_barrier(0);
#pragma unroll
                    for (int t = 0; t < CT; t++) Bx[t] = nx[t], By[t] = ny[t], Bz[t] = nz[t], Bv[t] = nv[t];
                } else {
#pragma unroll
                    for (int u = 0; u < NU; u++) {
                        if (u + 1 < NU)
                            read_unit(u + 1, sadr);
                        else
                            read_unit(0, nadr);
                        __builtin_amdgcn_sched_barrier(0);
                        mfma_unit(u, A, sa);
                        __builtin_amdgcn_sched_barrier(0);
                    }
                }
                sadr = nadr;
            };

#if KGWAS_MX_PRIO || KGWAS_MX_PRIO_EPI
            __builtin_amdgcn_s_setprio(KGWAS_MX_PRIO);
#endif
            for (uint32_t g = 0; g < a.n_full; g++) {
                const char* bg = lds + (size_t)g * 4u * CT * SB;
                const bool last_g = g + 1u == a.n_full;
#pragma unroll
                for (int j = 0; j < 4; j++) {
                    mxv8i A[RT];
#pragma unroll
                    for (int rt = 0; rt < RT; rt++) {
                        A[rt] = (mxv8i){0, 0, 0, 0, 0, 0, 0, 0};
#pragma unroll
                        for (int q = 0; q < 4; q++) {
                            if (KGWAS_MX_ABLATE & 2)
                                A[rt][q] = (int)piece[rt][q];
                            else
                                A[rt][q] = j < 3 ? (int)(piece[rt][q] & (0x11111111u << j)) : (int)((piece[rt][q] >> 1) & 0x44444444u);
                        }
                    }
                    const char* bs = bg + j * CT * SB;
                    const char* bs_next = bs + CT * SB;
                    if (j == 3) {
                        __builtin_amdgcn_sched_barrier(0);
                        uint32_t on[RT];
#pragma unroll
                        for (int rt = 0; rt < RT; rt++) on[rt] = last_g ? ro_next[rt] : ro[rt];
                        load_group(piece, on, last_g ? 0u : g + 1u);
                        if (last_g && a.n_quarter == 0) bs_next = lds;
                        __builtin_amdgcn_sched_barrier(0);
                    }
                    run_step(A, bs_next, j == 0 ? 0x7F7F7F7F : j == 1 ? 0x7E7E7E7E : 0x7D7D7D7D);
                }
            }
            for (uint32_t x = 0; x < a.n_quarter; x++) {
                uint32_t b0 = 64u * a.n_full + 16u * x + 4u * kb;
                b0 = b0 + 4u <= avail_b ? b0 : avail_b - 4u;
                mxv8i A[RT];
#pragma unroll
                for (int rt = 0; rt < RT; rt++) {
                    const uint32_t w = (KGWAS_MX_ABLATE & 8) ? ro[rt] + b0 : *reinterpret_cast<const uint32_t*>(rows_base + (ro[rt] + b0));
                    A[rt] = (mxv8i){(int)(w & 0x11111111u), (int)((w >> 1) & 0x11111111u), (int)((w >> 2) & 0x11111111u),
                                    (int)((w >> 3) & 0x11111111u), 0, 0, 0, 0};
                }
                const char* bs = lds + (size_t)(4u * a.n_full + x) * CT * SB;
                run_step(A, x + 1u == a.n_quarter ? lds : bs + CT * SB, 0x7F7F7F7F);
            }

#if KGWAS_MX_PRIO || KGWAS_MX_PRIO_EPI
            __builtin_amdgcn_s_setprio(KGWAS_MX_PRIO_EPI);
#endif
            float2* trm = reinterpret_cast<float2*>(wscr + RT * 16);
            {
                float* n1s = wscr;
                if (m == 15u) {
#pragma unroll
                    for (int rt = 0; rt < RT; rt++) *reinterpret_cast<mxv4f*>(n1s + kb * (RT * 4u) + rt * 4) = acc[rt][CT - 1];
                }
                __builtin_amdgcn_wave_barrier();
                const uint64_t left = a.n_rows - rbase;
                const uint32_t rows_here = left < RT * 16u ? (uint32_t)left : RT * 16u;
                const bool mac_any = a.S >= 2u * a.min_count;
                const uint32_t span = a.S - 2u * a.min_count;
#pragma unroll
                for (int w = 0; w < NW; w++) {
                    const uint32_t e = lane + 64u * w;
                    const uint32_t kbe = e / (RT * 4u), ie = e % (RT * 4u);
                    const uint32_t row = 16u * (ie >> 2) + 4u * kbe + (ie & 3u);
                    const float f = n1s[e];
                    const uint32_t n1r = (uint32_t)f;
                    const bool ok = mac_any & (row < rows_here) & ((n1r - a.min_count) <= span);
                    if (lg == 0) tested_local += ok ? 1u : 0u;
                    const float sq = __builtin_amdgcn_sqrtf(f * (Nf - f)) * 0.99999905f;
                    float2 tm;
                    tm.x = ok ? sq : __builtin_huge_valf();
                    tm.y = (a.eg_max + fminf(a.rall_max, f * a.rmax_max)) * 1.000001f;
                    trm[e] = tm;
                }
                __builtin_amdgcn_wave_barrier();
            }

            float alc[CT];
            float al_min = __builtin_huge_valf();
#pragma unroll
            for (int t = 0; t < CT; t++) {
                alc[t] = colc[t * 16 + m];
                al_min = fminf(al_min, alc[t]);
            }
            const bool ones_lane = m == 15u;
#pragma unroll
            for (int w = 0; w < NW; w++) {
                float sqd[16], er[16];
#pragma unroll
                for (int i = 0; i < 16; i += 2) {
                    const float4 v = *reinterpret_cast<const float4*>(trm + kb * (RT * 4u) + 16 * w + i);
                    sqd[i] = v.x;
                    er[i] = v.y;
                    sqd[i + 1] = v.z;
                    er[i + 1] = v.w;
                }
                auto pair_margin = [&](int i, int t, float al) {
                    const int gi = 16 * w + i;
                    return fmaf(-al, sqd[i], fabsf(acc[gi >> 2][t][gi & 3]));
                };
                uint64_t hit[16];
                if (!(KGWAS_MX_ABLATE & 1)) {
                    float mx[16];
#pragma unroll
                    for (int i = 0; i < 16; i++) {
                        const int gi = 16 * w + i;
                        const float v = acc[gi >> 2][CT - 1][gi & 3];
                        mx[i] = ones_lane ? 0.0f : fabsf(v);
                    }
#pragma unroll
                    for (int t = 0; t + 1 < CT; t++)
#pragma unroll
                        for (int i = 0; i < 16; i++) {
                            const int gi = 16 * w + i;
                            mx[i] = fmaxf(mx[i], fabsf(acc[gi >> 2][t][gi & 3]));
                        }
#pragma unroll
                    for (int i = 0; i < 16; i++) hit[i] = __ballot(fmaf(-al_min, sqd[i], mx[i]) + er[i] >= 0.0f);
                } else {
#pragma unroll
                    for (int i = 0; i < 16; i++) hit[i] = 0;
                    int x = 0;
#pragma unroll
                    for (int i = 0; i < 16; i++)
#pragma unroll
                        for (int t = 0; t < CT; t++) x ^= __float_as_int(acc[(16 * w + i) >> 2][t][i & 3]);
                    hit[0] = __ballot(x == 0x7fffffff);
                }
                uint64_t hit_any = 0;
#pragma unroll
                for (int i = 0; i < 16; i++) hit_any |= hit[i];
                if ((KGWAS_MX_ABLATE & 32) && hit_any) {
                    if (lane == 0) atomicAdd(&a.tested[0], 0ull);
                    hit_any = 0;
                }
                if (hit_any) {
                    uint32_t mb[CT];
#pragma unroll
                    for (int t = 0; t < CT; t++) mb[t] = 0;
#pragma unroll
                    for (int i = 0; i < 16; i++) {
                        if (hit[i]) {
#pragma unroll
                            for (int t = 0; t < CT; t++) {
                                float al = alc[t];
                                asm volatile("" : "+v"(al));
                                mb[t] |= (pair_margin(i, t, al) + er[i] >= 0.0f) ? (1u << i) : 0u;
                            }
                        }
                    }
                    unsigned short* bm16 = reinterpret_cast<unsigned short*>(a.bitmap) + ((rbase >> 6) + w) * 4u + kb;
#pragma unroll
                    for (int t = 0; t < CT; t++)
                        if (mb[t]) bm16[(uint64_t)colp[t * 16 + m] * a.words_per_col * 4u] = (unsigned short)mb[t];
                }
            }
            __builtin_amdgcn_wave_barrier();
#pragma unroll
            for (int rt = 0; rt < RT; rt++) ro[rt] = ro_next[rt];
        }
    }
#if KGWAS_MX_WARM
    asm volatile("s_waitcnt vmcnt(0)" ::: "memory");
#endif
    if (a.tested) {
        uint32_t v = tested_local;
#pragma unroll
        for (int d = 1; d < 64; d <<= 1) v += __shfl_xor(v, d);
        if (lane == 0u && v) atomicAdd(&a.tested[blockIdx.x % TESTED_SHARDS], (unsigned long long)v);
    }
}

size_t mx_lds_bytes(uint32_t n_steps, uint32_t CT, uint32_t n_slices, uint32_t s1_fp6) {
    const uint32_t sb = n_slices == 1 ? MX_PART0 : (s1_fp6 ? 2u * MX_PART0 : MX_PART0 + 1024u);
    return (size_t)n_steps * CT * sb + 3u * 112u * 4u + 12u * 768u + 256u;
}
uint32_t mx_step_bytes_rt(uint32_t n_slices, uint32_t s1_fp6) { return n_slices == 1 ? MX_PART0 : (s1_fp6 ? 2u * MX_PART0 : MX_PART0 + 1024u); }
uint32_t mx_row_tiles(uint32_t CT) { return 4u; }

template <int CT, int RT, int NS, int S1F, int TH = 512>
static hipError_t launch_mx_t(const MxArgs& a, uint32_t rows_per_block, size_t lds, hipStream_t st) {
    const uint32_t rpp = (TH / 64) * RT * 16u;
    rows_per_block = (rows_per_block + rpp - 1) / rpp * rpp;
    const uint32_t n_rowblocks = (uint32_t)((a.n_rows + rows_per_block - 1) / rows_per_block);
    if (lds > 64 * 1024) {
        hipError_t e = hipFuncSetAttribute((const void*)mx_kernel<CT, RT, NS, S1F, TH>, hipFuncAttributeMaxDynamicSharedMemorySize, (int)lds);
        if (e != hipSuccess) return e;
    }
    const uint32_t grid_lg = a.n_lgroups > 1 ? 1u : 0u;
    uint32_t grid = grid_lg ? (n_rowblocks + 7u) / 8u * 8u * a.n_lgroups : n_rowblocks;
    if (KGWAS_MX_PERSIST && !grid_lg) {
        static int n_cu = 0;
        if (!n_cu) {
            int dev = 0;
            hipDeviceProp_t pr;
            n_cu = (hipGetDevice(&dev) == hipSuccess && hipGetDeviceProperties(&pr, dev) == hipSuccess && pr.multiProcessorCount > 0) ? pr.multiProcessorCount : 256;
        }
        const uint64_t n_pass = (a.n_rows + rpp - 1) / rpp;
        grid = (uint32_t)std::min<uint64_t>(n_pass, (uint64_t)n_cu);
    }
    launch_last(mx_kernel<CT, RT, NS, S1F, TH>, dim3(grid), dim3(TH), lds, st, a, rows_per_block, n_rowblocks, grid_lg);
    return hipGetLastError();
}

template <int NS, int S1F>
static hipError_t launch_mx_ct(const MxArgs& a, uint32_t CT, uint32_t rows_per_block, size_t lds, hipStream_t st) {
    switch (CT) {
        case 1: return launch_mx_t<1, 4, NS, S1F, 768>(a, rows_per_block, lds, st);
        case 2: return launch_mx_t<2, 4, NS, S1F, 768>(a, rows_per_block, lds, st);
        case 3: return launch_mx_t<3, 4, NS, S1F, 768>(a, rows_per_block, lds, st);
        case 4: return launch_mx_t<4, 4, NS, S1F>(a, rows_per_block, lds, st);
        case 5: return launch_mx_t<5, 4, NS, S1F>(a, rows_per_block, lds, st);
        case 6: return launch_mx_t<6, 4, NS, S1F>(a, rows_per_block, lds, st);
        case 7: return launch_mx_t<7, 4, NS, S1F>(a, rows_per_block, lds, st);
    }
    return hipErrorInvalidValue;
}

hipError_t launch_mx(const MxArgs& a, uint32_t CT, uint32_t rows_per_block, hipStream_t st) {
    if (a.n_rows == 0) return hipSuccess;
    const size_t lds = mx_lds_bytes(4u * a.n_full + a.n_quarter, CT, a.n_slices, a.s1_fp6);
    if (lds > 160u * 1024u) return hipErrorInvalidValue;
    if ((a.n_rows * a.src.stride_dw + a.src.off_dw + a.src.avail_dw) * 4ull >= (1ull << 32)) return hipErrorInvalidValue;
#ifdef KGWAS_MX_BENCH_ONLY
    if (a.n_slices == 2 && !a.s1_fp6 && CT == 7) return launch_mx_t<7, 4, 2, 4>(a, rows_per_block, lds, st);
    return hipErrorInvalidValue;
#else
    if (a.n_slices == 1) return launch_mx_ct<1, 4>(a, CT, rows_per_block, lds, st);
    if (a.n_slices == 2 && !a.s1_fp6) return launch_mx_ct<2, 4>(a, CT, rows_per_block, lds, st);
    if (a.n_slices == 2 && a.s1_fp6) return launch_mx_ct<2, 2>(a, CT, rows_per_block, lds, st);
    return hipErrorInvalidValue;
#endif
}

}
```

Baseline: 552.9 billion.

## Fold FP4 slice of last MX tile into FP6 padding to shrink LDS footprint

```diff
diff --git a/include/kgwas.h b/include/kgwas.h
--- a/include/kgwas.h
+++ b/include/kgwas.h
@@ -117,9 +117,11 @@
     uint32_t coarse_mx_stream;
     uint32_t columns_selected;
     uint32_t columns_replayed_at_finish;
+    uint32_t coarse_mx_fold;
+    uint32_t reserved1;
 } kgwas_scan_stats;
 
-#define KGWAS_ABI_VERSION 14
+#define KGWAS_ABI_VERSION 15
 uint32_t kgwas_abi_version(void);
 
 int kgwas_scan_create(const kgwas_scan_params* p, kgwas_scan** out);
diff --git a/kmersgwas_amd/capi.py b/kmersgwas_amd/capi.py
--- a/kmersgwas_amd/capi.py
+++ b/kmersgwas_amd/capi.py
@@ -78,6 +78,7 @@
         ("columns_popped_ahead", C.c_uint64),
         ("coarse_mx32", C.c_uint32), ("coarse_mx_stream", C.c_uint32),
         ("columns_selected", C.c_uint32), ("columns_replayed_at_finish", C.c_uint32),
+        ("coarse_mx_fold", C.c_uint32), ("reserved1", C.c_uint32),
     ]
 
     def as_dict(self):
@@ -143,7 +144,7 @@
 lib.kgwas_device_count.argtypes = [C.POINTER(C.c_int)]
 lib.kgwas_abi_version.argtypes = []
 lib.kgwas_abi_version.restype = C.c_uint32
-ABI_VERSION = 14
+ABI_VERSION = 15
 if lib.kgwas_abi_version() != ABI_VERSION:
     raise ImportError("libkgwas.so speaks ABI version %d, kmersgwas_amd/capi.py %d: rebuild (make -C kmersgwas_amd/csrc)" % (lib.kgwas_abi_version(), ABI_VERSION))
 lib.kgwas_host_cpu_quota.argtypes = []
diff --git a/kmersgwas_amd/csrc/kernels.h b/kmersgwas_amd/csrc/kernels.h
--- a/kmersgwas_amd/csrc/kernels.h
+++ b/kmersgwas_amd/csrc/kernels.h
@@ -104,6 +104,8 @@
     uint32_t n_slices;
     uint32_t s1_fp6;
     uint32_t scale0;
+    uint32_t fold;
+    uint32_t n_cu;
     const uint8_t* Bq;
     const CoarseCol* cols;
     const double* thr;
@@ -112,7 +114,9 @@
     unsigned long long* tested;
     float eg_max, rall_max, rmax_max;
 };
-size_t mx_lds_bytes(uint32_t n_steps, uint32_t CT, uint32_t n_slices, uint32_t s1_fp6);
+constexpr uint32_t MX_FOLD_SLOTS = 8;
+constexpr uint32_t mx_ones_slot(bool fold) { return fold ? MX_FOLD_SLOTS - 1u : 15u; }
+size_t mx_lds_bytes(uint32_t n_steps, uint32_t CT, uint32_t n_slices, uint32_t s1_fp6, uint32_t fold = 0);
 uint32_t mx_step_bytes_rt(uint32_t n_slices, uint32_t s1_fp6);
 uint32_t mx_row_tiles(uint32_t CT);
 hipError_t launch_mx(const MxArgs& a, uint32_t CT, uint32_t rows_per_block, hipStream_t st);
diff --git a/kmersgwas_amd/csrc/scan_api.cpp b/kmersgwas_amd/csrc/scan_api.cpp
--- a/kmersgwas_amd/csrc/scan_api.cpp
+++ b/kmersgwas_amd/csrc/scan_api.cpp
@@ -628,6 +628,7 @@
         s->st.coarse_mx_s1_fp6 = old.coarse_mx_s1_fp6;
         s->st.coarse_mx_steps = old.coarse_mx_steps;
         s->st.coarse_mx_stream = old.coarse_mx_stream;
+        s->st.coarse_mx_fold = old.coarse_mx_fold;
         s->st.replay_threads = old.replay_threads;
         for (int mi = 0; mi < 2; mi++) {
             s->st.coarse_mode_tiles[mi] = old.coarse_mode_tiles[mi];
diff --git a/kmersgwas_amd/csrc/scan_create.cpp b/kmersgwas_amd/csrc/scan_create.cpp
--- a/kmersgwas_amd/csrc/scan_create.cpp
+++ b/kmersgwas_amd/csrc/scan_create.cpp
@@ -21,6 +21,11 @@
     KGWAS_HIP(hipSetDevice(p->device));
     std::unique_ptr<kgwas_scan> s(new kgwas_scan);
     s->device = p->device;
+    {
+        int n_cu = 0;
+        KGWAS_HIP(hipDeviceGetAttribute(&n_cu, hipDeviceAttributeMultiprocessorCount, p->device));
+        s->n_cu = n_cu > 0 ? (uint32_t)n_cu : 256u;
+    }
     s->S_f = p->n_acc_file;
     s->S = p->n_acc;
     s->W_f = (s->S_f + 63) / 64;
@@ -148,7 +153,9 @@
             Pt.n_lgroups = (uint32_t)(fp.groups / fp.ng);
             Pt.stream = fp.stream;
             Pt.ng = fp.ng;
+            Pt.fold = fp.fold;
             if (fp.stream) s->st.coarse_mx_stream = fp.stream;
+            if (fp.fold) s->st.coarse_mx_fold = 1;
             groups_all += Pt.n_lgroups;
             double* resid = s->dbg_keep_resid ? s->dbg_resid[mi].data() : nullptr;
             const PartOperands op = fs.mx ? block_scaled_operands(sh, fs, fp, s->Y, sums, resid)
diff --git a/kmersgwas_amd/csrc/scan_gpu.cpp b/kmersgwas_amd/csrc/scan_gpu.cpp
--- a/kmersgwas_amd/csrc/scan_gpu.cpp
+++ b/kmersgwas_amd/csrc/scan_gpu.cpp
@@ -412,6 +412,8 @@
                     x.n_slices = M.slices;
                     x.s1_fp6 = M.mx_s1_fp6;
                     x.scale0 = M.mx_scale0;
+                    x.fold = Pt.fold;
+                    x.n_cu = s->n_cu;
                     x.Bq = reinterpret_cast<const uint8_t*>(Pt.d_Bq.p);
                     x.cols = Pt.d_cols.p;
                     x.thr = c.thr;
diff --git a/kmersgwas_amd/csrc/scan_internal.h b/kmersgwas_amd/csrc/scan_internal.h
--- a/kmersgwas_amd/csrc/scan_internal.h
+++ b/kmersgwas_amd/csrc/scan_internal.h
@@ -359,6 +359,7 @@
 
 struct kgwas_scan {
     int device = 0;
+    uint32_t n_cu = 0;
     uint64_t S_f = 0, S = 0, W_f = 0, W_m = 0, L = 0, n_pheno = 0, min_count = 0;
     std::vector<uint64_t> col, topn;
     std::vector<float> Y;
@@ -393,6 +394,7 @@
         uint32_t T = 0, n_lgroups = 0;
         uint32_t stream = 0;
         uint32_t ng = 1;
+        uint32_t fold = 0;
         DevBuf<int8_t> d_Bq;
         DevBuf<CoarseCol> d_cols;
     };
@@ -585,6 +587,7 @@
     int coarse_slices = -1;
     bool mx_s1_fp6 = false;
     int mxs = 1, mxs_form = 0;
+    int mx_fold = 1;
     bool narrow = true;
     bool debug_residuals = false;
     bool debug_survivors = false;
@@ -602,6 +605,7 @@
     uint32_t T;
     uint64_t groups;
     uint32_t stream = 0, ng = 1;
+    uint32_t fold = 0;
 };
 struct FilterSet {
     bool mx = false;
diff --git a/kmersgwas_amd/csrc/scan_plan.cpp b/kmersgwas_amd/csrc/scan_plan.cpp
--- a/kmersgwas_amd/csrc/scan_plan.cpp
+++ b/kmersgwas_amd/csrc/scan_plan.cpp
@@ -10,6 +10,7 @@
     o.mx_s1_fp6 = opt_int("KGWAS_MX_S1", -1) == 6;
     o.mxs = (int)opt_int("KGWAS_MXS", 1);
     o.mxs_form = (int)opt_int("KGWAS_MXS_FORM", 0);
+    o.mx_fold = (int)std::max<long long>(0, std::min<long long>(2, opt_int("KGWAS_MX_FOLD", o.mxs == 0 ? 0 : 1)));
     o.narrow = !(opt_int("KGWAS_NARROW", 1) == 0);
     o.debug_residuals = opt_set("KGWAS_DEBUG_RESIDUALS");
     o.debug_survivors = opt_set("KGWAS_DEBUG_SURVIVORS");
@@ -163,6 +164,16 @@
     for (uint32_t ct = 7; ct >= 1; ct--)
         if (mx_lds_bytes(n_steps, ct, ns, s1_fp6) <= 160u * 1024u) return ct;
     return 0u;
+}
+
+static uint32_t folded_tiles(uint32_t n_steps) {
+    for (uint32_t ct = 7; ct >= 2; ct--)
+        if (mx_lds_bytes(n_steps, ct, 2, 0, 1) <= 160u * 1024u) return ct;
+    return 0u;
+}
+static uint32_t folded_group_tiles(uint64_t P, uint64_t groups, uint32_t ctf) {
+    const uint64_t cper = (P + groups - 1) / groups, ct = tiles_for(cper);
+    return (ct >= 2 && ct <= ctf && cper + 1 - (ct - 1) * 16 <= MX_FOLD_SLOTS) ? (uint32_t)ct : 0u;
 }
 
 static bool streams(const FilterOpts& o, bool mxs_can, uint64_t P, uint32_t ct) {
@@ -222,9 +233,23 @@
     }
     if (!CTmax && fs.parts.empty()) throw Error(KGWAS_ERR_ARG, "coarse filter: too many accessions for the LDS");
     const bool streamed = !fs.parts.empty();
-    if (!streamed) fs.parts = split_parts(P, 1, CTmax, 2.5, o.split);
+    if (!streamed && ns == 2 && !fs.s1_fp6 && o.mx_fold >= 1 && CTmax) {
+        const uint32_t ctf = folded_tiles(fs.n_steps);
+        const uint64_t g_plain = groups_for(P, CTmax);
+        uint64_t g = 1;
+        if (o.mx_fold >= 2)
+            while (g < g_plain && !folded_group_tiles(P, g, ctf)) g++;
+        const uint32_t ct = (ctf && g < g_plain) ? folded_group_tiles(P, g, ctf) : 0u;
+        if (ct) {
+            FilterPart fp{0, P, (P + g - 1) / g, ct, g};
+            fp.fold = 1;
+            fs.parts = {fp};
+        }
+    }
+    const bool folded = !fs.parts.empty() && fs.parts[0].fold;
+    if (fs.parts.empty()) fs.parts = split_parts(P, 1, CTmax, 2.5, o.split);
     for (const FilterPart& fp : fs.parts) fs.tile_slices += fp.T * (uint32_t)ns * (uint32_t)fp.groups;
-    fs.tile_slices_eq = (double)fs.tile_slices * (double)fs.n_steps / (8.0 * (double)n_kgroups) * ((CTmax <= 3 && !streamed) ? 1.30 : 1.0);
+    fs.tile_slices_eq = (double)fs.tile_slices * (double)fs.n_steps / (8.0 * (double)n_kgroups) * (((folded ? fs.parts[0].T : CTmax) <= 3 && !streamed) ? 1.30 : 1.0);
     return fs;
 }
 
@@ -525,12 +550,18 @@
     const uint32_t CT = fp.T, slots = CT * 16;
     const uint64_t NGs = fp.ng;
     const uint32_t SB = mx_step_bytes_rt((uint32_t)ns, s1_fp6);
-    const size_t group_bytes = (size_t)n_steps * CT * SB;
+    const bool fold = fp.fold != 0;
+    if (fold && !(ns == 2 && !s1_fp6 && !fp.stream && NGs == 1 && CT >= 2 && fp.cper + 1 <= (CT - 1) * 16ull + MX_FOLD_SLOTS))
+        throw Error(KGWAS_ERR_STATE, "block-scaled operands: a folded tile needs FP6 + FP4 slices and at most 8 used slots");
+    const size_t step_bytes = (size_t)NGs * CT * SB - (fold ? 1024u : 0u);
+    const size_t group_bytes = (size_t)n_steps * (CT * SB - (fold ? 1024u : 0u));
+    const uint64_t ones_slot = (CT - 1) * 16ull + mx_ones_slot(fold);
     PartOperands op = empty_part(fp, fp.groups * group_bytes + 1024, slots);
     auto put = [&](uint64_t lg, uint64_t slot, const std::vector<int>& v0, const std::vector<int>& v1) {
         const uint64_t t = slot / 16, n = slot % 16;
         for (uint64_t st = 0; st < n_steps; st++) {
-            uint8_t* blk = &op.Bq[(lg / NGs) * (NGs * group_bytes) + ((st * NGs + lg % NGs) * CT + t) * SB];
+            uint8_t* blk = &op.Bq[(lg / NGs) * (NGs * group_bytes) + st * step_bytes + ((lg % NGs) * CT + t) * SB];
+            const size_t fp4_at = (fold && t == CT - 1u) ? 128u : 1536u;
             for (uint64_t kb = 0; kb < 4; kb++) {
                 const uint64_t lane = kb * 16 + n;
                 for (uint64_t e = 0; e < 32; e++) {
@@ -551,7 +582,7 @@
                         if (s1_fp6)
                             put6(blk + 1536, v1[smp]);
                         else
-                            blk[1536 + lane * 16 + e / 2] |= (uint8_t)(e2m1(v1[smp]) << (4 * (e % 2)));
+                            blk[fp4_at + lane * 16 + e / 2] |= (uint8_t)(e2m1(v1[smp]) << (4 * (e % 2)));
                     }
                 }
             }
@@ -580,7 +611,7 @@
     }
     {
         std::vector<int> ones(S, t_ones), zeros(S, 0);
-        for (uint64_t lg = 0; lg < fp.groups; lg++) put(lg, slots - 1, ns == 1 ? ones : zeros, ones);
+        for (uint64_t lg = 0; lg < fp.groups; lg++) put(lg, ones_slot, ns == 1 ? ones : zeros, ones);
     }
     return op;
 }
diff --git a/kmersgwas_amd/csrc/score_mx.hip b/kmersgwas_amd/csrc/score_mx.hip
--- a/kmersgwas_amd/csrc/score_mx.hip
+++ b/kmersgwas_amd/csrc/score_mx.hip
@@ -40,10 +40,13 @@
     return NS == 1 ? MX_PART0 : (S1F == 4 ? MX_PART0 + 1024u : 2u * MX_PART0);
 }
 
-template <int CT, int RT, int NS, int S1F, int TH>
+template <int CT, int RT, int NS, int S1F, int TH, bool FOLD>
 __global__ void __launch_bounds__(TH) mx_kernel(MxArgs a, uint32_t rows_per_block, uint32_t n_rowblocks, uint32_t grid_lg) {
+    static_assert(!FOLD || (NS == 2 && S1F == 4 && CT >= 2), "folded last tile: FP6 + FP4 slices, two tiles or more");
     extern __shared__ uint4 mlds[];
     constexpr uint32_t SB = mx_step_bytes<NS, S1F>();
+    constexpr uint32_t STEPB = CT * SB - (FOLD ? 1024u : 0u);
+    constexpr uint32_t ONES_M = mx_ones_slot(FOLD);
     constexpr int SLOTS = CT * 16;
     constexpr int NW = RT / 4;
     uint32_t rb = blockIdx.x, lg0 = 0, lg1 = a.n_lgroups;
@@ -58,7 +61,7 @@
     const uint32_t lane = threadIdx.x & 63u, wave = threadIdx.x >> 6;
     const uint32_t kb = lane >> 4, m = lane & 15u;
     const uint32_t n_steps = 4u * a.n_full + a.n_quarter;
-    const uint32_t group_bytes = n_steps * CT * SB;
+    const uint32_t group_bytes = FOLD ? n_steps * STEPB : n_steps * CT * SB;
     char* lds = reinterpret_cast<char*>(mlds);
     float* colc = reinterpret_cast<float*>(lds + group_bytes);
     const int* colp = reinterpret_cast<const int*>(colc + 2 * SLOTS);
@@ -158,7 +161,7 @@
                 Bx[t] = *reinterpret_cast<const u32x4*>(p16);
                 By[t] = *reinterpret_cast<const u32x2*>(p8);
                 if (NS == 2) {
-                    Bz[t] = *reinterpret_cast<const u32x4*>(p16 + MX_PART0);
+                    Bz[t] = *reinterpret_cast<const u32x4*>(p16 + ((FOLD && t == CT - 1) ? 128u : MX_PART0));
                     if (S1F == 2) Bv[t] = *reinterpret_cast<const u32x2*>(p8 + MX_PART0);
                 }
             }
@@ -256,7 +259,7 @@
             __builtin_amdgcn_s_setprio(KGWAS_MX_PRIO);
 #endif
             for (uint32_t g = 0; g < a.n_full; g++) {
-                const char* bg = lds + (size_t)g * 4u * CT * SB;
+                const char* bg = lds + (FOLD ? (size_t)g * 4u * STEPB : (size_t)g * 4u * CT * SB);
                 const bool last_g = g + 1u == a.n_full;
 #pragma unroll
                 for (int j = 0; j < 4; j++) {
@@ -272,8 +275,8 @@
                                 A[rt][q] = j < 3 ? (int)(piece[rt][q] & (0x11111111u << j)) : (int)((piece[rt][q] >> 1) & 0x44444444u);
                         }
                     }
-                    const char* bs = bg + j * CT * SB;
-                    const char* bs_next = bs + CT * SB;
+                    const char* bs = bg + (FOLD ? j * STEPB : j * CT * SB);
+                    const char* bs_next = bs + (FOLD ? STEPB : CT * SB);
                     if (j == 3) {
                         __builtin_amdgcn_sched_barrier(0);
                         uint32_t on[RT];
@@ -296,8 +299,8 @@
                     A[rt] = (mxv8i){(int)(w & 0x11111111u), (int)((w >> 1) & 0x11111111u), (int)((w >> 2) & 0x11111111u),
                                     (int)((w >> 3) & 0x11111111u), 0, 0, 0, 0};
                 }
-                const char* bs = lds + (size_t)(4u * a.n_full + x) * CT * SB;
-                run_step(A, x + 1u == a.n_quarter ? lds : bs + CT * SB, 0x7F7F7F7F);
+                const char* bs = lds + (FOLD ? (size_t)(4u * a.n_full + x) * STEPB : (size_t)(4u * a.n_full + x) * CT * SB);
+                run_step(A, x + 1u == a.n_quarter ? lds : bs + (FOLD ? STEPB : CT * SB), 0x7F7F7F7F);
             }
 
 #if KGWAS_MX_PRIO || KGWAS_MX_PRIO_EPI
@@ -306,7 +309,7 @@
             float2* trm = reinterpret_cast<float2*>(wscr + RT * 16);
             {
                 float* n1s = wscr;
-                if (m == 15u) {
+                if (m == ONES_M) {
 #pragma unroll
                     for (int rt = 0; rt < RT; rt++) *reinterpret_cast<mxv4f*>(n1s + kb * (RT * 4u) + rt * 4) = acc[rt][CT - 1];
                 }
@@ -340,7 +343,7 @@
                 alc[t] = colc[t * 16 + m];
                 al_min = fminf(al_min, alc[t]);
             }
-            const bool ones_lane = m == 15u;
+            const bool ones_lane = FOLD ? m >= ONES_M : m == ONES_M;
 #pragma unroll
             for (int w = 0; w < NW; w++) {
                 float sqd[16], er[16];
@@ -428,35 +431,30 @@
     }
 }
 
-size_t mx_lds_bytes(uint32_t n_steps, uint32_t CT, uint32_t n_slices, uint32_t s1_fp6) {
+size_t mx_lds_bytes(uint32_t n_steps, uint32_t CT, uint32_t n_slices, uint32_t s1_fp6, uint32_t fold) {
     const uint32_t sb = n_slices == 1 ? MX_PART0 : (s1_fp6 ? 2u * MX_PART0 : MX_PART0 + 1024u);
-    return (size_t)n_steps * CT * sb + 3u * 112u * 4u + 12u * 768u + 256u;
+    const uint32_t n_waves = (fold && CT > 3) ? 8u : 12u;
+    return (size_t)n_steps * (CT * sb - (fold ? 1024u : 0u)) + 3u * 112u * 4u + n_waves * 768u + 256u;
 }
 uint32_t mx_step_bytes_rt(uint32_t n_slices, uint32_t s1_fp6) { return n_slices == 1 ? MX_PART0 : (s1_fp6 ? 2u * MX_PART0 : MX_PART0 + 1024u); }
 uint32_t mx_row_tiles(uint32_t CT) { return 4u; }
 
-template <int CT, int RT, int NS, int S1F, int TH = 512>
+template <int CT, int RT, int NS, int S1F, int TH = 512, bool FOLD = false>
 static hipError_t launch_mx_t(const MxArgs& a, uint32_t rows_per_block, size_t lds, hipStream_t st) {
     const uint32_t rpp = (TH / 64) * RT * 16u;
     rows_per_block = (rows_per_block + rpp - 1) / rpp * rpp;
     const uint32_t n_rowblocks = (uint32_t)((a.n_rows + rows_per_block - 1) / rows_per_block);
     if (lds > 64 * 1024) {
-        hipError_t e = hipFuncSetAttribute((const void*)mx_kernel<CT, RT, NS, S1F, TH>, hipFuncAttributeMaxDynamicSharedMemorySize, (int)lds);
+        hipError_t e = hipFuncSetAttribute((const void*)mx_kernel<CT, RT, NS, S1F, TH, FOLD>, hipFuncAttributeMaxDynamicSharedMemorySize, (int)lds);
         if (e != hipSuccess) return e;
     }
     const uint32_t grid_lg = a.n_lgroups > 1 ? 1u : 0u;
     uint32_t grid = grid_lg ? (n_rowblocks + 7u) / 8u * 8u * a.n_lgroups : n_rowblocks;
     if (KGWAS_MX_PERSIST && !grid_lg) {
-        static int n_cu = 0;
-        if (!n_cu) {
-            int dev = 0;
-            hipDeviceProp_t pr;
-            n_cu = (hipGetDevice(&dev) == hipSuccess && hipGetDeviceProperties(&pr, dev) == hipSuccess && pr.multiProcessorCount > 0) ? pr.multiProcessorCount : 256;
-        }
         const uint64_t n_pass = (a.n_rows + rpp - 1) / rpp;
-        grid = (uint32_t)std::min<uint64_t>(n_pass, (uint64_t)n_cu);
-    }
-    launch_last(mx_kernel<CT, RT, NS, S1F, TH>, dim3(grid), dim3(TH), lds, st, a, rows_per_block, n_rowblocks, grid_lg);
+        grid = (uint32_t)std::min<uint64_t>(n_pass, (uint64_t)a.n_cu);
+    }
+    launch_last(mx_kernel<CT, RT, NS, S1F, TH, FOLD>, dim3(grid), dim3(TH), lds, st, a, rows_per_block, n_rowblocks, grid_lg);
     return hipGetLastError();
 }
 
@@ -474,15 +472,30 @@
     return hipErrorInvalidValue;
 }
 
+static hipError_t launch_mx_fold(const MxArgs& a, uint32_t CT, uint32_t rows_per_block, size_t lds, hipStream_t st) {
+    switch (CT) {
+        case 2: return launch_mx_t<2, 4, 2, 4, 768, true>(a, rows_per_block, lds, st);
+        case 3: return launch_mx_t<3, 4, 2, 4, 768, true>(a, rows_per_block, lds, st);
+        case 4: return launch_mx_t<4, 4, 2, 4, 512, true>(a, rows_per_block, lds, st);
+        case 5: return launch_mx_t<5, 4, 2, 4, 512, true>(a, rows_per_block, lds, st);
+        case 6: return launch_mx_t<6, 4, 2, 4, 512, true>(a, rows_per_block, lds, st);
+        case 7: return launch_mx_t<7, 4, 2, 4, 512, true>(a, rows_per_block, lds, st);
+    }
+    return hipErrorInvalidValue;
+}
+
 hipError_t launch_mx(const MxArgs& a, uint32_t CT, uint32_t rows_per_block, hipStream_t st) {
     if (a.n_rows == 0) return hipSuccess;
-    const size_t lds = mx_lds_bytes(4u * a.n_full + a.n_quarter, CT, a.n_slices, a.s1_fp6);
+    if (a.fold && !(a.n_slices == 2 && !a.s1_fp6)) return hipErrorInvalidValue;
+    if (a.n_cu == 0) return hipErrorInvalidValue;
+    const size_t lds = mx_lds_bytes(4u * a.n_full + a.n_quarter, CT, a.n_slices, a.s1_fp6, a.fold);
     if (lds > 160u * 1024u) return hipErrorInvalidValue;
     if ((a.n_rows * a.src.stride_dw + a.src.off_dw + a.src.avail_dw) * 4ull >= (1ull << 32)) return hipErrorInvalidValue;
 #ifdef KGWAS_MX_BENCH_ONLY
-    if (a.n_slices == 2 && !a.s1_fp6 && CT == 7) return launch_mx_t<7, 4, 2, 4>(a, rows_per_block, lds, st);
+    if (a.n_slices == 2 && !a.s1_fp6 && CT == 7) return a.fold ? launch_mx_t<7, 4, 2, 4, 512, true>(a, rows_per_block, lds, st) : launch_mx_t<7, 4, 2, 4>(a, rows_per_block, lds, st);
     return hipErrorInvalidValue;
 #else
+    if (a.fold) return launch_mx_fold(a, CT, rows_per_block, lds, st);
     if (a.n_slices == 1) return launch_mx_ct<1, 4>(a, CT, rows_per_block, lds, st);
     if (a.n_slices == 2 && !a.s1_fp6) return launch_mx_ct<2, 4>(a, CT, rows_per_block, lds, st);
     if (a.n_slices == 2 && a.s1_fp6) return launch_mx_ct<2, 2>(a, CT, rows_per_block, lds, st);
```

Result: slower. 546.5 billion (-1.2%).
